# JuliaSmoothOptimizers/CaNNOLeS.jl

Hardware: AMD Instinct MI355X
Metric: Newton systems/sec (fp64), batched n=1e4 NLS; achieved HBM GB/s vs peak (higher is better)
Workload: dtype f64; 1 GPU; cfg3 band constrained NLS n=10000 nequ=10000 ncon=50, 16384 independent problems per GPU, one newton_system! per problem per step; batch_per_gpu=16384, total_problems=16384, ordering=canonical+early, nnzL_stored=145150, nnzL_exact=100180, fronts=1000, all_success=True

## Files before the change

cannoles.jl_amd/csrc/band.cpp:

```cpp
#include "band.h"

#include <algorithm>
#include <cstdio>
#include <map>

namespace cnl {

namespace {

struct XEnt { int32_t src; };
struct RowInfo {
  int32_t dsrc = -1, ndiag = 0;
  std::vector<int32_t> xs, srcs;
};
struct BorderInfo {
  int32_t dsrc = -1, ndiag = 0;
  std::vector<int32_t> xs, srcs;
};

struct RowOp { int32_t di, j[BAND_NB], rr, r; };
struct StepOp {
  int32_t flags = 0;
  int32_t dg[3] = {-1, -1, -1}, rho = -1, od[2 * BAND_HW], bc[2] = {-1, -1}, rx = -1;
  int32_t border = -1;
  int32_t xpiv = -1;
  int32_t lev_b = -1, lev_x = -1;
  std::vector<RowOp> rows;
  StepOp() { for (int i = 0; i < 2 * BAND_HW; i++) od[i] = -1; }
};
inline int32_t rhs_src(int64_t i) { return (int32_t)(-(i + 2)); }

struct Packer {
  int32_t len[3];
  struct Piece { int32_t arr, base, slot; };
  std::vector<Piece> pieces;
  bool pack(std::vector<int32_t> (&need)[3]) {
    pieces.clear();
    for (int a = 0; a < 3; a++) {
      std::vector<int32_t>& v = need[a];
      std::sort(v.begin(), v.end());
      v.erase(std::unique(v.begin(), v.end()), v.end());
      size_t i = 0;
      while (i < v.size()) {
        int32_t b = v[i];
        if (b > len[a] - 8) b = len[a] - 8;
        if (b < 0) return false;
        pieces.push_back({a, b, (int32_t)pieces.size()});
        while (i < v.size() && v[i] < b + 8) i++;
      }
    }
    return (int)pieces.size() <= npiece;
  }
  int32_t npiece = BAND_NPIECE;
  int32_t esz = 8;
  int32_t off(int a, int32_t e) const {
    for (const Piece& pc : pieces)
      if (pc.arr == a && e >= pc.base && e < pc.base + 8) return (int32_t)((BAND_IN_OFF + 8 * pc.slot + (e - pc.base)) * esz);
    return -1;
  }
};

}

void build_band_plan(BandPlan& B, int64_t N, int64_t nnz, const int64_t* rows1, const int64_t* cols1, int64_t nvar, int64_t nequ,
                     int64_t ncon, int nparts_wanted, int esz, int npiece) {
  B = BandPlan();
  if (esz != 8 && esz != 4) { B.ok = false; B.why = "element size must be 8 or 4 bytes"; return; }
  if (npiece != BAND_NPIECE && npiece != BAND_NPIECE_WIDE) { B.ok = false; B.why = "piece count must be 15 or 20"; return; }
  B.npiece = npiece;
  const int32_t LOUT_OFF = band_lout_off(npiece), DX_OFF = band_dx_off(npiece), DR_OFF = band_dr_off(npiece), ZERO_OFF = band_zero_off(npiece);
  const int32_t EW = band_ew(npiece);
  auto EF = [npiece](int f) { return band_ef(f, npiece); };
  auto no = [&](const std::string& w) { B.ok = false; B.why = w; };
  const int64_t n = nvar, m = nequ, p = ncon;
  if (N != n + m + p) return no("N != nvar + nequ + ncon");
  if (n < 2 * BAND_NB + 2 || nnz < 16 || N < 16 || nnz >= (1 << 27) || N >= (1 << 27)) return no("size out of range");
  B.n = (int32_t)n; B.N = (int32_t)N; B.nnz = (int32_t)nnz;
  std::vector<std::vector<int32_t>> xx_of_col(n);
  std::vector<int32_t> xx_row(nnz, -1);
  std::vector<RowInfo> R(m);
  std::vector<BorderInfo> L(p);
  for (int64_t e = 0; e < nnz; e++) {
    const int64_t r0 = rows1[e] - 1, c0 = cols1[e] - 1;
    if (r0 < 0 || r0 >= N || c0 < 0 || c0 > r0) return no("entry outside the lower triangle");
    if (r0 < n) {
      if (r0 - c0 > BAND_HW) return no("Hessian entry outside the band");
      xx_of_col[c0].push_back((int32_t)e);
      xx_row[e] = (int32_t)r0;
    } else if (r0 < n + m) {
      RowInfo& q = R[r0 - n];
      if (c0 < n) { q.xs.push_back((int32_t)c0); q.srcs.push_back((int32_t)e); }
      else if (c0 == r0) { q.dsrc = (int32_t)e; q.ndiag++; }
      else return no("entry inside the residual block off its diagonal");
    } else {
      BorderInfo& q = L[r0 - n - m];
      if (c0 < n) { q.xs.push_back((int32_t)c0); q.srcs.push_back((int32_t)e); }
      else if (c0 == r0) { q.dsrc = (int32_t)e; q.ndiag++; }
      else return no("entry coupling a multiplier with a residual or another multiplier");
    }
  }
  for (int64_t r = 0; r < m; r++) {
    RowInfo& q = R[r];
    if (q.ndiag != 1) return no("residual row without exactly one diagonal entry");
    if (!q.xs.empty()) {
      const auto mm = std::minmax_element(q.xs.begin(), q.xs.end());
      if (*mm.second - *mm.first > BAND_HW) return no("residual row wider than the band");
      std::vector<int32_t> s = q.xs;
      std::sort(s.begin(), s.end());
      if (std::adjacent_find(s.begin(), s.end()) != s.end()) return no("duplicate Jacobian entry");
    }
  }
  for (int64_t k = 0; k < p; k++) {
    BorderInfo& q = L[k];
    if (q.ndiag != 1) return no("multiplier without exactly one diagonal entry");
    if (q.xs.empty()) return no("constraint row without entries");
  }
  const int64_t rho_begin = nnz - n;
  int nparts = nparts_wanted >= 2 && n >= 16 * BAND_NB ? 2 : 1;
  int32_t m0 = (int32_t)n;
  if (nparts == 2) {
    auto valid = [&](int64_t c) {
      if (c < BAND_NB || c + BAND_HW + BAND_NB > n) return false;
      for (int64_t k = 0; k < p; k++) {
        const auto mm = std::minmax_element(L[k].xs.begin(), L[k].xs.end());
        if (!(*mm.second < c + BAND_HW || *mm.first >= c)) return false;
      }
      return true;
    };
    const int64_t want = (n - BAND_HW) / 2;
    int64_t found = -1;
    for (int64_t dlt = 0; dlt <= n / 4 && found < 0; dlt++) {
      if (valid(want + dlt)) found = want + dlt;
      else if (valid(want - dlt)) found = want - dlt;
    }
    if (found < 0) nparts = 1;
    else m0 = (int32_t)found;
  }
  B.nparts = nparts; B.m0 = m0;
  int64_t loff = 0;
  for (int part = 0; part < nparts; part++) {
    BandPart& Q = B.part[part];
    std::vector<int32_t> seq;
    int32_t npiv;
    if (nparts == 1) { for (int32_t x = 0; x < n; x++) seq.push_back(x); npiv = (int32_t)n; }
    else if (part == 0) { for (int32_t x = 0; x < m0 + BAND_HW; x++) seq.push_back(x); npiv = m0; }
    else { for (int32_t x = (int32_t)n - 1; x >= m0; x--) seq.push_back(x); npiv = (int32_t)n - m0 - BAND_HW; }
    std::vector<int32_t> pos(n, -1);
    for (size_t t = 0; t < seq.size(); t++) pos[seq[t]] = (int32_t)t;
    auto owns = [&](int32_t hi) { return nparts == 1 || (part == 0 ? hi < m0 + BAND_HW : hi >= m0 + BAND_HW); };
    const int32_t nsteps_raw = npiv + BAND_HW;
    std::vector<StepOp> S(nsteps_raw);
    for (int32_t u = 0; u < nsteps_raw; u++) {
      if (u < (int32_t)seq.size()) S[u].flags |= BF_ENTER_X;
      if (u >= BAND_HW && u - BAND_HW < npiv) { S[u].flags |= BF_PIVOT_X; S[u].xpiv = seq[u - BAND_HW]; }
    }
    for (int64_t c = 0; c < n; c++)
      for (int32_t e : xx_of_col[c]) {
        const int32_t a = xx_row[e], b = (int32_t)c;
        if (!owns(std::max(a, b))) continue;
        if (pos[a] < 0 || pos[b] < 0) return no("internal: entry outside its part");
        const int32_t u = std::max(pos[a], pos[b]), k = std::abs(pos[a] - pos[b]);
        StepOp& st = S[u];
        if (k == 0) {
          if (e >= rho_begin) { if (st.rho >= 0) return no("two rho slots on one variable"); st.rho = e; }
          else {
            if (st.rho >= 0) return no("plain entry behind the rho slot");
            int q = 0;
            while (q < 3 && st.dg[q] >= 0) q++;
            if (q == 3) return no("more than three plain entries on one diagonal position");
            st.dg[q] = e;
          }
        } else {
          int32_t* o = st.od + 2 * (k - 1);
          if (o[0] < 0) o[0] = e;
          else if (o[1] < 0) o[1] = e;
          else return no("more than two entries on one off-diagonal position");
        }
      }
    for (size_t t = 0; t < seq.size(); t++)
      if (owns(seq[t])) S[t].rx = rhs_src(seq[t]);
    struct RowAt { int32_t r, u, deadline; };
    std::vector<RowAt> mine_rows;
    for (int64_t r = 0; r < m; r++) {
      const RowInfo& q = R[r];
      int32_t hi = -1;
      for (int32_t x : q.xs) hi = std::max(hi, x);
      if (q.xs.empty()) { if (part == 0) mine_rows.push_back({(int32_t)r, 0, 0}); continue; }
      if (!owns(hi)) continue;
      int32_t plo = 1 << 30, phi = -1;
      for (int32_t x : q.xs) { if (pos[x] < 0) return no("internal: row outside its part"); plo = std::min(plo, pos[x]); phi = std::max(phi, pos[x]); }
      if (phi - plo > BAND_HW) return no("residual row wider than the band");
      mine_rows.push_back({(int32_t)r, phi, std::min(plo + BAND_HW, nsteps_raw - 1)});
    }
    std::stable_sort(mine_rows.begin(), mine_rows.end(), [&](const RowAt& x, const RowAt& y) { return x.u != y.u ? x.u < y.u : (part == 0 ? x.r < y.r : x.r > y.r); });
    {
      int32_t next_free = 0;
      for (RowAt& ra : mine_rows) {
        const int32_t want = std::max(ra.u, next_free);
        if (want <= ra.deadline) ra.u = want;
        next_free = std::max(next_free, ra.u + 1);
      }
    }
    for (const RowAt& ra : mine_rows) {
      const RowInfo& q = R[ra.r];
      const int32_t u = ra.u;
      RowOp ro;
      ro.di = q.dsrc; ro.rr = rhs_src(n + ra.r); ro.r = ra.r;
      for (int s = 0; s < BAND_NB; s++) ro.j[s] = -1;
      for (size_t i = 0; i < q.xs.size(); i++) {
        const int32_t k = pos[q.xs[i]] - (u - BAND_HW);
        if (k < 0 || k > BAND_HW) return no("internal: row column outside the window");
        ro.j[k] = q.srcs[i];
      }
      S[u].rows.push_back(ro);
    }
    for (StepOp& st : S) {
      if (st.rows.size() > 15) return no("more than 15 residual rows complete at one variable");
      std::sort(st.rows.begin(), st.rows.end(), [&](const RowOp& x, const RowOp& y) { return part == 0 ? x.r < y.r : x.r > y.r; });
    }
    std::vector<std::pair<int32_t, int32_t>> live;
    for (int64_t k = 0; k < p; k++) {
      const BorderInfo& q = L[k];
      int32_t lo = 1 << 30, hi = -1;
      for (int32_t x : q.xs) { lo = std::min(lo, x); hi = std::max(hi, x); }
      const bool mine = nparts == 1 || (part == 0 ? hi < m0 + BAND_HW : !(hi < m0 + BAND_HW));
      if (!mine) continue;
      int32_t plo = 1 << 30, phi = -1;
      for (int32_t x : q.xs) { if (pos[x] < 0) return no("constraint row straddles the split"); plo = std::min(plo, pos[x]); phi = std::max(phi, pos[x]); }
      if (phi >= nsteps_raw) return no("internal: border beyond the part");
      const int32_t bi = (int32_t)(Q.borders.size() / BAND_BW);
      Q.borders.push_back(q.dsrc); Q.borders.push_back((int32_t)(n + m + k)); Q.borders.push_back((int32_t)(n + m + k)); Q.borders.push_back(0);
      if (S[plo].flags & (BF_ENTER_B | BF_PIVOT_B)) return no("two multipliers live at once");
      if (S[phi].flags & (BF_ENTER_B | BF_PIVOT_B) && plo != phi) return no("two multipliers live at once");
      S[plo].flags |= BF_ENTER_B; S[plo].border = bi;
      S[phi].flags |= BF_PIVOT_B; S[phi].border = bi;
      live.push_back({plo, phi});
      for (size_t i = 0; i < q.xs.size(); i++) {
        StepOp& st = S[pos[q.xs[i]]];
        if (st.bc[0] < 0) st.bc[0] = q.srcs[i];
        else if (st.bc[1] < 0) st.bc[1] = q.srcs[i];
        else return no("more than two entries on one constraint position");
      }
    }
    std::sort(live.begin(), live.end());
    for (size_t i = 1; i < live.size(); i++)
      if (live[i].first <= live[i - 1].second) return no("two multipliers live at once");
    const int32_t nsteps = nsteps_raw;
    Q.nsteps = nsteps; Q.npiv = npiv;
    int32_t nev = 0;
    for (StepOp& st : S) {
      if (st.flags & BF_PIVOT_B) st.lev_b = nev++;
      if (st.flags & BF_PIVOT_X) st.lev_x = nev++;
    }
    Q.nevents = nev;
    Q.loff = loff;
    const int64_t lpart = (int64_t)nev * BAND_LREC;
    loff += (lpart + 16 + 7) & ~(int64_t)7;
    Q.epochs.clear();
    Q.fops.clear(); Q.bops.clear();
    std::vector<std::vector<int32_t>> fblocks(nsteps), bblocks(nsteps);
    Packer pk;
    pk.len[0] = (int32_t)nnz; pk.len[1] = (int32_t)N; pk.len[2] = (int32_t)(lpart + 16);
    pk.esz = esz; pk.npiece = npiece;
    if (lpart + 16 >= (1 << 27)) return no("factor too long");
    const int32_t ZB = ZERO_OFF * esz;
    std::string why_not;
    auto try_epoch = [&](const int32_t u0, const int32_t u1, int32_t* E) -> bool {
      auto no = [&](const std::string& w) { why_not = w; return false; };
      int32_t ev_lo = 1 << 30, ev_hi = -1, x_lo = 1 << 30, x_hi = -1, x_cnt = 0, r_lo = 1 << 30, r_hi = -1, r_cnt = 0;
      for (int32_t u = u0; u < u1; u++) {
        const StepOp& st = S[u];
        for (int32_t ev : {st.lev_b, st.lev_x}) if (ev >= 0) { ev_lo = std::min(ev_lo, ev); ev_hi = std::max(ev_hi, ev); }
        if (st.flags & BF_PIVOT_X) { x_lo = std::min(x_lo, st.xpiv); x_hi = std::max(x_hi, st.xpiv); x_cnt++; }
        for (const RowOp& ro : st.rows) { r_lo = std::min(r_lo, ro.r); r_hi = std::max(r_hi, ro.r); r_cnt++; }
      }
      int32_t oplen = 0;
      for (int32_t u = u0; u < u1; u++) oplen += BAND_SW + BAND_RW * (int32_t)S[u].rows.size();
      if (oplen > BAND_REC_MAX) return no("the blocks of an epoch do not fit the record buffer");
      E[EF(BE_OPLEN)] = oplen;
      const int32_t lbase = ev_hi >= 0 ? ev_lo * BAND_LREC : 0, lcnt = ev_hi >= 0 ? (ev_hi - ev_lo + 1) * BAND_LREC : 0;
      const int32_t uh = std::min(u1, u0 + BAND_EPOCH / 2);
      int32_t evh_lo = 1 << 30, evh_hi = -1, evg_lo = 1 << 30, evg_hi = -1;
      for (int32_t u = u0; u < u1; u++)
        for (int32_t ev : {S[u].lev_b, S[u].lev_x})
          if (ev >= 0) {
            if (u < uh) { evh_lo = std::min(evh_lo, ev); evh_hi = std::max(evh_hi, ev); }
            else { evg_lo = std::min(evg_lo, ev); evg_hi = std::max(evg_hi, ev); }
          }
      const int32_t lbase1 = evh_hi >= 0 ? evh_lo * BAND_LREC : 0, lcnt1 = evh_hi >= 0 ? (evh_hi - evh_lo + 1) * BAND_LREC : 0;
      const int32_t lbase2 = evg_hi >= 0 ? evg_lo * BAND_LREC : 0, lcnt2 = evg_hi >= 0 ? (evg_hi - evg_lo + 1) * BAND_LREC : 0;
      if (lcnt1 > BAND_LOUT_MAX || lcnt2 > BAND_LOUT_MAX) return no("more factor records in half an epoch than the ring holds");
      if (x_cnt && x_hi - x_lo + 1 != x_cnt) return no("pivots of an epoch are not consecutive variables");
      if (r_cnt && r_hi - r_lo + 1 != r_cnt) return no("rows of an epoch are not consecutive");
      if (x_cnt > BAND_DX_MAX || r_cnt > BAND_DR_MAX) return no("more outputs in an epoch than the rings hold");
      E[EF(BE_LBASE)] = lbase1; E[EF(BE_LCNT)] = lcnt1; E[EF(BE_LBASE2)] = lbase2; E[EF(BE_LCNT2)] = lcnt2;
      E[EF(BE_DXLO)] = x_cnt ? x_lo : 0; E[EF(BE_DXCNT)] = x_cnt;
      E[EF(BE_DRLO)] = r_cnt ? (int32_t)(n + r_lo) : 0; E[EF(BE_DRCNT)] = r_cnt;
      for (int dir = 0; dir < 2; dir++) {
        std::vector<int32_t> need[3];
        auto want = [&](int32_t s) {
          if (s == -1) return;
          if (s >= 0) need[0].push_back(s); else need[1].push_back(-(s + 2));
        };
        for (int32_t u = u0; u < u1; u++) {
          const StepOp& st = S[u];
          if (dir == 0) {
            for (int q = 0; q < 3; q++) want(st.dg[q]);
            want(st.rho);
            for (int q = 0; q < 2 * BAND_HW; q++) want(st.od[q]);
            want(st.bc[0]); want(st.bc[1]); want(st.rx);
          }
          for (const RowOp& ro : st.rows) {
            want(ro.di); want(ro.rr);
            for (int s = 0; s < BAND_NB; s++) want(ro.j[s]);
          }
        }
        if (dir == 1) for (int32_t i = 0; i < lcnt; i++) need[2].push_back(lbase + i);
        if (!pk.pack(need)) {
          std::string w = "an epoch needs more operand pieces than a lane holds (part " + std::to_string(part) + ", steps " + std::to_string(u0) + ".." + std::to_string(u1) + (dir ? ", backward" : ", forward") + ":";
          for (auto& pc : pk.pieces) w += " " + std::to_string(pc.arr) + ":" + std::to_string(pc.base);
          B.pieces_short = true;
          return no(w + ")");
        }
        int32_t* PP = E + EF(dir == 0 ? BE_FP : BE_BP);
        for (int k = 0; k < npiece; k++) PP[k] = -1;
        for (const Packer::Piece& pc : pk.pieces) PP[pc.slot] = pc.base | (pc.arr << 28);
        auto off = [&](int32_t s) -> int32_t {
          if (s == -1) return ZB;
          return s >= 0 ? pk.off(0, s) : pk.off(1, -(s + 2));
        };
        for (int32_t u = u0; u < u1; u++) {
          const StepOp& st = S[u];
          std::vector<int32_t>& blk = dir == 0 ? fblocks[u] : bblocks[u];
          blk.assign(BAND_SW + BAND_RW * st.rows.size(), 0);
          blk[BS_FLAGS] = st.flags | ((int32_t)st.rows.size() << 8);
          blk[BS_BORDER] = st.border;
          for (int q = 0; q < 3; q++) blk[BS_DG0 + q] = dir == 0 ? off(st.dg[q]) : ZB;
          blk[BS_RHO] = dir == 0 ? off(st.rho) : ZB;
          if (dir == 0 && st.rho < 0) blk[BS_FLAGS] |= 1 << 16;
          for (int q = 0; q < 2 * BAND_HW; q++) blk[BS_OD + q] = dir == 0 ? off(st.od[q]) : ZB;
          blk[BS_BC0] = dir == 0 ? off(st.bc[0]) : ZB; blk[BS_BC1] = dir == 0 ? off(st.bc[1]) : ZB;
          blk[BS_RX] = dir == 0 ? off(st.rx) : ZB;
          if (dir == 0) {
            const int32_t lbh = u < uh ? lbase1 : lbase2;
            blk[BS_LB] = st.lev_b >= 0 ? (LOUT_OFF + st.lev_b * BAND_LREC - lbh) * esz : ZB;
            blk[BS_LX] = st.lev_x >= 0 ? (LOUT_OFF + st.lev_x * BAND_LREC - lbh) * esz : ZB;
            blk[BS_DX] = ZB;
          } else {
            blk[BS_LB] = st.lev_b >= 0 ? pk.off(2, st.lev_b * BAND_LREC) : ZB;
            blk[BS_LX] = st.lev_x >= 0 ? pk.off(2, st.lev_x * BAND_LREC) : ZB;
            for (int32_t ev : {st.lev_b, st.lev_x})
              if (ev >= 0)
                for (int i = 0; i < BAND_LREC; i++)
                  if (pk.off(2, ev * BAND_LREC + i) != pk.off(2, ev * BAND_LREC) + esz * i) return no("internal: factor record not contiguous in LDS");
            blk[BS_DX] = (st.flags & BF_PIVOT_X) ? (DX_OFF + st.xpiv - x_lo) * esz : ZB;
          }
          for (size_t i = 0; i < st.rows.size(); i++) {
            const RowOp& ro = st.rows[i];
            int32_t* rb = blk.data() + BAND_SW + BAND_RW * i;
            rb[BR_DI] = off(ro.di); rb[BR_RR] = off(ro.rr);
            for (int s = 0; s < BAND_NB; s++) rb[BR_J0 + s] = off(ro.j[s]);
            rb[BR_DR] = (DR_OFF + ro.r - r_lo) * esz;
            if (rb[BR_DI] < 0 || rb[BR_RR] < 0) return no("internal: operand without a piece");
            for (int s = 0; s < BAND_NB; s++) if (rb[BR_J0 + s] < 0) return no("internal: operand without a piece");
          }
          for (int q = BS_DG0; q <= BS_RX; q++) if (blk[q] < 0) return no("internal: operand without a piece");
        }
      }
      return true;
    };
    for (int32_t u0 = 0; u0 < nsteps;) {
      std::vector<int32_t> E(EW, 0);
      const int32_t cnt = std::min<int32_t>(BAND_EPOCH, nsteps - u0);
      if (!try_epoch(u0, u0 + cnt, E.data())) return no(why_not);
      E[EF(BE_NSTEP)] = cnt;
      Q.epochs.insert(Q.epochs.end(), E.begin(), E.end());
      u0 += cnt;
    }
    Q.nepochs = (int32_t)(Q.epochs.size() / EW);
    {
      int32_t fo = 0;
      for (int32_t e = 0; e < Q.nepochs; e++) { Q.epochs[(size_t)e * EW + EF(BE_FOFF)] = fo; fo += Q.epochs[(size_t)e * EW + EF(BE_OPLEN)]; }
      int32_t bo = 0;
      for (int32_t e = Q.nepochs - 1; e >= 0; e--) { Q.epochs[(size_t)e * EW + EF(BE_BOFF)] = bo; bo += Q.epochs[(size_t)e * EW + EF(BE_OPLEN)]; }
    }
    for (int32_t u = 0; u < nsteps; u++) Q.fops.insert(Q.fops.end(), fblocks[u].begin(), fblocks[u].end());
    for (int32_t u = nsteps - 1; u >= 0; u--) {
      const std::vector<int32_t>& blk = bblocks[u];
      Q.bops.insert(Q.bops.end(), blk.begin(), blk.begin() + BAND_SW);
      const int nr = (int)((blk.size() - BAND_SW) / BAND_RW);
      for (int i = nr - 1; i >= 0; i--) Q.bops.insert(Q.bops.end(), blk.begin() + BAND_SW + BAND_RW * i, blk.begin() + BAND_SW + BAND_RW * (i + 1));
    }
    Q.fops.resize(Q.fops.size() + BAND_REC_MAX + 64, 0);
    Q.bops.resize(Q.bops.size() + BAND_REC_MAX + 64, 0);
  }
  B.lsize = loff + 8;
  B.ok = true;
}

}
```

cannoles.jl_amd/csrc/band.h:

```cpp
#pragma once
#include <cstdint>
#include <string>
#include <vector>

namespace cnl {

constexpr int BAND_HW = 4;
constexpr int BAND_NB = BAND_HW + 1;
constexpr int BAND_EPOCH = 8;
constexpr int BAND_NS = BAND_EPOCH;
constexpr int BAND_NPIECE = 15;
constexpr int BAND_NPIECE_WIDE = 20;
constexpr int BAND_REC_MAX = 256;
constexpr int BAND_LREC = 6;

constexpr int BAND_IN_OFF = 0;
constexpr int BAND_LOUT_OFF = BAND_NPIECE * 8;
constexpr int BAND_LOUT_MAX = 32;
constexpr int BAND_DX_OFF = BAND_LOUT_OFF;
constexpr int BAND_DX_MAX = 8;
constexpr int BAND_DR_OFF = BAND_DX_OFF + BAND_DX_MAX;
constexpr int BAND_DR_MAX = 24;
constexpr int BAND_ZERO_OFF = BAND_LOUT_OFF + BAND_LOUT_MAX;
constexpr int BAND_LANE_DOUBLES = BAND_ZERO_OFF + 1;
static_assert(BAND_DR_OFF + BAND_DR_MAX <= BAND_ZERO_OFF && BAND_LANE_DOUBLES % 2 == 1, "lane block layout");
constexpr int band_lout_off(int npc) { return npc * 8; }
constexpr int band_dx_off(int npc) { return band_lout_off(npc); }
constexpr int band_dr_off(int npc) { return band_dx_off(npc) + BAND_DX_MAX; }
constexpr int band_zero_off(int npc) { return band_lout_off(npc) + BAND_LOUT_MAX; }
constexpr int band_lane_elems(int npc) { return band_zero_off(npc) + 1; }
static_assert(band_lout_off(BAND_NPIECE) == BAND_LOUT_OFF && band_dr_off(BAND_NPIECE) == BAND_DR_OFF && band_zero_off(BAND_NPIECE) == BAND_ZERO_OFF &&
              band_lane_elems(BAND_NPIECE) == BAND_LANE_DOUBLES && band_lane_elems(BAND_NPIECE_WIDE) % 2 == 1, "lane block layout");

constexpr int BAND_IL_GROUP = 32;
constexpr long long band_il_blocks(long long len) { return (len + 7) / 8 + 1; }
constexpr long long band_il_len(long long batch, long long len) { return (batch + BAND_IL_GROUP - 1) / BAND_IL_GROUP * band_il_blocks(len) * (BAND_IL_GROUP * 8); }
constexpr long long band_il_index(long long p, long long e, long long len) {
  return ((p / BAND_IL_GROUP * band_il_blocks(len) + e / 8) * BAND_IL_GROUP + p % BAND_IL_GROUP) * 8 + e % 8;
}

enum {
  BS_FLAGS = 0,
  BS_DG0, BS_DG1, BS_DG2,
  BS_RHO,
  BS_OD,
  BS_BC0 = BS_OD + 2 * BAND_HW, BS_BC1,
  BS_RX,
  BS_LB,
  BS_LX,
  BS_DX,
  BS_BORDER,
  BS_SPARE,
  BAND_SW = 20
};
enum { BF_ENTER_B = 1, BF_PIVOT_B = 2, BF_PIVOT_X = 4, BF_ENTER_X = 8 };
enum { BR_DI = 0, BR_J0 , BR_RR = BR_J0 + BAND_NB, BR_DR, BAND_RW = 8 };
enum {
  BE_FP = 0,
  BE_BP = BE_FP + BAND_NPIECE,
  BE_LBASE = BE_BP + BAND_NPIECE,
  BE_LCNT, BE_LBASE2, BE_LCNT2,
  BE_DXLO, BE_DXCNT,
  BE_DRLO, BE_DRCNT,
  BE_NSTEP,
  BE_FOFF,
  BE_BOFF,
  BE_OPLEN,
  BAND_EW = 44
};
constexpr int band_ef(int f, int npc) { return f < BE_BP ? f : f < BE_LBASE ? f + (npc - BAND_NPIECE) : f + 2 * (npc - BAND_NPIECE); }
constexpr int band_ew(int npc) { return (band_ef(BE_OPLEN, npc) + 1 + 3) & ~3; }
static_assert(band_ew(BAND_NPIECE) == BAND_EW && band_ew(BAND_NPIECE_WIDE) == 52, "epoch block layout");
enum { BB_DSRC = 0, BB_RHS, BB_DOUT, BB_SPARE, BAND_BW = 4 };

struct BandPart {
  int32_t nsteps = 0, nepochs = 0, npiv = 0, nevents = 0;
  std::vector<int32_t> fops, bops;
  std::vector<int32_t> epochs;
  std::vector<int32_t> borders;
  int64_t loff = 0;
};

struct BandPlan {
  bool ok = false;
  std::string why;
  bool pieces_short = false;
  int32_t npiece = BAND_NPIECE;
  int32_t nparts = 0;
  int32_t m0 = 0;
  int32_t n = 0, N = 0, nnz = 0;
  int64_t lsize = 0;
  BandPart part[2];
};

void build_band_plan(BandPlan& B, int64_t N, int64_t nnz, const int64_t* rows1, const int64_t* cols1, int64_t nvar, int64_t nequ,
                     int64_t ncon, int nparts_wanted, int esz = 8, int npiece = BAND_NPIECE);

}
```

cannoles.jl_amd/csrc/band.hip:

```cpp
#include <hip/hip_runtime.h>

#include "band.h"
#include "kernels.h"

namespace cnl {

namespace {

template <class T>
__device__ __forceinline__ T* as_global(T* p) {
  return (T*)(__attribute__((address_space(1))) T*)p;
}

typedef const __attribute__((address_space(4))) int* cptr;
__device__ __forceinline__ cptr as_const(const int* p) { return (cptr)(const __attribute__((address_space(1))) int*)p; }

constexpr int EXCH_OFF = BAND_IN_OFF;
static_assert(48 <= BAND_NPIECE * 8, "exchange area inside the operand pieces");

__device__ __forceinline__ constexpr int sidx(int a, int b) { return a >= b ? a * (a + 1) / 2 + b : b * (b + 1) / 2 + a; }

template <class T>
__device__ __forceinline__ T rrcp(T d) {
  T r;
// ... 105 lines not shown
#pragma unroll
    for (int ka = 0; ka < BAND_NB; ka++) {
      const T ta = J[ka] * w;
#pragma unroll
      for (int kb = 0; kb <= ka; kb++) W.S[sidx(lslot(PH, ka), lslot(PH, kb))] = fma(ta, J[kb], W.S[sidx(lslot(PH, ka), lslot(PH, kb))]);
      W.c[lslot(PH, ka)] = fma(tr, J[ka], W.c[lslot(PH, ka)]);
    }
  }
  if (fl & BF_PIVOT_B) {
    cptr bt = borders + BAND_BW * __builtin_amdgcn_readfirstlane(st.v[BS_BORDER]);
    W.S55 += gvals[pv + band_il_offset(bt[BB_DSRC], vstride)];
    W.c5 += has_rhs ? grhs[pr + band_il_offset(bt[BB_RHS], rstride)] : T(0);
    const T d = W.S55;
    npos += d > tol;
    nzer += fabs(d) <= tol;
    const T r = rrcp(d);
    T l[BAND_NB], w[BAND_NB];
#pragma unroll
    for (int k = 0; k < BAND_NB; k++) { w[k] = W.X[lslot(PH, k)]; l[k] = rdiv(w[k], d, r); }
    const T z = rdiv(W.c5, d, r);
#pragma unroll
    for (int ka = 0; ka < BAND_NB; ka++) {
#pragma unroll
      for (int kb = 0; kb <= ka; kb++) W.S[sidx(lslot(PH, ka), lslot(PH, kb))] = fma(w[ka], -l[kb], W.S[sidx(lslot(PH, ka), lslot(PH, kb))]);
      W.c[lslot(PH, ka)] = fma(w[ka], -z, W.c[lslot(PH, ka)]);
    }
    if constexpr (direct_records(RNL)) {
      if (recst) {
        T* lo = recp + frec_index<T>(st.v[BS_LB], recb0) * RNL;
#pragma unroll
        for (int k = 0; k < BAND_NB; k++) lo[k * RNL] = l[k];
        lo[BAND_NB * RNL] = z;
      }
    } else {
      T* lo = reinterpret_cast<T*>(myb + st.v[BS_LB]);
#pragma unroll
      for (int k = 0; k < BAND_NB; k++) lo[k] = l[k];
      lo[BAND_NB] = z;
    }
#pragma unroll
    for (int k = 0; k < BAND_NB; k++) W.X[lslot(PH, k)] = T(0);
    W.S55 = T(0); W.c5 = T(0);
  }
  if (fl & BF_PIVOT_X) {
    const T d = W.S[sidx(ps, ps)];
    npos += d > tol;
    nzer += fabs(d) <= tol;
    const T r = rrcp(d);
    T l[BAND_NB], w[BAND_NB];
#pragma unroll
    for (int k = 1; k < BAND_NB; k++) { w[k] = W.S[sidx(lslot(PH, k), ps)]; l[k] = rdiv(w[k], d, r); }
    const T w5 = W.X[ps], l5 = rdiv(w5, d, r), z = rdiv(W.c[ps], d, r);
#pragma unroll
    for (int ka = 1; ka < BAND_NB; ka++) {
#pragma unroll
      for (int kb = 1; kb <= ka; kb++) W.S[sidx(lslot(PH, ka), lslot(PH, kb))] = fma(w[ka], -l[kb], W.S[sidx(lslot(PH, ka), lslot(PH, kb))]);
      W.X[lslot(PH, ka)] = fma(w5, -l[ka], W.X[lslot(PH, ka)]);
      W.c[lslot(PH, ka)] = fma(w[ka], -z, W.c[lslot(PH, ka)]);
    }
    W.S55 = fma(w5, -l5, W.S55);
    W.c5 = fma(w5, -z, W.c5);
    if constexpr (direct_records(RNL)) {
      if (recst) {
        T* lo = recp + frec_index<T>(st.v[BS_LX], recb0) * RNL;
#pragma unroll
        for (int k = 1; k < BAND_NB; k++) lo[(k - 1) * RNL] = l[k];
        lo[4 * RNL] = l5;
        lo[5 * RNL] = z;
      }
    } else {
      T* lo = reinterpret_cast<T*>(myb + st.v[BS_LX]);
#pragma unroll
      for (int k = 1; k < BAND_NB; k++) lo[k - 1] = l[k];
      lo[4] = l5;
      lo[5] = z;
    }
  }
}

template <class T>
struct BOps { T lx[BAND_LREC], lb[BAND_LREC], rj[BAND_NB]; T rdr, rrr; };
template <class T>
__device__ __forceinline__ void bload(BOps<T>& P, const Rec& st, const RowRec& row0, const int fl, char* myb) {
#pragma unroll
  for (int q = 0; q < BAND_LREC; q++) { P.lx[q] = T(0); P.lb[q] = T(0); }
#pragma unroll
  for (int k = 0; k < BAND_NB; k++) P.rj[k] = T(0);
  P.rdr = T(1); P.rrr = T(0);
  if (fl & BF_PIVOT_X) {
    const T* lo = reinterpret_cast<const T*>(myb + st.v[BS_LX]);
#pragma unroll
    for (int q = 0; q < BAND_LREC; q++) P.lx[q] = lo[q];
  }
  if (fl & BF_PIVOT_B) {
    const T* lo = reinterpret_cast<const T*>(myb + st.v[BS_LB]);
#pragma unroll
    for (int q = 0; q < BAND_LREC; q++) P.lb[q] = lo[q];
  }
  if ((fl >> 8) & 255) {
#pragma unroll
    for (int k = 0; k < BAND_NB; k++) P.rj[k] = LDSD(row0.v[BR_J0 + k]);
    P.rdr = LDSD(row0.v[BR_DI]);
    P.rrr = LDSD(row0.v[BR_RR]);
  }
}
template <int PH, class T>
__device__ __forceinline__ void bstep(T (&xs)[NS + 1], const BOps<T>& OP, const Rec& st, const RowRec& row0, const int fl, const char* recb,
                                      const int o, char* myb, cptr borders, T* __restrict__ gd, long long pd, bool okme) {
  constexpr int ps = lslot(PH, 0);
  const int nrows = (fl >> 8) & 255;
  const T (&lx)[BAND_LREC] = OP.lx;
  const T (&lb)[BAND_LREC] = OP.lb;
  const T (&rj)[BAND_NB] = OP.rj;
  const T rdr = OP.rdr, rrr = OP.rrr;
  if (fl & BF_PIVOT_X) {
    T x = lx[5];
#pragma unroll
    for (int k = 1; k < BAND_NB; k++) x = fma(-lx[k - 1], xs[lslot(PH, k)], x);
    x = fma(-lx[4], xs[NS], x);
    xs[ps] = x;
    LDSW(st.v[BS_DX]) = -x;
  }
  if (fl & BF_PIVOT_B) {
    T x = lb[BAND_NB];
#pragma unroll
    for (int k = 0; k < BAND_NB; k++) x = fma(-lb[k], xs[lslot(PH, k)], x);
    xs[NS] = x;
    if (okme) gd[pd + borders[BAND_BW * __builtin_amdgcn_readfirstlane(st.v[BS_BORDER]) + BB_DOUT]] = -x;
  }
  for (int i = 0; i < nrows; i++) {
    T J[BAND_NB], dr, rr;
    int dro;
    if (i == 0) {
#pragma unroll
      for (int k = 0; k < BAND_NB; k++) J[k] = rj[k];
      dr = rdr; rr = rrr; dro = row0.v[BR_DR];
    } else {
      RowRec rb;
      load_row(rb, recb, o + BAND_SW + BAND_RW * i);
#pragma unroll
      for (int k = 0; k < BAND_NB; k++) J[k] = LDSD(rb.v[BR_J0 + k]);
      dr = LDSD(rb.v[BR_DI]); rr = LDSD(rb.v[BR_RR]); dro = rb.v[BR_DR];
    }
    T acc = -rr;
#pragma unroll
    for (int k = 0; k < BAND_NB; k++) acc = fma(J[k], xs[lslot(PH, k)], acc);
    LDSW(dro) = rdiv(acc, dr, rrcp(dr));
  }
  if (fl & BF_ENTER_B) xs[NS] = T(0);
}

}

#define EF(F) band_ef(F, NPC)
template <class T, int NL, int NPC>
__global__ void __launch_bounds__(128, (NL <= 8 && NPC == BAND_NPIECE ? 2 : 1)) band_newton_kernel(const BandDev P, const LaunchArgs Ain) {
  constexpr int NI = NL / 8;
  constexpr int LANE_D = band_lane_elems(NPC), LOUT_OFF = band_lout_off(NPC), DX_OFF = band_dx_off(NPC), DR_OFF = band_dr_off(NPC),
                ZERO_OFF = band_zero_off(NPC), EW = band_ew(NPC);
  static_assert(NPC == BAND_NPIECE || NPC == BAND_NPIECE_WIDE, "fifteen or twenty operand pieces");
  constexpr int ES = (int)sizeof(T), LS = ES == 8 ? 3 : 2;
  static_assert(ES == 8 || ES == 4, "double or float");
  extern __shared__ double lds[];
  const int mode = Ain.mode, batch = Ain.batch;
  T* const gvals = as_global(reinterpret_cast<T*>(Ain.vals));
  const T* const grhs = as_global(reinterpret_cast<const T*>(Ain.rhs));
  T* const gd = as_global(reinterpret_cast<T*>(Ain.d));
  T* const gL = as_global(reinterpret_cast<T*>(Ain.L));
  const int lane = threadIdx.x & 63;
  const int part = __builtin_amdgcn_readfirstlane((int)(threadIdx.x >> 6));
  const int lq = lane >> 3, le = lane & 7;
  const int prob0 = blockIdx.x * NL;
  const bool has_rhs = mode != MODE_FACTOR && grhs != nullptr;
  T* const ldsT = reinterpret_cast<T*>(lds);
  char* wblk = reinterpret_cast<char*>(ldsT + (size_t)part * NL * LANE_D);
  char* recb = reinterpret_cast<char*>(ldsT + (size_t)P.nparts * NL * LANE_D) + (size_t)part * BAND_REC_MAX * 4;
  double* ctrl = reinterpret_cast<double*>(reinterpret_cast<char*>(ldsT + (size_t)P.nparts * NL * LANE_D) + (size_t)P.nparts * BAND_REC_MAX * 4);
  const int* fops_g = as_global(P.fops[part]);
  const int* bops_g = as_global(P.bops[part]);
  cptr epochs = as_const(P.epochs[part]);
  cptr borders = as_const(P.borders[part]);
  const int nepochs = P.nepochs[part];
  const int nnz = P.nnz, N = P.N;
  const long long lsize = P.lsize;
  constexpr int G8 = BAND_IL_GROUP * 8;
  static_assert(BAND_IL_GROUP % NL == 0, "a workgroup's problems lie in one group of the interleaved layout");
  const bool vil = (Ain.layout & 1) != 0, ril = (Ain.layout & 2) != 0;
  const int vstride = vil ? G8 : 0, rstride = ril ? G8 : 0;
  const long long ilg = prob0 / BAND_IL_GROUP;
  const int ilp = (prob0 % BAND_IL_GROUP) * 8;
  const T* vbase = gvals + (vil ? ilg * band_il_blocks(nnz) * G8 + ilp : (long long)prob0 * nnz);
  const T* rbase = !has_rhs ? gvals : grhs + (ril ? ilg * band_il_blocks(N) * G8 + ilp : (long long)prob0 * N);
  constexpr bool DREC = direct_records(NL);
  T* lbase_g = gL + (long long)prob0 * lsize + (DREC ? 0 : P.loff[part]);
  const int loff8 = DREC ? (int)P.loff[part] : 0;
  T* const recp = lbase_g + (long long)loff8 * NL + (lane < NL ? lane : 0);
  T* dbase = gd ? gd + (long long)prob0 * N : nullptr;
  unsigned movp[NI], ldsb[NI];
  bool movok[NI];
#pragma unroll
  for (int i = 0; i < NI; i++) {
    int pl = i * 8 + lq;
    movok[i] = prob0 + pl < batch;
    if (!movok[i]) pl = batch - 1 - prob0;
    movp[i] = (unsigned)pl;
    ldsb[i] = ((unsigned)(i * 8 + lq) * (unsigned)LANE_D + (unsigned)le) << LS;
  }
  const bool clane = lane < NL;
  const int cprob = prob0 + (clane ? lane : 0);
  const bool valid = clane && cprob < batch;
  const int cpl = valid ? cprob - prob0 : batch - 1 - prob0;
  char* myb = wblk + (size_t)(clane ? lane : 0) * LANE_D * ES;
  const long long pv = vil ? ilg * band_il_blocks(nnz) * G8 + ilp + cpl * 8 : (long long)(prob0 + cpl) * nnz;
  const long long pr = ril ? ilg * band_il_blocks(N) * G8 + ilp + cpl * 8 : (long long)(prob0 + cpl) * N;
  for (int t = lane; t < NL; t += 64) *reinterpret_cast<T*>(wblk + ((size_t)t * LANE_D + ZERO_OFF) * ES) = T(0);

  const T tol = (T)Ain.params[0], kdec = (T)Ain.params[2], kinc = (T)Ain.params[3], klarge = (T)Ain.params[4], rho0 = (T)Ain.params[5],
          rhomax = (T)Ain.params[6], rhomin = (T)Ain.params[7];
  T rho = T(0), wrote = T(0);
  T rho_old = (mode == MODE_NEWTON && valid) ? as_global(reinterpret_cast<T*>(Ain.rho_old))[cprob] : T(0);
  int nfact = 0;
  bool done = !valid, success = false, ovr = false;
  const bool recst = valid && mode != MODE_FACTOR;

  static_assert(NI <= 4, "at most four problem groups per mover lane");
  T stg[NPC][NI];
  int4 rstg0;
  int pcs[NPC];
  static_assert(BAND_REC_MAX <= 256, "record buffer: one dwordx4 per lane");
#define BAND_ISSUE1(K, I) if constexpr (I < NI) stg[K][I] = *reinterpret_cast<const T*>(pb + ((movp[I] * strd + tl) << LS));
#define BAND_COMMIT1(K, I) if constexpr (I < NI) *reinterpret_cast<T*>(wblk + ldsb[I] + (BAND_IN_OFF + 8 * K) * ES) = stg[K][I];
#define BAND_ISSUE(K)                                                                                                         \
  if (pcs[K] >= 0) {                                                                                      \
    const int pc = pcs[K];                                                                                                    \
    const int arr = pc >> 28;                                                                                                 \
    const int el_ = (pc & ((1 << 28) - 1)) + (arr == 2 ? loff8 : 0);                                                          \
                               \
    const bool il_ = arr == 0 ? vil : arr == 1 ? ril : DREC;                                              \
    const int ilw_ = arr == 2 ? NL * 8 : BAND_IL_GROUP * 8;     \
    const int m_ = il_ ? (el_ & 7) : 0;                                                                                       \
    const unsigned gap_ = il_ && !(DREC && arr == 2) ? (unsigned)(ilw_ - 8) : 0u;                                              \
    const unsigned tm_ = arr == 2 && DREC ? (unsigned)NL : 1u;                                                                \
    const char* pb = (arr == 0 ? reinterpret_cast<const char*>(vbase) : arr == 1 ? reinterpret_cast<const char*>(rbase)       \
                                                                                 : reinterpret_cast<const char*>(lbase_g)) +   \
                     ((il_ ? (long long)(el_ >> 3) * ilw_ : (long long)el_) << LS);                                           \
    const unsigned strd = DREC ? (arr == 2 ? 1u : il_ ? 8u : arr == 0 ? (unsigned)nnz : (unsigned)N)                         \
                               : (il_ ? 8u : arr == 0 ? (unsigned)nnz : arr == 1 ? (unsigned)N : (unsigned)lsize);             \
    const unsigned t_ = (unsigned)m_ + (unsigned)le;                                                                          \
    const unsigned tl = t_ * tm_ + (t_ >> 3) * gap_;                                                                          \
    BAND_ISSUE1(K, 0) BAND_ISSUE1(K, 1) BAND_ISSUE1(K, 2) BAND_ISSUE1(K, 3)                                                   \
  }
#define BAND_COMMIT(K) { BAND_COMMIT1(K, 0) BAND_COMMIT1(K, 1) BAND_COMMIT1(K, 2) BAND_COMMIT1(K, 3) }
#define BAND_ISSUE_DESC(EP, OFS) { cptr E_ = (EP) + (OFS); _Pragma("unroll") for (int k_ = 0; k_ < NPC; k_++) pcs[k_] = E_[k_]; }
#define BAND_ISSUE_REC(OPS, OPOFF) { rstg0 = (reinterpret_cast<const int4*>((OPS) + (OPOFF)) + lane)[0]; }
#define BAND_ISSUE_ALL(EP, OFS, OPS, OPOFF)                                                                                   \
  {                                                                                                                           \
    BAND_ISSUE_DESC(EP, OFS)                                                                                                  \
    BAND_ISSUE(0) BAND_ISSUE(1) BAND_ISSUE(2) BAND_ISSUE(3) BAND_ISSUE(4) BAND_ISSUE(5) BAND_ISSUE(6) BAND_ISSUE(7)           \
    BAND_ISSUE(8) BAND_ISSUE(9) BAND_ISSUE(10) BAND_ISSUE(11) BAND_ISSUE(12) BAND_ISSUE(13) BAND_ISSUE(14)                    \
    if constexpr (NPC > 15) { BAND_ISSUE(15) BAND_ISSUE(16) BAND_ISSUE(17) BAND_ISSUE(18) BAND_ISSUE(19) }                    \
    BAND_ISSUE_REC(OPS, OPOFF)                                                                                                \
  }
#define BAND_COMMIT_ALL()                                                                                                     \
  {                                                                                                                           \
    BAND_COMMIT(0) BAND_COMMIT(1) BAND_COMMIT(2) BAND_COMMIT(3) BAND_COMMIT(4) BAND_COMMIT(5) BAND_COMMIT(6) BAND_COMMIT(7)   \
    BAND_COMMIT(8) BAND_COMMIT(9) BAND_COMMIT(10) BAND_COMMIT(11) BAND_COMMIT(12) BAND_COMMIT(13) BAND_COMMIT(14)             \
    if constexpr (NPC > 15) { BAND_COMMIT(15) BAND_COMMIT(16) BAND_COMMIT(17) BAND_COMMIT(18) BAND_COMMIT(19) }               \
    reinterpret_cast<int4*>(recb)[lane] = rstg0;                                                                              \
  }
#define BAND_ISSUE_G0()                                                                                                       \
  if constexpr (NPC > 15) { BAND_ISSUE(0) BAND_ISSUE(1) BAND_ISSUE(2) BAND_ISSUE(3) BAND_ISSUE(4) }                           \
  else { BAND_ISSUE(0) BAND_ISSUE(1) BAND_ISSUE(2) BAND_ISSUE(3) }
#define BAND_ISSUE_G1()                                                                                                       \
  if constexpr (NPC > 15) { BAND_ISSUE(5) BAND_ISSUE(6) BAND_ISSUE(7) BAND_ISSUE(8) BAND_ISSUE(9) }                           \
  else { BAND_ISSUE(4) BAND_ISSUE(5) BAND_ISSUE(6) BAND_ISSUE(7) }
#define BAND_ISSUE_G2()                                                                                                       \
  if constexpr (NPC > 15) { BAND_ISSUE(10) BAND_ISSUE(11) BAND_ISSUE(12) BAND_ISSUE(13) BAND_ISSUE(14) }                      \
  else { BAND_ISSUE(8) BAND_ISSUE(9) BAND_ISSUE(10) BAND_ISSUE(11) }
#define BAND_ISSUE_G3()                                                                                                       \
  if constexpr (NPC > 15) { BAND_ISSUE(15) BAND_ISSUE(16) BAND_ISSUE(17) BAND_ISSUE(18) BAND_ISSUE(19) }                      \
  else { BAND_ISSUE(12) BAND_ISSUE(13) BAND_ISSUE(14) }

  Win<T> W;
  int npos = 0, nzer = 0;
  T lj[6], zj[4];
  for (int q = 0; q < 6; q++) lj[q] = T(0);
  for (int q = 0; q < 4; q++) zj[q] = T(0);
  while (true) {
#pragma unroll
    for (int q = 0; q < NS * (NS + 1) / 2; q++) W.S[q] = T(0);
#pragma unroll
    for (int q = 0; q < NS; q++) { W.X[q] = T(0); W.c[q] = T(0); }
    W.S55 = T(0); W.c5 = T(0);
    npos = 0; nzer = 0;
    BAND_ISSUE_ALL(epochs, EF(BE_FP), fops_g, 0)
    for (int e = 0; e < nepochs; e++) {
      cptr E = epochs + e * EW;
      BAND_COMMIT_ALL()
      const bool more_ = e + 1 < nepochs;
      if (more_) BAND_ISSUE_DESC(epochs + (e + 1) * EW, EF(BE_FP))
      const int nst = E[EF(BE_NSTEP)];
      const int recb1 = E[EF(BE_LBASE)] - LOUT_OFF, recb2 = E[EF(BE_LBASE2)] - LOUT_OFF;
      int o = 0;
      Rec stC, stN;
      RowRec rwC, rwN;
      load_rec(stC, recb, 0);
      load_row(rwC, recb, BAND_SW);
#define BAND_FSTEP(PHV)                                                                                                     \
      if (PHV < nst) {                                                                                                      \
        const int fl = __builtin_amdgcn_readfirstlane(stC.v[BS_FLAGS]);                                                     \
        const int onext = o + BAND_SW + BAND_RW * ((fl >> 8) & 255);                                                        \
        if (PHV + 1 < nst) { load_rec(stN, recb, onext); load_row(rwN, recb, onext + BAND_SW); }                            \
        if (clane) {                                                                                                        \
          FOps<T> op_;                                                                                                      \
          fload(op_, stC, rwC, fl, myb);                                                                                    \
          fstep<PHV, NL>(W, op_, stC, fl, recb, o, myb, gvals, grhs, borders, pv, pr, has_rhs, rho, ovr, tol, npos, nzer, vstride, rstride, \
                         recp, PHV < BAND_EPOCH / 2 ? recb1 : recb2, recst);                                              \
        }                                                                                                                   \
        o = onext; stC = stN; rwC = rwN;                                                                                    \
      }
#define BAND_LFLUSH(LB, LC)                                                                                                 \
      if constexpr (!DREC) {                                                                                                \
        if (mode != MODE_FACTOR) {                                                                                          \
          const int lc_ = (LC);                                                                                             \
          char* lout = reinterpret_cast<char*>(lbase_g) + ((long long)(LB) << LS);                                          \
          T lx_[BAND_LOUT_MAX / 8][NI];                                                                                     \
          _Pragma("unroll") for (int cpc = 0; cpc < BAND_LOUT_MAX / 8; cpc++)                                               \
            _Pragma("unroll") for (int i = 0; i < NI; i++) lx_[cpc][i] = *reinterpret_cast<const T*>(wblk + ldsb[i] + (LOUT_OFF + 8 * cpc) * ES); \
          _Pragma("unroll") for (int cpc = 0; cpc < BAND_LOUT_MAX / 8; cpc++)                                               \
            _Pragma("unroll") for (int i = 0; i < NI; i++)                                                                  \
              if (movok[i] && cpc * 8 + le < lc_)                                                                           \
                *reinterpret_cast<T*>(lout + (((movp[i] * (unsigned)lsize + (unsigned)le) << LS) + 8 * ES * cpc)) = lx_[cpc][i]; \
        }                                                                                                                   \
      }
      BAND_FSTEP(0)
      if (more_) { BAND_ISSUE_G0() }
      BAND_FSTEP(1)
      if (more_) { BAND_ISSUE_G1() }
      BAND_FSTEP(2)
      if (more_) { BAND_ISSUE_G2() }
      BAND_FSTEP(3)
      if (more_) { BAND_ISSUE_G3() BAND_ISSUE_REC(fops_g, epochs[(e + 1) * EW + EF(BE_FOFF)]) }
      BAND_LFLUSH(E[EF(BE_LBASE)], E[EF(BE_LCNT)])
      BAND_FSTEP(4) BAND_FSTEP(5) BAND_FSTEP(6) BAND_FSTEP(7)
      static_assert(BAND_EPOCH == 8, "eight step instantiations per epoch");
      if (nst == BAND_EPOCH) {
#pragma unroll
        for (int a = 0; a < NS; a++)
#pragma unroll
          for (int b = 0; b <= a; b++)
            if (b < 4) W.S[sidx(a, b)] = T(0);
#pragma unroll
        for (int a = 0; a < 4; a++) { W.X[a] = T(0); W.c[a] = T(0); }
      }
      BAND_LFLUSH(E[EF(BE_LBASE2)], E[EF(BE_LCNT2)])
    }
    int tpos = npos, tzer = nzer;
    if (P.nparts == 2) {
      if (clane) {
        T* ex = reinterpret_cast<T*>(myb + EXCH_OFF * ES);
#pragma unroll
        for (int q = 0; q < NS * (NS + 1) / 2; q++) ex[q] = W.S[q];
#pragma unroll
        for (int q = 0; q < NS; q++) ex[36 + q] = W.c[q];
        ex[44] = (T)npos; ex[45] = (T)nzer;
      }
      __syncthreads();
      if (part == 0 && clane) {
        const T* exL = reinterpret_cast<const T*>(myb + EXCH_OFF * ES);
        const T* exR = reinterpret_cast<const T*>(myb + (size_t)NL * LANE_D * ES + EXCH_OFF * ES);
        const int tL = P.m0 % NS, tR = (P.n - 1 - P.m0) % NS;
        T SJ[10], cJ[4];
#pragma unroll
        for (int i = 0; i < 4; i++) {
          const int aL = (tL + i) % NS, aR = (tR - i + NS) % NS;
#pragma unroll
          for (int j = 0; j <= i; j++) {
            const int bL = (tL + j) % NS, bR = (tR - j + NS) % NS;
            const int iL = aL >= bL ? aL * (aL + 1) / 2 + bL : bL * (bL + 1) / 2 + aL;
            const int iR = aR >= bR ? aR * (aR + 1) / 2 + bR : bR * (bR + 1) / 2 + aR;
            SJ[i * (i + 1) / 2 + j] = exL[iL] + exR[iR];
          }
          cJ[i] = exL[36 + aL] + exR[36 + aR];
        }
        tpos += (int)exR[44]; tzer += (int)exR[45];
#pragma unroll
        for (int i = 0; i < 4; i++) {
          const T d = SJ[sidx(i, i)];
          tpos += d > tol;
          tzer += fabs(d) <= tol;
          const T r = rrcp(d);
          zj[i] = rdiv(cJ[i], d, r);
          T w[4];
#pragma unroll
          for (int a = i + 1; a < 4; a++) { w[a] = SJ[sidx(a, i)]; lj[sidx(a - 1, i)] = rdiv(w[a], d, r); }
#pragma unroll
          for (int a = i + 1; a < 4; a++) {
#pragma unroll
            for (int b = i + 1; b <= a; b++) SJ[sidx(a, b)] = fma(w[a], -lj[sidx(b - 1, i)], SJ[sidx(a, b)]);
            cJ[a] = fma(w[a], -zj[i], cJ[a]);
          }
        }
      }
    }
    bool alldone = true;
// ... 39 lines not shown
    return;
  }
  {
    T xs[NS + 1];
#pragma unroll
    for (int q = 0; q < NS + 1; q++) xs[q] = T(0);
    if (P.nparts == 2) {
      if (part == 0 && clane) {
        T xj[4];
        xj[3] = zj[3];
        xj[2] = fma(-lj[sidx(2, 2)], xj[3], zj[2]);
        xj[1] = fma(-lj[sidx(2, 1)], xj[3], fma(-lj[sidx(1, 1)], xj[2], zj[1]));
        xj[0] = fma(-lj[sidx(2, 0)], xj[3], fma(-lj[sidx(1, 0)], xj[2], fma(-lj[sidx(0, 0)], xj[1], zj[0])));
        T* ex = reinterpret_cast<T*>(myb + EXCH_OFF * ES);
        T* exR = reinterpret_cast<T*>(myb + (size_t)NL * LANE_D * ES + EXCH_OFF * ES);
#pragma unroll
        for (int i = 0; i < 4; i++) {
          ex[i] = xj[i]; exR[i] = xj[i];
          if (valid && success) gd[(long long)cprob * N + P.m0 + i] = -xj[i];
        }
      }
      __syncthreads();
      if (clane) {
        const T* ex = reinterpret_cast<const T*>(myb + EXCH_OFF * ES);
        const int t0 = part == 0 ? P.m0 % NS : (P.n - 1 - P.m0) % NS;
#pragma unroll
        for (int s = 0; s < NS; s++) {
          const int i = part == 0 ? (s - t0 + NS) % NS : (t0 - s + NS) % NS;
          xs[s] = i < 4 ? ex[i] : T(0);
        }
      }
    }
    if (part == 0 && clane) ctrl[NL + lane] = (valid && success) ? 2.0 : 0.0;
    __syncthreads();
    bool movst[NI];
#pragma unroll
    for (int i = 0; i < NI; i++) movst[i] = movok[i] && ctrl[NL + i * 8 + lq] != 0.0;
    const bool okme = valid && ctrl[NL + lane % NL] != 0.0 && clane;
    const long long pd = (long long)(prob0 + cpl) * N;
    BAND_ISSUE_ALL(epochs + (nepochs - 1) * EW, EF(BE_BP), bops_g, 0)
    for (int e = nepochs - 1; e >= 0; e--) {
      cptr E = epochs + e * EW;
      BAND_COMMIT_ALL()
      const bool more_ = e > 0;
      if (more_) BAND_ISSUE_DESC(epochs + (e - 1) * EW, EF(BE_BP))
      const int nst = E[EF(BE_NSTEP)];
      int o = 0;
      Rec stC, stN;
      RowRec rwC, rwN;
      load_rec(stC, recb, 0);
      load_row(rwC, recb, BAND_SW);
#define BAND_BSTEP(PHV)                                                                                                     \
      if (PHV < nst) {                                                                                                      \
        const int fl = __builtin_amdgcn_readfirstlane(stC.v[BS_FLAGS]);                                                     \
        const int onext = o + BAND_SW + BAND_RW * ((fl >> 8) & 255);                                                        \
        if (PHV > 0) { load_rec(stN, recb, onext); load_row(rwN, recb, onext + BAND_SW); }                                  \
        if (clane) {                                                                                                        \
          BOps<T> op_;                                                                                                      \
          bload(op_, stC, rwC, fl, myb);                                                                                    \
          bstep<PHV>(xs, op_, stC, rwC, fl, recb, o, myb, borders, gd, pd, okme);                                           \
        }                                                                                                                   \
        o = onext; stC = stN; rwC = rwN;                                                                                    \
      }
      BAND_BSTEP(7)
      if (more_) { BAND_ISSUE_G0() }
      BAND_BSTEP(6)
      if (more_) { BAND_ISSUE_G1() }
      BAND_BSTEP(5)
      if (more_) { BAND_ISSUE_G2() }
      BAND_BSTEP(4)
      if (more_) { BAND_ISSUE_G3() BAND_ISSUE_REC(bops_g, epochs[(e - 1) * EW + EF(BE_BOFF)]) }
      BAND_BSTEP(3) BAND_BSTEP(2) BAND_BSTEP(1) BAND_BSTEP(0)
      const int xlo = E[EF(BE_DXLO)], xc = E[EF(BE_DXCNT)], rlo = E[EF(BE_DRLO)], rc = E[EF(BE_DRCNT)];
      char* dxo = reinterpret_cast<char*>(dbase) + ((long long)xlo << LS);
      char* dro = reinterpret_cast<char*>(dbase) + ((long long)rlo << LS);
      {
        T dx_[NI], dr_[BAND_DR_MAX / 8][NI];
#pragma unroll
        for (int i = 0; i < NI; i++) dx_[i] = *reinterpret_cast<const T*>(wblk + ldsb[i] + DX_OFF * ES);
#pragma unroll
        for (int cpc = 0; cpc < BAND_DR_MAX / 8; cpc++)
#pragma unroll
          for (int i = 0; i < NI; i++) dr_[cpc][i] = *reinterpret_cast<const T*>(wblk + ldsb[i] + (DR_OFF + 8 * cpc) * ES);
#pragma unroll
        for (int i = 0; i < NI; i++)
          if (movst[i] && le < xc) *reinterpret_cast<T*>(dxo + ((movp[i] * (unsigned)N + (unsigned)le) << LS)) = dx_[i];
#pragma unroll
        for (int cpc = 0; cpc < BAND_DR_MAX / 8; cpc++)
#pragma unroll
          for (int i = 0; i < NI; i++)
            if (movst[i] && cpc * 8 + le < rc) *reinterpret_cast<T*>(dro + (((movp[i] * (unsigned)N + (unsigned)le) << LS) + 8 * ES * cpc)) = dr_[cpc][i];
      }
    }
  }
  if (part == 0 && mode == MODE_NEWTON) {
    if (nfact > 1 && rho <= rhomax) rho_old = rho;
    if (valid) {
      as_global(reinterpret_cast<T*>(Ain.rho))[cprob] = rho;
      as_global(reinterpret_cast<T*>(Ain.rho_old))[cprob] = rho_old;
      as_global(Ain.nfact)[cprob] = nfact;
      as_global(Ain.success)[cprob] = success ? 1 : 0;
    }
    for (int q = 0; q < NL; q++) {
      const int nf = __builtin_amdgcn_readlane(nfact, q);
      const int vq = __builtin_amdgcn_readlane((int)valid, q);
      if (nf > 1 && vq) {
        T wq;
        if constexpr (ES == 8) wq = __hiloint2double(__builtin_amdgcn_readlane(__double2hiint(wrote), q), __builtin_amdgcn_readlane(__double2loint(wrote), q));
        else wq = __int_as_float(__builtin_amdgcn_readlane(__float_as_int(wrote), q));
        if (vil) {
          T* vg = gvals + ilg * band_il_blocks(nnz) * G8 + ilp + q * 8;
          for (int i = lane; i < P.nvar; i += 64) vg[band_il_offset(nnz - P.nvar + i, vstride)] = wq;
        } else {
          T* vt = gvals + (long long)(prob0 + q) * nnz + (nnz - P.nvar);
          for (int i = lane; i < P.nvar; i += 64) vt[i] = wq;
        }
      }
    }
  }
}

#undef EF

bool band_wide_has(int esz, int nl) { return nl == 8 || nl == 16 || (nl == 32 && esz == 4); }

size_t band_lds_bytes(int nparts, int nl, int esz, int npiece) {
  return (size_t)nparts * nl * band_lane_elems(npiece) * esz + (2 * (size_t)nl + 8) * sizeof(double) + (size_t)nparts * BAND_REC_MAX * 4;
}

template <class T>
static hipError_t launch_band_t(const BandDev& P, int nl, const LaunchArgs& a, hipStream_t stream, int npiece) {
  if (npiece != BAND_NPIECE && npiece != BAND_NPIECE_WIDE) return hipErrorInvalidConfiguration;
  const bool wide = npiece == BAND_NPIECE_WIDE;
  const size_t ldsb = band_lds_bytes(P.nparts, nl, (int)sizeof(T), npiece);
  const int grid = (a.batch + nl - 1) / nl;
  auto go = [&](auto kern) {
    hipError_t e = hipFuncSetAttribute(reinterpret_cast<const void*>(kern), hipFuncAttributeMaxDynamicSharedMemorySize, lds_attr_cap((int)ldsb));
    if (e != hipSuccess) return e;
    hipLaunchKernelGGL(kern, dim3(grid), dim3(64 * P.nparts), ldsb, stream, P, a);
    return hipGetLastError();
  };
  if (wide) {
    if constexpr (sizeof(T) == 4) { if (nl == 32) return go(band_newton_kernel<T, 32, BAND_NPIECE_WIDE>); }
    if (nl == 16) return go(band_newton_kernel<T, 16, BAND_NPIECE_WIDE>);
    if (nl == 8) return go(band_newton_kernel<T, 8, BAND_NPIECE_WIDE>);
    return hipErrorInvalidConfiguration;
  }
  if (nl == 32) return go(band_newton_kernel<T, 32, BAND_NPIECE>);
  if (nl == 16) return go(band_newton_kernel<T, 16, BAND_NPIECE>);
  if (nl == 8) return go(band_newton_kernel<T, 8, BAND_NPIECE>);
  return hipErrorInvalidConfiguration;
}

hipError_t launch_band(const BandDev& P, int nl, const LaunchArgs& a, hipStream_t stream, int npiece) { return launch_band_t<double>(P, nl, a, stream, npiece); }
hipError_t launch_band_f32(const BandDev& P, int nl, const LaunchArgs& a, hipStream_t stream, int npiece) { return launch_band_t<float>(P, nl, a, stream, npiece); }

}
```

cannoles.jl_amd/csrc/capi.cpp:

```cpp
#include <hip/hip_runtime_api.h>

#include <algorithm>
#include <atomic>
#include <chrono>
#include <condition_variable>
#include <functional>
#include <mutex>
#include <cfloat>
#include <cmath>
#include <cstdio>
#include <cstdlib>
#include <cstring>
#include <string>
#include <thread>
#include <vector>

#include "../../include/cannoles_hip.h"
#include "band.h"
#include "condense.h"
#include "dense.h"
#include "kernels.h"
#include "options.h"
#include "plan.h"

struct cnl_plan {
  cnl::Cond C;
  cnl::Plan P;
  int64_t N = 0, nnz = 0, nvar = 0, nequ = 0, ncon = 0;
  std::vector<int32_t> perm_outer;
  bool latency = false;
  bool prefer_dense = false;
  cnl::DensePlan D;
  std::vector<int32_t> gpos;
  cnl::Tuning opt{};
  std::atomic<int> refs{1};
  bool split_mode = false;
  struct BandSlot {
    cnl::BandPlan B;
    std::vector<int32_t> info, pinfo[2];
  };
  BandSlot band_prog[2][2];
};
static const char* const kBandPrefix[2][2] = {{"band_", "bandw_"}, {"band4_", "bandw4_"}};

struct cnl_handle {
  cnl_plan* plan = nullptr;
  int device = 0;
  int64_t batch = 1;
  std::vector<void*> dev_allocs;
  cnl::DevPlan dp{};
  cnl::KernelConfig cfg{};
  bool use_v2 = false;
  bool staged = false;
  const int32_t* d_tasks = nullptr;
  int* d_gcnt = nullptr;
  void* pin = nullptr;
  size_t pin_bytes = 0;
  int* d_dep = nullptr;
  int* d_status = nullptr;
  int *d_lgcnt = nullptr, *d_lad = nullptr, *d_ldep = nullptr, *d_stat = nullptr;
  long long zero_ints = 0;
  int resident_waves = 0;
  int lad_mode = 0;
  bool ladder_ran = false;
  int ntasks = 0;
  int df_waves = 1024;
  std::vector<int32_t> stage_ptr;
  bool v2_solve = false;
  bool first_attempt_only = false;
  int* d_act = nullptr;
  bool lean = false;
  cnl::DevPlan2 dp2{};
  int wpb2 = 1;
  size_t lds2 = 0;
  double* d_gs = nullptr;
  cnl::DevCond dc{};
  double* d_cbuf = nullptr;
  double* d_d2 = nullptr;
  int *d_xpos = nullptr, *d_xzer = nullptr;
  const double* last_vals = nullptr;
  double* d_L = nullptr;
  double* d_scratch = nullptr;
  double *d_vals = nullptr, *d_rhs = nullptr, *d_d = nullptr, *d_rho_old = nullptr, *d_rho = nullptr;
  int32_t *d_nfact = nullptr, *d_success = nullptr;
  int64_t *d_npos = nullptr, *d_nzero = nullptr;
  hipStream_t stream = nullptr;
  int64_t split_staged = 0;
  bool split_halves = false;
  bool in_split = false;
  cnl_handle* tail = nullptr;
  bool tail_redone = false;
  bool tail_fresh = false;
  hipStream_t aux_stream = nullptr;
  hipEvent_t ev_fork = nullptr, ev_join = nullptr;
  static constexpr int kPipeUp = 2;
  hipStream_t pipe_stream[kPipeUp + 1] = {};
  std::vector<hipEvent_t> pipe_ev;
  hipEvent_t ev0 = nullptr, ev1 = nullptr;
  bool timing = false;
  float last_ms = 0.f;
  bool factorized = false;
  std::vector<char> last_ok;
  cnl::DevJt djt{};
  cnl::DenseState* dense = nullptr;
  cnl::DenseState* gdense = nullptr;
  cnl::GeneralOps gops{};
  void* cgls_ws = nullptr;
  bool band = false;
  cnl::BandDev bd{};
  int band_nl = 16;
  int band_npiece = 15;
  bool jac_segments = false;
  int64_t jf_lo = 0, jf_n = 0, jc_lo = 0, jc_n = 0;
  int layout = 0;
  void* d_Lband = nullptr;
  bool f32 = false;
  float *f_vals = nullptr, *f_rhs = nullptr, *f_d = nullptr, *f_res = nullptr;
};

namespace {

thread_local std::string g_err;

int fail(int code, const std::string& m) {
  g_err = m;
  return code;
}

int need_f64(const cnl_handle* h, const char* fn) {
  if (h && h->f32) return fail(CNL_ERR_STATE, std::string(fn) + ": this is a Float32 handle (cnl_create_f32); it takes the _f32 entry points only");
  return CNL_OK;
}
int need_f32(const cnl_handle* h, const char* fn) {
  if (h && !h->f32) return fail(CNL_ERR_STATE, std::string(fn) + ": this is a Float64 handle; the _f32 entry points need one made by cnl_create_f32");
  return CNL_OK;
}
double* as_args(const float* p) { return reinterpret_cast<double*>(const_cast<float*>(p)); }
#define CNL_NEED_F64(h) do { if (int rc_ = need_f64((h), __func__)) return rc_; } while (0)
#define CNL_NEED_F32(h) do { if (int rc_ = need_f32((h), __func__)) return rc_; } while (0)

const char* const kHostLayout = "host-pointer calls take the reference's problem-major arrays: this handle was created with batch_layout = "
                                "CNL_LAYOUT_INTERLEAVED (device-pointer entry points only)";

void band_summaries(cnl_plan* p) {
  for (auto& row : p->band_prog)
    for (cnl_plan::BandSlot& s : row) {
      const cnl::BandPlan& Bp = s.B;
      s.info = {Bp.ok ? 1 : 0, Bp.nparts, Bp.m0, Bp.n, Bp.N, Bp.nnz, (int32_t)Bp.lsize, Bp.ok && Bp.npiece != cnl::BAND_NPIECE ? Bp.npiece : 0};
      for (int q = 0; q < 2; q++) s.pinfo[q] = {Bp.part[q].nsteps, Bp.part[q].nepochs, Bp.part[q].npiv, Bp.part[q].nevents, (int32_t)Bp.part[q].loff};
    }
}

void build_band_programs(cnl_plan* p, const int64_t* rows1, const int64_t* cols1, int esz) {
  const cnl::Tuning& o = p->opt;
  const int64_t N = p->N, nnz = p->nnz, nvar = p->nvar, nequ = p->nequ, ncon = p->ncon;
  cnl::BandPlan &B15 = p->band_prog[esz == 4][0].B, &Bw = p->band_prog[esz == 4][1].B;
  const int nparts = o.band_kernel == 2 ? 1 : 2;
  cnl::build_band_plan(B15, N, nnz, rows1, cols1, nvar, nequ, ncon, nparts, esz, cnl::BAND_NPIECE);
  Bw = cnl::BandPlan();
  Bw.why = B15.ok ? "fifteen operand pieces per epoch suffice" : B15.why;
  if (o.band_pieces != 15 && (B15.ok ? o.band_pieces == 20 : B15.pieces_short))
    cnl::build_band_plan(Bw, N, nnz, rows1, cols1, nvar, nequ, ncon, nparts, esz, cnl::BAND_NPIECE_WIDE);
}
const cnl::BandPlan& band_program(const cnl_plan* plan, bool f32) {
  return plan->band_prog[f32][plan->band_prog[f32][1].B.ok].B;
}

bool band_wide_serves_f64(const cnl_plan* plan) {
  return band_program(plan, false).npiece == cnl::BAND_NPIECE || plan->opt.band_pieces == cnl::BAND_NPIECE_WIDE;
}

#define HIPCHK(expr)                                                                                   \
  do {                                                                                                 \
    hipError_t e_ = (expr);                                                                            \
    if (e_ != hipSuccess) return fail(CNL_ERR_HIP, std::string(#expr) + ": " + hipGetErrorString(e_)); \
  } while (0)

template <class T>
int upload(cnl_handle* h, const std::vector<T>& v, const T** out) {
  void* p = nullptr;
  size_t bytes = std::max<size_t>(v.size(), 1) * sizeof(T);
  HIPCHK(hipMalloc(&p, bytes));
  h->dev_allocs.push_back(p);
  if (!v.empty()) HIPCHK(hipMemcpy(p, v.data(), v.size() * sizeof(T), hipMemcpyHostToDevice));
  *out = (const T*)p;
  return CNL_OK;
}

template <class T>
int dalloc(cnl_handle* h, T** out, size_t count) {
  void* p = nullptr;
  static const size_t G = getenv("CNL_DBG_GUARD") ? (size_t)atol(getenv("CNL_DBG_GUARD")) : 0;
  const size_t bytes = std::max<size_t>(count, 1) * sizeof(T);
  HIPCHK(hipMalloc(&p, bytes + 2 * G));
  if (G) HIPCHK(hipMemset(p, getenv("CNL_DBG_GUARD_PAT") ? atoi(getenv("CNL_DBG_GUARD_PAT")) : 0xFF, bytes + 2 * G));
  h->dev_allocs.push_back(p);
  *out = (T*)(static_cast<char*>(p) + G);
  if (G && getenv("CNL_DBG_GUARD_LOG")) fprintf(stderr, "[dalloc] #%zu %p + %zu bytes\n", h->dev_allocs.size(), (void*)*out, bytes);
  return CNL_OK;
}

int choose_config(cnl_handle* h) {
  const cnl::Plan& P = h->plan->P;
  cnl::DevPlan& dp = h->dp;
  int64_t pb_off = std::max<int64_t>(P.fwd_peak, P.bwd_peak);
  pb_off = (pb_off + 1) & ~(int64_t)1;
  int64_t wv_off = pb_off + ((P.panel_max + 1) & ~1);
  int64_t work = wv_off + 2 * (int64_t)((P.fmax + 1) & ~1);
  if (work >= ((int64_t)1 << 30)) return fail(CNL_ERR_DIM, "work area too large");
  dp.pb_off = (int32_t)pb_off;
  dp.wv_off = (int32_t)wv_off;
  dp.work_doubles = (int32_t)work;
  size_t maxlds = cnl::max_lds_bytes();
  if (maxlds == 0) return fail(CNL_ERR_HIP, "cannot query LDS size (no HIP device?)");
  maxlds = std::min<size_t>(maxlds, 160 * 1024);
  cnl::KernelConfig& c = h->cfg;
  const size_t hdr = 16 * sizeof(double);
  const size_t per = (size_t)work * sizeof(double);
  int tpp, ppb, ldsw;
  if (hdr + per <= maxlds) {
    ldsw = 1;
    if (P.fmax <= 96) {
      tpp = 64;
      size_t fit = (maxlds - hdr) / per;
      size_t fit2 = maxlds / 2 > hdr ? (maxlds / 2 - hdr) / per : 0;
      size_t cap = fit2 >= 1 ? fit2 : fit;
      size_t want = (size_t)std::min<int64_t>(16, std::max<int64_t>(1, h->batch / 256));
      ppb = 1;
      for (int cand : {16, 8, 4, 2, 1})
        if ((size_t)cand <= cap && (size_t)cand <= want) { ppb = cand; break; }
    } else {
      tpp = P.fmax <= 400 ? 256 : 1024;
      ppb = 1;
    }
  } else {
    ldsw = 0;
    tpp = P.fmax <= 96 ? 64 : (P.fmax <= 400 ? 256 : 1024);
    ppb = tpp == 64 ? 4 : 1;
  }
  const cnl::Tuning& o = h->plan->opt;
  if (o.v1_tpp > 0) tpp = o.v1_tpp;
  if (o.v1_ppb > 0) ppb = o.v1_ppb;
  if (o.v1_lds >= 0) ldsw = o.v1_lds;
  c.tpp = tpp; c.ppb = ppb; c.lds_work = ldsw;
  c.lds_bytes = hdr + (ldsw ? (size_t)ppb * per : 0);
  if (c.lds_bytes > maxlds) return fail(CNL_ERR_DIM, "kernel configuration exceeds LDS");
  return CNL_OK;
}

int setup_v2(cnl_handle* h) {
  const cnl::Plan& P = h->plan->P;
  h->use_v2 = false;
  const cnl::Tuning& o = h->plan->opt;
  if (!P.v2_ok || !o.register_front) return CNL_OK;
  if (!h->plan->gpos.empty() && (o.general_dense == 2 || (h->plan->prefer_dense && h->batch <= 16))) return CNL_OK;
  cnl::DevPlan2& d = h->dp2;
  std::vector<int32_t> rec(P.rec), brec(P.brec);
  rec.resize(rec.size() + 2048, 0);
  brec.resize(brec.size() + 2048, 0);
  int rc;
  if ((rc = upload(h, rec, &d.rec))) return rc;
  if ((rc = upload(h, brec, &d.brec))) return rc;
  d.nsuper = P.nsuper; d.N = (int32_t)P.N; d.nnz = (int32_t)P.nnz; d.rho_begin = P.rho_begin; d.nvar = (int32_t)P.nvar;
  d.N0 = (int32_t)P.N;
  d.reccap = (P.rec_maxlen + 64 + 3) & ~3;
  d.breccap = (P.brec_maxlen + 3) & ~3;
  d.recwords = std::max(d.reccap, 2 * d.breccap);
  d.u2_peak = P.u2_peak;
  d.jraw_off = (int32_t)((P.u2_peak + std::max<int64_t>(P.fs2_max, 72) + 1) & ~(int64_t)1);
  d.bpanel_off = (int32_t)((P.bwd_peak + 2 + 1) & ~(int64_t)1);
  int64_t prob = std::max<int64_t>((int64_t)d.jraw_off + (P.rec_direct && P.listprod_fronts > 0 ? 128 : 0), (int64_t)d.bpanel_off);
  prob = (prob + 1) & ~(int64_t)1;
  if (o.lds_pad) while (prob % 32 != 16) prob += 2;
  d.prob_doubles = (int32_t)prob;
  d.gs_doubles = P.gs_doubles + 64;
  d.lsize = h->dp.lsize;
  d.vstride = h->dp.vstride; d.rstride = h->dp.rstride; d.dstride = h->dp.dstride;
  if (P.rec_direct) {
    d.nnz = P.nnz_outer; d.rho_begin = P.nnz_outer - (int32_t)P.nvar;
    d.vstride = P.nnz_outer; d.rstride = P.n_outer;
    d.N0 = P.n_outer;
    if (P.d_outer) d.dstride = P.n_outer;
    d.count_d = P.d_owned == (int64_t)h->plan->C.r_dsrc.size() ? 1 : 0;
  }
  if (4 * 8 * (uint64_t)std::max<int64_t>({d.lsize, d.vstride, d.rstride, d.dstride, (int64_t)d.nnz + d.N0}) >= (1ull << 32)) return CNL_OK;
  const size_t wave_bytes = ((size_t)(d.recwords >> 1) + 4 * (size_t)d.prob_doubles + 16) * sizeof(double);
  size_t maxlds = std::min<size_t>(cnl::max_lds_bytes(), 160 * 1024);
  if (wave_bytes + 512 > maxlds) return CNL_OK;
  int wpb = 1;
  if (o.waves_per_block > 0) wpb = std::max(1, std::min(4, o.waves_per_block));
  while (wpb > 1 && wpb * wave_bytes + 512 > maxlds) wpb--;
  h->wpb2 = wpb;
  h->lds2 = wpb * wave_bytes + 512;
  if ((rc = dalloc(h, &h->d_gs, (size_t)h->batch * (size_t)d.gs_doubles))) return rc;
  h->use_v2 = true;
  h->staged = false;
  if ((rc = dalloc(h, &h->d_status, 1))) return rc;
  if (hipMemset(h->d_status, 0, sizeof(int)) != hipSuccess) return fail(CNL_ERR_HIP, "hipMemset failed");
  {
    hipDeviceProp_t prop;
    if (hipGetDeviceProperties(&prop, h->device) == hipSuccess && prop.multiProcessorCount > 0) {
      const size_t per_wg = (size_t)wpb * wave_bytes + 512;
      const long long by_lds = (long long)(std::min<size_t>(prop.maxSharedMemoryPerMultiProcessor ? prop.maxSharedMemoryPerMultiProcessor : maxlds, 160 * 1024) / per_wg) * wpb;
      const long long resident = (long long)prop.multiProcessorCount * std::max<long long>(1, std::min<long long>(8, by_lds));
      h->resident_waves = (int)std::min<long long>(resident, 1 << 20);
    }
  }
  if (!P.tasks.empty() && P.rec_direct && P.d_outer && d.count_d && o.staged) {
    std::vector<int32_t> tk;
    for (const cnl::Task& t : P.tasks) { tk.push_back(t.rec_off); tk.push_back(t.f1 - t.f0); tk.push_back(t.brec_off); tk.push_back(t.is_root); tk.push_back(t.parent); tk.push_back(t.nchild); }
    if ((rc = upload(h, tk, &h->d_tasks))) return rc;
    h->ntasks = (int)P.tasks.size();
    h->df_waves = o.dataflow_waves > 0 ? o.dataflow_waves : 1024;
    if (h->resident_waves > 0) h->df_waves = std::min(h->df_waves, h->resident_waves);
    {
      const size_t B = (size_t)h->batch, nq = (B + 3) / 4, tq = 2 * (size_t)h->ntasks * nq;
      const size_t total = 4 * B + (size_t)cnl::LAD_WORDS * nq + tq + 2 + (o.dataflow ? tq : 0);
      if ((rc = dalloc(h, &h->d_gcnt, total))) return rc;
      if (hipMemset(h->d_gcnt, 0, total * sizeof(int)) != hipSuccess) return fail(CNL_ERR_HIP, "hipMemset failed");
      h->d_lgcnt = h->d_gcnt + 2 * B;
      h->d_lad = h->d_lgcnt + 2 * B;
      h->d_ldep = h->d_lad + (size_t)cnl::LAD_WORDS * nq;
      h->d_stat = h->d_ldep + tq;
      if (o.dataflow) h->d_dep = h->d_stat + 2;
      h->zero_ints = (long long)total;
    }
    h->stage_ptr = P.stage_ptr;
    h->staged = true;
    h->lad_mode = 0;
    if (o.device_ladder && h->resident_waves >= h->ntasks) {
      const long long slots = h->resident_waves / h->ntasks, nq = (h->batch + 3) / 4;
      const long long launches = (nq + slots - 1) / slots;
      if (launches == 1 || (launches <= 4 && h->ntasks >= 16)) h->lad_mode = o.device_ladder_fused ? 2 : 1;
    }
  }
  h->v2_solve = P.rec_direct && P.d_outer && P.ncls[1] == 0 && P.ncls[2] == 0 && !o.v1_solve;
  h->lean = o.lean_kernel && P.rec_direct && P.d_outer && d.count_d && P.ncls[1] == 0 && P.ncls[2] == 0 && P.listprod_fronts == 0;
  return CNL_OK;
}

const int* dbg_ldsfill() {
  static const int pat = [] { const char* e = getenv("CNL_DBG_LDSFILL"); return e ? (int)strtol(e, nullptr, 0) : -1; }();
  static const bool on = getenv("CNL_DBG_LDSFILL") != nullptr;
  return on ? &pat : nullptr;
}

std::atomic<long long> g_launches[3];

int read_timing(cnl_handle* h) {
  HIPCHK(hipEventSynchronize(h->ev1));
  HIPCHK(hipEventElapsedTime(&h->last_ms, h->ev0, h->ev1));
  return CNL_OK;
}

int ensure_pinned(cnl_handle* h, size_t bytes) {
  if (h->pin && h->pin_bytes >= bytes) return CNL_OK;
  if (h->pin) (void)hipHostFree(h->pin);
  h->pin = nullptr;
  HIPCHK(hipHostMalloc(&h->pin, bytes, hipHostMallocDefault));
  h->pin_bytes = bytes;
  return CNL_OK;
}

template <class T, class Ok>
hipError_t copy_rows_where(Ok ok, T* dst, const T* d_src, size_t B, size_t N, hipStream_t stream) {
  size_t b0 = 0;
  while (b0 < B) {
    while (b0 < B && !ok(b0)) b0++;
    size_t b1 = b0;
    while (b1 < B && ok(b1)) b1++;
    if (b1 > b0)
      if (hipError_t e = hipMemcpyAsync(dst + b0 * N, d_src + b0 * N, (b1 - b0) * N * sizeof(T), hipMemcpyDeviceToHost, stream)) return e;
    b0 = b1;
  }
  return hipSuccess;
}

cnl::LaunchArgs shifted(cnl::LaunchArgs a, int64_t b0) {
  if (a.rho_old) a.rho_old += b0;
  if (a.rho) a.rho += b0;
  if (a.nfact) a.nfact += b0;
  if (a.success) a.success += b0;
  if (a.npos) a.npos += b0;
  if (a.nzero) a.nzero += b0;
  return a;
}

int run_band(cnl_handle* h, cnl::LaunchArgs& a, double* d_vals, const double* d_rhs, double* d_d, hipStream_t stream) {
  if (a.skip_done || a.only_if_status || (a.mode == cnl::MODE_NEWTON && !d_rhs))
    return fail(CNL_ERR_STATE, "this call is not served by the band kernels, and a band handle has no other"
                               " (no factor panels, no condensed buffer; interleaved `vals` are the band kernels' layout)");
  if (a.mode == cnl::MODE_SOLVE && !h->last_vals) return fail(CNL_ERR_STATE, "cnl_solve before cnl_factorize");
  if (const int* pat = dbg_ldsfill()) (void)cnl::launch_lds_fill(*pat, stream);
  a.vals = a.mode == cnl::MODE_SOLVE ? const_cast<double*>(h->last_vals) : d_vals;
  a.rhs = d_rhs; a.d = d_d;
  a.batch = (int)h->batch;
  a.L = static_cast<double*>(h->d_Lband);
  a.layout = h->layout;
  if (h->timing) HIPCHK(hipEventRecord(h->ev0, stream));
  const hipError_t e = h->f32 ? cnl::launch_band_f32(h->bd, h->band_nl, a, stream, h->band_npiece)
                              : cnl::launch_band(h->bd, h->band_nl, a, stream, h->band_npiece);
  g_launches[0]++;
  if (e != hipSuccess)
    return fail(CNL_ERR_HIP, std::string("band kernel launch (") + (h->f32 ? "Float32, " : "") + std::to_string(h->band_nl) +
                                 " problems per workgroup): " + hipGetErrorString(e));
  if (a.mode == cnl::MODE_FACTOR) h->last_vals = d_vals;
  if (h->timing) {
    HIPCHK(hipEventRecord(h->ev1, stream));
    return read_timing(h);
  }
  return CNL_OK;
}

int launch(cnl_handle* h, cnl::LaunchArgs& a, hipStream_t stream) {
  if (const int* pat = dbg_ldsfill()) (void)cnl::launch_lds_fill(*pat, stream);
  a.batch = (int)h->batch;
  a.lean = h->lean ? 1 : 0;
  a.back_rows = (h->lean && h->plan->P.back_rows) ? 1 : 0;
  a.L = h->d_L;
  a.scratch = h->d_scratch;
  hipError_t e;
  if (h->timing) HIPCHK(hipEventRecord(h->ev0, stream));
  if (h->use_v2 && (a.mode != cnl::MODE_SOLVE || h->v2_solve)) {
    a.scratch = h->d_gs;
    e = cnl::launch_newton2(h->dp2, h->wpb2, h->lds2, a, stream);
    g_launches[1]++;
  } else {
    e = cnl::launch_newton(h->dp, h->cfg, a, stream);
    g_launches[2]++;
  }
  if (e != hipSuccess)
    return fail(CNL_ERR_HIP, std::string("kernel launch (tpp=") + std::to_string(h->cfg.tpp) + " ppb=" + std::to_string(h->cfg.ppb) +
                                 " lds=" + std::to_string(h->cfg.lds_work) + "): " + hipGetErrorString(e));
  if (h->timing) HIPCHK(hipEventRecord(h->ev1, stream));
  return CNL_OK;
}

int launch_staged(cnl_handle* h, cnl::LaunchArgs& a, hipStream_t stream) {
  if (const int* pat = dbg_ldsfill()) (void)cnl::launch_lds_fill(*pat, stream);
  a.batch = (int)h->batch; a.L = h->d_L; a.scratch = h->d_gs;
  a.tasks = h->d_tasks; a.gcnt = h->d_gcnt; a.skip_done = 0; a.dep = h->d_dep; a.df_waves = h->df_waves;
  a.lean = h->lean ? 1 : 0;
  a.back_rows = (h->lean && h->plan->P.back_rows) ? 1 : 0;
  a.status_total = h->d_status;
  a.status_call = h->d_stat;
  a.lad = h->d_lad; a.lgcnt = h->d_lgcnt; a.ldep = h->d_ldep; a.lad_zero_ints = h->d_stat ? h->zero_ints : 0;
  a.lad_capacity = h->resident_waves;
  a.lad_mode = (a.mode == cnl::MODE_NEWTON && h->d_lad && !h->first_attempt_only) ? h->lad_mode : 0;
  h->ladder_ran = a.lad_mode != 0;
  a.spin_limit = h->plan->opt.dataflow_spin_limit > 0 ? h->plan->opt.dataflow_spin_limit : (1 << 22);
  if (h->timing) HIPCHK(hipEventRecord(h->ev0, stream));
  hipError_t e = cnl::launch_newton2_staged(h->dp2, h->wpb2, h->lds2, a, h->stage_ptr.data(), (int)h->stage_ptr.size() - 1, stream);
  if (e != hipSuccess) return fail(CNL_ERR_HIP, std::string("staged launch: ") + hipGetErrorString(e));
  return CNL_OK;
}

struct SubBatch {
  cnl_handle* h;
  int64_t batch;
  double *L, *gs, *scratch, *cbuf, *d2;
  void* Lband;
  int *xpos, *xzer, *gcnt, *dep, *lad, *stat;
  const double* last_vals;
  bool staged;
  SubBatch(cnl_handle* h_, int64_t b0, int64_t nb, bool allow_staged = true) : h(h_) {
    last_vals = h->last_vals; staged = h->staged;
    const size_t esz = h->f32 ? sizeof(float) : sizeof(double);
    if (h->last_vals) h->last_vals = reinterpret_cast<const double*>(reinterpret_cast<const char*>(h->last_vals) + b0 * h->plan->nnz * esz);
    if (!allow_staged) h->staged = false;
    batch = h->batch; L = h->d_L; gs = h->d_gs; scratch = h->d_scratch; cbuf = h->d_cbuf; d2 = h->d_d2;
    xpos = h->d_xpos; xzer = h->d_xzer; gcnt = h->d_gcnt; dep = h->d_dep; lad = h->d_lad; stat = h->d_stat;
    Lband = h->d_Lband;
    if (h->d_Lband) h->d_Lband = static_cast<char*>(h->d_Lband) + b0 * h->bd.lsize * esz;
    const cnl::Cond& C = h->plan->C;
    h->batch = nb;
    h->d_L += b0 * h->dp.lsize;
    if (h->d_gs) h->d_gs += b0 * h->dp2.gs_doubles;
    if (h->d_scratch) h->d_scratch += b0 * (int64_t)h->dp.work_doubles;
    if (h->d_cbuf) h->d_cbuf += b0 * C.cstride;
    if (h->d_d2) h->d_d2 += b0 * C.N2;
    if (h->d_xpos) h->d_xpos += b0;
    if (h->d_xzer) h->d_xzer += b0;
    if (h->d_gcnt) h->d_gcnt += 2 * b0;
    h->d_dep = nullptr; h->d_lad = nullptr; h->d_stat = nullptr;
  }
  ~SubBatch() {
    h->batch = batch; h->d_L = L; h->d_gs = gs; h->d_scratch = scratch; h->d_cbuf = cbuf; h->d_d2 = d2;
    h->d_xpos = xpos; h->d_xzer = xzer; h->d_gcnt = gcnt; h->d_dep = dep; h->d_lad = lad; h->d_stat = stat;
    h->last_vals = last_vals; h->staged = staged; h->d_Lband = Lband;
  }
};

int run(cnl_handle* h, cnl::LaunchArgs& a, double* d_vals, const double* d_rhs, double* d_d, hipStream_t stream);

int run_split(cnl_handle* h, cnl::LaunchArgs& a, double* d_vals, const double* d_rhs, double* d_d, hipStream_t stream) {
  if (!h->aux_stream && !h->tail && !h->split_halves) {
    HIPCHK(hipStreamCreateWithFlags(&h->aux_stream, hipStreamNonBlocking));
    HIPCHK(hipEventCreateWithFlags(&h->ev_fork, hipEventDisableTiming));
    HIPCHK(hipEventCreateWithFlags(&h->ev_join, hipEventDisableTiming));
  }
  const int64_t nA = h->split_staged, nB = h->batch - nA, nnz = h->plan->nnz, N = h->plan->N;
  const bool tm = h->timing;
  if (tm) HIPCHK(hipEventRecord(h->ev0, stream));
  h->timing = false;
  h->in_split = true;
  if (h->tail) {
    cnl_handle* t = h->tail;
    const bool on_tail = a.mode != cnl::MODE_SOLVE || h->tail_fresh;
    int rc;
    {
      SubBatch view(h, 0, nA, true);
      cnl::LaunchArgs b = a;
      rc = run(h, b, d_vals, d_rhs, d_d, stream);
    }
    if (rc == CNL_OK) {
      cnl::LaunchArgs b = shifted(a, nA);
      double* tv = d_vals ? d_vals + nA * nnz : nullptr;
      const double* tr = d_rhs ? d_rhs + nA * N : nullptr;
      double* td = d_d ? d_d + nA * N : nullptr;
      if (on_tail) {
        t->first_attempt_only = h->first_attempt_only;
        rc = run(t, b, tv, tr, td, stream);
        t->first_attempt_only = false;
        if (rc == CNL_OK && a.mode != cnl::MODE_SOLVE) { t->last_vals = tv; t->factorized = true; h->tail_fresh = true; }
      } else {
        SubBatch view(h, nA, nB, true);
        rc = run(h, b, tv, tr, td, stream);
      }
    }
    h->in_split = false;
    h->timing = tm;
    if (rc) return rc;
    if (a.mode == cnl::MODE_FACTOR) h->last_vals = d_vals;
    if (tm) {
      HIPCHK(hipEventRecord(h->ev1, stream));
      return read_timing(h);
    }
    return CNL_OK;
  }
  if (h->split_halves) {
    int rc = CNL_OK;
    for (int part = 0; part < 2 && rc == CNL_OK; part++) {
      const int64_t b0 = part ? nA : 0, nb = part ? nB : nA;
      SubBatch view(h, b0, nb, true);
      cnl::LaunchArgs b = shifted(a, b0);
      rc = run(h, b, d_vals ? d_vals + b0 * nnz : nullptr, d_rhs ? d_rhs + b0 * N : nullptr, d_d ? d_d + b0 * N : nullptr, stream);
    }
    h->in_split = false;
    h->timing = tm;
    if (rc) return rc;
    if (a.mode == cnl::MODE_FACTOR) h->last_vals = d_vals;
    if (tm) {
      HIPCHK(hipEventRecord(h->ev1, stream));
      return read_timing(h);
// ... 195 lines not shown
  if ((rc = dalloc(h, &h->d_rho, 3 * B + 8))) return rc;
  h->d_rho_old = h->d_rho + B;
  h->d_nfact = reinterpret_cast<int32_t*>(h->d_rho_old + B);
  h->d_success = h->d_nfact + B;
  if ((rc = dalloc(h, &h->d_npos, B * 2))) return rc;
  h->d_nzero = h->d_npos + B;
  return CNL_OK;
}

}

struct cnl_multi {
  std::vector<cnl_handle*> h;
  std::vector<int64_t> start, count;
  std::vector<int> device;
  int64_t N = 0, nnz = 0, batch = 0;
  std::vector<std::thread> workers;
  std::mutex mu;
  std::condition_variable cv_job, cv_done;
  std::function<int(size_t)> job;
  uint64_t generation = 0;
  size_t pending = 0;
  bool stop = false;
  std::vector<int> rc;
  std::vector<std::string> msg;
};

namespace {
void multi_worker(cnl_multi* m, size_t i) {
  (void)hipSetDevice(m->device[i]);
  uint64_t seen = 0;
  for (;;) {
    std::function<int(size_t)> f;
    {
      std::unique_lock<std::mutex> lk(m->mu);
      m->cv_job.wait(lk, [&] { return m->stop || m->generation != seen; });
      if (m->stop) return;
      seen = m->generation;
      f = m->job;
    }
    const int r = f(i);
    {
      std::lock_guard<std::mutex> lk(m->mu);
      m->rc[i] = r;
      if (r) m->msg[i] = g_err;
      if (--m->pending == 0) m->cv_done.notify_all();
    }
  }
}

template <class F>
int multi_run(cnl_multi* m, F f) {
  const size_t n = m->h.size();
  {
    std::unique_lock<std::mutex> lk(m->mu);
    m->job = f;
    m->rc.assign(n, CNL_OK);
    m->msg.assign(n, std::string());
    m->pending = n;
    m->generation++;
    m->cv_job.notify_all();
    m->cv_done.wait(lk, [&] { return m->pending == 0; });
    m->job = nullptr;
  }
  for (size_t i = 0; i < n; i++)
    if (m->rc[i]) return fail(m->rc[i], "shard " + std::to_string(i) + " (device " + std::to_string(m->device[i]) + "): " + m->msg[i]);
  return CNL_OK;
}
}


template <class T>
static int prepare_impl(cnl_handle* h, int64_t nnzhF, int64_t nnzhc, int64_t nnzjF, int64_t nnzjc, const T* d_hF, const T* d_hc, const T* d_Jx,
                        const T* d_Jcx, const T* d_delta, T* d_vals, void* stream) {
  const cnl::DevJt& J = h->djt;
  if (nnzhF < 0 || nnzhc < 0 || nnzjF < 0 || nnzjc < 0 || nnzhF + nnzhc + nnzjF + nnzjc + J.nequ + J.ncon + J.nvar != J.nnz)
    return fail(CNL_ERR_DIM, "segment sizes do not add up to nnz (7-segment layout of src/CaNNOLeS.jl:256-315)");
  if (J.ncon > 0 && (!d_hc || !d_Jcx || !d_delta)) return fail(CNL_ERR_ARG, "hc / Jcx / delta are required when ncon > 0");
  if (J.ncon == 0 && (nnzhc != 0 || nnzjc != 0)) return fail(CNL_ERR_DIM, "constraint segments must be empty when ncon == 0");
  HIPCHK(hipSetDevice(h->device));
  hipError_t e = cnl::launch_prepare((int)nnzhF, (int)nnzhc, (int)nnzjF, (int)nnzjc, J.nvar, J.nequ, J.ncon, d_hF, d_hc, d_Jx, d_Jcx,
                                     d_delta, d_vals, (int)h->batch, h->layout & 1, (hipStream_t)stream);
  if (e != hipSuccess) return fail(CNL_ERR_HIP, std::string("prepare_newton_system: ") + hipGetErrorString(e));
  return CNL_OK;
}

template <class T>
static int cgls_impl(cnl_handle* h, const cnl::JacSrcT<T>& S, const T* d_r, T* d_lambda, T* d_Jxtr, T atol, T rtol, int64_t itmax,
                     int ones_if_zero, int32_t* d_iters, void* stream) {
  if (h->djt.ncon == 0) return CNL_OK;
  if (!d_lambda) return fail(CNL_ERR_ARG, "null lambda");
  if (h->djt.ncon > 1024) return fail(CNL_ERR_DIM, "cnl_cgls_multipliers_dev supports at most 1024 constraints");
  HIPCHK(hipSetDevice(h->device));
  T* ws = static_cast<T*>(h->cgls_ws);
  if (!ws) {
    int rc = dalloc(h, &ws, (size_t)h->batch * 2 * (size_t)h->djt.nvar);
    if (rc) return rc;
    h->cgls_ws = ws;
  }
  if (itmax <= 0) itmax = (int64_t)h->djt.nvar + h->djt.ncon;
  hipError_t e = cnl::launch_cgls(h->djt, S, d_r, d_lambda, d_Jxtr, ws, d_iters, atol, rtol, (int)itmax, ones_if_zero,
                                  (int)h->batch, (hipStream_t)stream);
  if (e != hipSuccess) return fail(CNL_ERR_HIP, std::string("cgls: ") + hipGetErrorString(e));
  return CNL_OK;
}

template <class T>
static int jac_source(cnl_handle* h, int64_t nnzjF, int64_t nnzjc, const T* d_Jx, const T* d_Jcx, cnl::JacSrcT<T>* S) {
  if (!h->jac_segments) return fail(CNL_ERR_STATE, "the J_F / J_c entries of this pattern are not one run of slots each (7-segment layout of src/CaNNOLeS.jl:256-315)");
  if (nnzjF != h->jf_n || nnzjc != h->jc_n) return fail(CNL_ERR_DIM, "nnzjF / nnzjc do not match the pattern's Jacobian entries");
  if (h->jf_n == 0) return fail(CNL_ERR_STATE, "the pattern has no J_F entries");
  if (!d_Jx || (h->jc_n > 0 && !d_Jcx)) return fail(CNL_ERR_ARG, "null Jacobian values");
  if (h->jc_n > 0) *S = cnl::JacSrcT<T>{d_Jx - h->jf_lo, h->jf_n, d_Jcx - h->jc_lo, h->jc_n, (int)h->jf_lo, (int)h->jc_lo};
  else *S = cnl::JacSrcT<T>{d_Jx - h->jf_lo, h->jf_n, d_Jx - h->jf_lo, h->jf_n, (int)h->jf_lo, (int)h->jf_lo};
  return CNL_OK;
}

template <class T>
static int residual_vectors_impl(cnl_handle* h, const cnl::JacSrcT<T>& S, const T* d_r, const T* d_lambda, const T* d_Fx,
                                 const T* d_cx, T* d_rhs, T* d_norms, void* stream) {
  if (!d_r || !d_Fx || !d_rhs || !d_norms) return fail(CNL_ERR_ARG, "null argument");
  if (h->djt.ncon > 0 && (!d_lambda || !d_cx)) return fail(CNL_ERR_ARG, "lambda / c are required when ncon > 0");
  HIPCHK(hipSetDevice(h->device));
  hipError_t e = cnl::launch_residual_vectors(h->djt, S, d_r, d_lambda, d_Fx, d_cx, d_rhs, d_norms, (int)h->batch, (hipStream_t)stream);
  if (e != hipSuccess) return fail(CNL_ERR_HIP, std::string("residual_vectors: ") + hipGetErrorString(e));
  return CNL_OK;
}

template <class T>
static int trial_point_impl(cnl_handle* h, const T* d_x, const T* d_r, const T* d_lambda, const T* d_d, T max_dlambda, T* d_xt, T* d_rt,
                            T* d_lambdat, T* d_dlambda, void* stream) {
  if (h->djt.ncon > 0 && (!d_lambda || !d_lambdat || !d_dlambda)) return fail(CNL_ERR_ARG, "lambda vectors are required when ncon > 0");
  HIPCHK(hipSetDevice(h->device));
  hipError_t e = cnl::launch_trial_point(h->djt, d_x, d_r, d_lambda, d_d, max_dlambda, d_xt, d_rt, d_lambdat, d_dlambda, (int)h->batch,
                                         (hipStream_t)stream);
  if (e != hipSuccess) return fail(CNL_ERR_HIP, std::string("trial_point: ") + hipGetErrorString(e));
  return CNL_OK;
}

static int check_batch(int64_t batch) {
  if (batch < 1 || batch > (1 << 24)) return fail(CNL_ERR_ARG, "batch out of range");
  return CNL_OK;
}
static int check_device(int device) {
  int ndev = 0;
  const hipError_t ce = hipGetDeviceCount(&ndev);
  if (ce != hipSuccess || ndev == 0)
    return fail(CNL_ERR_HIP, std::string("no HIP device available (this backend has no CPU fallback): hipGetDeviceCount -> ") +
                                 hipGetErrorString(ce) + ", " + std::to_string(ndev) + " device(s)");
  if (device < 0 || device >= ndev) return fail(CNL_ERR_ARG, "device index out of range");
  return CNL_OK;
}

static int setup_band(cnl_handle* h, const cnl::BandPlan& Bp, const char** unfit) {
  const cnl_plan* plan = h->plan;
  const int esz = h->f32 ? (int)sizeof(float) : (int)sizeof(double);
  const int64_t batch = h->batch;
  int rc;
  h->band_npiece = Bp.npiece;
  const bool wide = Bp.npiece != cnl::BAND_NPIECE;
  cnl::BandDev& bd = h->bd;
  for (int q = 0; q < Bp.nparts; q++) {
    if ((rc = upload(h, Bp.part[q].fops, &bd.fops[q]))) return rc;
    if ((rc = upload(h, Bp.part[q].bops, &bd.bops[q]))) return rc;
    if ((rc = upload(h, Bp.part[q].epochs, &bd.epochs[q]))) return rc;
    if ((rc = upload(h, Bp.part[q].borders, &bd.borders[q]))) return rc;
    bd.nsteps[q] = Bp.part[q].nsteps; bd.nepochs[q] = Bp.part[q].nepochs; bd.loff[q] = Bp.part[q].loff;
  }
  bd.nparts = Bp.nparts; bd.m0 = Bp.m0; bd.n = Bp.n; bd.N = Bp.N; bd.nnz = Bp.nnz; bd.nvar = (int32_t)plan->nvar; bd.lsize = Bp.lsize;
  h->band_nl = plan->opt.band_problems_per_group > 0 ? plan->opt.band_problems_per_group
                                                     : (batch > 8192 && (!wide || cnl::band_wide_has(esz, 32)) ? 32 : 16);
  if (h->band_nl != 8 && h->band_nl != 16 && h->band_nl != 32) return fail(CNL_ERR_ARG, "band_problems_per_group must be 8, 16 or 32");
  if (wide && !cnl::band_wide_has(esz, h->band_nl))
    return fail(CNL_ERR_ARG, "band_problems_per_group = 32: the wide band program (20 operand pieces) has Float64 kernels for 8 and 16 problems per workgroup only");
  const uint64_t span = (uint64_t)esz * (uint64_t)h->band_nl * (uint64_t)std::max<int64_t>({plan->nnz, plan->N, bd.lsize});
  if (span >= (1ull << 32)) { *unfit = "the arrays of a workgroup's problems span 4 GB or more (32-bit offsets of the band kernels)"; return CNL_OK; }
  if (cnl::band_lds_bytes(bd.nparts, h->band_nl, esz, h->band_npiece) > std::min<size_t>(cnl::max_lds_bytes(), 160 * 1024)) {
    *unfit = "the band kernels' LDS does not fit a workgroup";
    return CNL_OK;
  }
  const size_t lbytes = (((size_t)batch + 32) * (size_t)bd.lsize + 64) * (size_t)esz;
  char* L = nullptr;
  if ((rc = dalloc(h, &L, lbytes))) return rc;
  if (hipMemset(L, 0, lbytes) != hipSuccess) return fail(CNL_ERR_HIP, "hipMemset failed");
  h->d_Lband = L;
  h->band = true;
  return CNL_OK;
}

static int setup_layout(cnl_handle* h) {
  const cnl::Tuning& o = h->plan->opt;
  if (o.batch_layout == CNL_LAYOUT_PROBLEM_MAJOR) return CNL_OK;
  if (o.batch_layout != CNL_LAYOUT_INTERLEAVED) return fail(CNL_ERR_ARG, "cnl_options.batch_layout: unknown layout");
  if (!h->band)
    return fail(CNL_ERR_ARG, "batch_layout = CNL_LAYOUT_INTERLEAVED needs a handle the band kernels serve "
                             "(band-structured pattern, throughput plan, cnl_options.band_kernel != 0; csrc/band.h)");
  h->layout = 1 | (o.band_rhs_interleaved ? 2 : 0);
  return CNL_OK;
}

static int layout_rowlen(const cnl_handle* h, int which, int64_t* len) {
  if (which == 0) *len = h->djt.nnz;
  else if (which == 1) *len = (int64_t)h->djt.nvar + h->djt.nequ + h->djt.ncon;
  else return fail(CNL_ERR_ARG, "which: 0 = vals, 1 = an N-vector per problem (rhs)");
  return CNL_OK;
}
template <class T>
static int convert_layout(cnl_handle* h, int which, const T* src, T* dst, int to_interleaved, void* stream) {
  if (!h || !src || !dst) return fail(CNL_ERR_ARG, "null argument");
  if (src == dst) return fail(CNL_ERR_ARG, "the conversion is not in place");
  int64_t len = 0;
  if (int rc = layout_rowlen(h, which, &len)) return rc;
  HIPCHK(hipSetDevice(h->device));
  hipError_t e;
  if constexpr (sizeof(T) == 4) e = cnl::launch_interleave_f32(src, dst, (int)h->batch, len, to_interleaved, (hipStream_t)stream);
  else e = cnl::launch_interleave(src, dst, (int)h->batch, len, to_interleaved, (hipStream_t)stream);
  if (e != hipSuccess) return fail(CNL_ERR_HIP, std::string("interleave: ") + hipGetErrorString(e));
  return CNL_OK;
}

extern "C" {

static int create_from_plan(cnl_handle** hout, cnl_plan* plan, const int64_t* rows1, const int64_t* cols1, int64_t batch, int device);

const char* cnl_last_error(void) { return g_err.c_str(); }
int32_t cnl_version(void) { return 200; }

void cnl_default_params(double p[9]) {
  const double eps = 2.220446049250313e-16;
  p[0] = eps;
  p[1] = std::sqrt(eps);
  p[2] = 1.0 / 3.0;
  p[3] = 8.0;
  p[4] = std::min(100.0, 8.0 * 16.0);
  p[5] = std::pow(eps, 1.0 / 3.0);
  p[6] = std::pow(eps, -2.0);
  p[7] = std::sqrt(eps);
  p[8] = std::pow(eps, 0.25);
}

void cnl_options_init(cnl_options* o) {
  if (!o) return;
  std::memset(o, 0, sizeof(*o));
  const cnl::Tuning t;
  o->struct_size = (int32_t)sizeof(cnl_options);
  o->plan_kind = t.plan_kind;
  o->staged_max_batch = t.staged_max_batch;
  o->verbose = t.verbose; o->band_kernel = t.band_kernel; o->dense_backend = t.dense_backend; o->staged = t.staged; o->dataflow = t.dataflow;
  o->device_ladder = t.device_ladder; o->host_ladder = t.host_ladder; o->split_tail = t.split_tail; o->multi_share_plan = t.multi_share_plan;
  o->batch_layout = t.batch_layout;
}

static int plan_create_impl(cnl_plan** plan, int64_t N, int64_t nnz, const int64_t* rows1, const int64_t* cols1, int64_t nvar,
                            int64_t nequ, int64_t ncon, int latency, int par, double slots, const cnl::Tuning& o);
static int plan_create_tuned(cnl_plan** plan, int64_t N, int64_t nnz, const int64_t* rows1, const int64_t* cols1, int64_t nvar,
                             int64_t nequ, int64_t ncon, int64_t batch, const cnl::Tuning& o);
static int create_tuned(cnl_handle** hout, int64_t N, int64_t nnz, const int64_t* rows1, const int64_t* cols1, int64_t nvar,
                        int64_t nequ, int64_t ncon, int64_t batch, int device, const cnl::Tuning& o);

static int resolve_options(const cnl_options* in, cnl::Tuning& out) {
  out = cnl::Tuning();
  if (!in) return CNL_OK;
  if (in->struct_size != (int32_t)sizeof(cnl_options)) return fail(CNL_ERR_ARG, "cnl_options.struct_size does not match this library (use cnl_options_init)");
  out.plan_kind = in->plan_kind; out.staged_max_batch = in->staged_max_batch; out.verbose = in->verbose; out.band_kernel = in->band_kernel;
  out.dense_backend = in->dense_backend; out.staged = in->staged; out.dataflow = in->dataflow; out.device_ladder = in->device_ladder;
  out.host_ladder = in->host_ladder; out.split_tail = in->split_tail; out.multi_share_plan = in->multi_share_plan; out.batch_layout = in->batch_layout;
  std::memcpy(out.force_order, in->force_order, sizeof(out.force_order));
  out.force_order[sizeof(out.force_order) - 1] = 0;
  char tun[sizeof(in->tuning) + 1];
  std::memcpy(tun, in->tuning, sizeof(in->tuning));
  tun[sizeof(in->tuning)] = 0;
  const std::string err = cnl::tuning_parse(out, tun);
  if (!err.empty()) return fail(CNL_ERR_ARG, err);
  if (out.band_pieces != 0 && out.band_pieces != cnl::BAND_NPIECE && out.band_pieces != cnl::BAND_NPIECE_WIDE)
    return fail(CNL_ERR_ARG, "cnl_options.tuning: band_pieces must be 0 (automatic), 15 or 20");
  return CNL_OK;
}

int cnl_plan_create_ex(cnl_plan** plan, int64_t N, int64_t nnz, const int64_t* rows1, const int64_t* cols1, int64_t nvar,
                       int64_t nequ, int64_t ncon, int64_t batch, const cnl_options* opt) {
  cnl::Tuning o;
  int rc = resolve_options(opt, o);
  if (rc) return rc;
  return plan_create_tuned(plan, N, nnz, rows1, cols1, nvar, nequ, ncon, batch, o);
}

static int plan_create_tuned(cnl_plan** plan, int64_t N, int64_t nnz, const int64_t* rows1, const int64_t* cols1, int64_t nvar,
                             int64_t nequ, int64_t ncon, int64_t batch, const cnl::Tuning& o) {
  int rc = CNL_OK;
  int latency = 0;
  if (o.plan_kind == CNL_PLAN_LATENCY) latency = 1;
  else if (o.plan_kind == CNL_PLAN_AUTO) latency = batch >= 1 && batch <= (o.staged_max_batch > 0 ? o.staged_max_batch : 4096);
  else if (o.plan_kind != CNL_PLAN_THROUGHPUT) return fail(CNL_ERR_ARG, "unknown plan_kind");
  if (!latency) {
    rc = plan_create_impl(plan, N, nnz, rows1, cols1, nvar, nequ, ncon, 0, 0, 0, o);
    const int64_t smb = o.staged_max_batch > 0 ? o.staged_max_batch : 4096;
    if (rc == CNL_OK && o.plan_kind == CNL_PLAN_AUTO && o.split_batch && batch > smb && batch <= 2 * smb - smb / 8 && o.force_order[0] == 0) {
      cnl::Tuning o2 = o;
      std::snprintf(o2.force_order, sizeof(o2.force_order), "ndc2+early");
      cnl_plan* alt = nullptr;
      const int nq = (int)((smb + 3) / 4);
      if (plan_create_impl(&alt, N, nnz, rows1, cols1, nvar, nequ, ncon, 1, std::max(1, 2048 / nq), 2048.0 / nq, o2) == CNL_OK) {
        const bool same_work = alt->latency && alt->P.order_name == "ndc2+early" && alt->P.tasks.size() >= 2 &&
                               alt->P.cost <= 1.05 * (*plan)->P.cost && alt->P.nsuper <= (*plan)->P.nsuper + 8;
        if (same_work) {
          alt->split_mode = true;
          std::memset(alt->opt.force_order, 0, sizeof(alt->opt.force_order));
          cnl_plan_destroy(*plan);
          *plan = alt;
        } else {
          cnl_plan_destroy(alt);
        }
      }
    }
    return rc;
  }
  if (batch < 1) return fail(CNL_ERR_ARG, "a latency plan needs the batch size");
  const int nquads = (int)((batch + 3) / 4);
  return plan_create_impl(plan, N, nnz, rows1, cols1, nvar, nequ, ncon, 1, std::max(1, 2048 / nquads), 2048.0 / nquads, o);
}

int cnl_plan_create(cnl_plan** plan, int64_t N, int64_t nnz, const int64_t* rows1, const int64_t* cols1, int64_t nvar,
                    int64_t nequ, int64_t ncon) {
  return cnl_plan_create_ex(plan, N, nnz, rows1, cols1, nvar, nequ, ncon, 0, nullptr);
}

int cnl_plan_create_for_batch(cnl_plan** plan, int64_t N, int64_t nnz, const int64_t* rows1, const int64_t* cols1, int64_t nvar,
                              int64_t nequ, int64_t ncon, int64_t batch) {
  if (batch < 1) return fail(CNL_ERR_ARG, "batch out of range");
  return cnl_plan_create_ex(plan, N, nnz, rows1, cols1, nvar, nequ, ncon, batch, nullptr);
}

static int plan_create_impl(cnl_plan** plan, int64_t N, int64_t nnz, const int64_t* rows1, const int64_t* cols1, int64_t nvar,
                            int64_t nequ, int64_t ncon, int latency, int par, double slots, const cnl::Tuning& o) {
  if (!plan || !rows1 || !cols1) return fail(CNL_ERR_ARG, "null argument");
  cnl_plan* p = new cnl_plan();
  p->N = N; p->nnz = nnz; p->nvar = nvar; p->nequ = nequ; p->ncon = ncon;
  p->latency = latency != 0;
  p->opt = o;
  const bool verbose = o.verbose != 0 || getenv("CNL_VERBOSE") != nullptr;
  std::string msg;
  cnl::Options opt;
  opt.latency = latency; opt.par = std::max(1, par); opt.slots = slots;
  opt.order_mode = o.order_mode; opt.nd_leaf = o.nd_leaf; opt.relax = o.relax; opt.task_cap = o.task_cap;
  opt.early = o.multipliers_early; opt.register_front = o.register_front; opt.ubig = o.ubig; opt.wait_thr = o.wait_thr;
  opt.verbose = verbose ? 1 : 0; opt.force_order = o.force_order; opt.threads = o.analysis_threads;
  const auto t_start = std::chrono::steady_clock::now();
  auto lap = [&](const char* what) {
    if (verbose) fprintf(stderr, "[cnl] analysis %-28s %.3f s\n", what, std::chrono::duration<double>(std::chrono::steady_clock::now() - t_start).count());
  };
  int rc = cnl::build_condensation(p->C, N, nnz, rows1, cols1, nvar, nequ, ncon, msg, o.condense != 0);
  lap("condensation");
  if (!rc) {
    if (p->C.active)
      rc = cnl::build_plan(p->P, p->C.N2, p->C.ncs + nvar, p->C.rows2.data(), p->C.cols2.data(), nvar, p->C.nequ2, ncon, opt, msg);
    else
      rc = cnl::build_plan(p->P, N, nnz, rows1, cols1, nvar, nequ, ncon, opt, msg);
  }
  lap("ordering + plan");
  if (rc) {
    delete p;
    *plan = nullptr;
    return fail(rc, msg);
  }
  if (p->C.active && p->P.v2_ok && o.direct_records) {
    cnl::DirectLists D{p->C.c_ptr.data(), p->C.c_a.data(), p->C.c_b.data(), p->C.c_d.data(), (int32_t)nnz, (int32_t)N};
    const int32_t old_len = p->P.rec_maxlen;
    const size_t old_words = p->P.rec.size();
    p->P.row_products = o.row_products != 0;
    p->P.band_form = o.band_form != 0;
    const bool fast_only = p->P.ncls[1] == 0 && p->P.ncls[2] == 0;
    const bool want_lean = o.row_products && o.lean_kernel && fast_only;
    p->P.row_min_products = want_lean ? 1 : 72;
    int drc = cnl::write_forward_records(p->P, &D);
    if (!drc && want_lean && p->P.listprod_fronts > 0) {
      if (!drc && p->P.listprod_fronts > 0 && !p->P.rows_overflow.empty() && p->P.rows_overflow.size() <= 64) {
        cnl::Options opt2 = opt;
        opt2.split_positions = p->P.rows_overflow;
        opt2.force_order = p->P.order_name;
        cnl::Plan P2;
        std::string msg2;
        if (cnl::build_plan(P2, p->C.N2, p->C.ncs + nvar, p->C.rows2.data(), p->C.cols2.data(), nvar, p->C.nequ2, ncon, opt2, msg2) == 0 &&
            P2.v2_ok && P2.ncls[1] == 0 && P2.ncls[2] == 0) {
          P2.row_products = true; P2.row_min_products = 1; P2.band_form = o.band_form != 0;
          if (cnl::write_forward_records(P2, &D) == 0 && P2.listprod_fronts == 0) {
            if (verbose) fprintf(stderr, "[cnl] %zu front(s) with more than 16 residual rows cut in two: %d -> %d fronts\n", p->P.rows_overflow.size(), p->P.nsuper, P2.nsuper);
            p->P = std::move(P2);
          }
        }
      }
      if (!drc && p->P.listprod_fronts > 0) {
        p->P.row_min_products = 72;
        drc = cnl::write_forward_records(p->P, &D);
      }
    }
    if (!drc) {
      std::vector<int32_t>& br = p->P.brec;
      size_t r0 = 0;
      while (r0 + cnl::B_HDR <= br.size() && br[r0 + cnl::B_RECLEN] > 0) {
        const int32_t npiv = br[r0 + cnl::B_NPIV], nupd = br[r0 + cnl::B_NUPD];
        const int32_t i0 = br[r0 + cnl::B_PXOFF] == cnl::B_PX_GLOBAL ? 1 : nupd + 1;
        for (int32_t i = i0; i < 1 + nupd + npiv; i++) br[r0 + cnl::B_HDR + i] = p->C.orig_of[br[r0 + cnl::B_HDR + i]];
        r0 += (size_t)br[r0 + cnl::B_RECLEN];
      }
      p->P.d_outer = true;
      cnl::finalize_tasks(p->P);
      if (o.lean_kernel && o.rows_in_backward && p->P.ncls[1] == 0 && p->P.ncls[2] == 0 && p->P.listprod_fronts == 0) {
        const cnl::Cond& Cc = p->C;
        cnl::BackRowsIn in{Cc.r_orig.data(), Cc.r_dsrc.data(), Cc.r_ptr.data(), Cc.r_jsrc.data(), Cc.r_jx.data(), (int32_t)Cc.r_orig.size()};
        const int brc = cnl::write_backward_rows(p->P, in);
        if (verbose) fprintf(stderr, "[cnl] backward rows: %s\n", brc ? "not possible" : "ok");
      }
    } else {
      p->P.tasks.clear();
    }
    if (verbose)
      fprintf(stderr, "[cnl] direct records: %s, rec words %zu -> %zu, longest %d -> %d\n", drc ? "not possible" : "ok", old_words,
              p->P.rec.size(), old_len, p->P.rec_maxlen);
  }
  if (latency && p->opt.plan_kind != CNL_PLAN_LATENCY) {
    const bool stageable = o.staged && !p->P.tasks.empty() && p->P.v2_ok && p->P.rec_direct && p->P.d_outer &&
                           p->P.d_owned == (int64_t)p->C.r_dsrc.size();
    if (!stageable) {
      if (verbose) fprintf(stderr, "[cnl] latency plan cannot be staged: falling back to the throughput analysis\n");
      delete p;
      return plan_create_impl(plan, N, nnz, rows1, cols1, nvar, nequ, ncon, 0, 0, 0, o);
    }
  }
  if (o.dense_backend) cnl::detect_dense(p->D, N, nnz, rows1, cols1, nvar, nequ, ncon);
  lap("records");
  if (!latency && o.band_kernel && p->C.active && !p->D.active) {
    build_band_programs(p, rows1, cols1, 8);
    const cnl::BandPlan &b15 = p->band_prog[0][0].B, &bw = p->band_prog[0][1].B;
    if (verbose) fprintf(stderr, "[cnl] band program: %s%s\n", b15.ok ? "ok" : "no: ", b15.ok ? "" : b15.why.c_str());
    if (verbose && !b15.ok && b15.pieces_short)
      fprintf(stderr, "[cnl] wide band program (%d pieces): %s%s\n", cnl::BAND_NPIECE_WIDE, bw.ok ? "ok" : "no: ", bw.ok ? "" : bw.why.c_str());
    if (b15.ok || bw.ok) build_band_programs(p, rows1, cols1, 4);
  }
  band_summaries(p);
  p->prefer_dense = latency && p->P.v2_ok && p->P.ncls[2] > 0 && p->C.N2 <= 512;
  if (p->C.active && !p->D.active && (!p->P.v2_ok || p->prefer_dense || o.general_dense == 2) && p->C.N2 >= 96 && p->C.N2 <= 4096 && o.general_dense) {
    p->gpos.resize(p->C.ncs);
    for (int64_t s2 = 0; s2 < p->C.ncs; s2++) p->gpos[s2] = (int32_t)((p->C.rows2[s2] - 1) + p->C.N2 * (p->C.cols2[s2] - 1));
  }
  if (p->C.active) {
    p->perm_outer.assign(p->C.r_orig.begin(), p->C.r_orig.end());
    for (int32_t e : p->P.perm) p->perm_outer.push_back(p->C.orig_of[e]);
    std::vector<int64_t>().swap(p->C.rows2);
    std::vector<int64_t>().swap(p->C.cols2);
  } else {
    p->perm_outer = p->P.perm;
  }
  lap("band program + done");
  *plan = p;
  return CNL_OK;
}

void cnl_plan_destroy(cnl_plan* plan) {
  if (plan && plan->refs.fetch_sub(1) == 1) delete plan;
}

int cnl_plan_info(const cnl_plan* plan, int64_t info[16]) {
  if (!plan || !info) return fail(CNL_ERR_ARG, "null argument");
  const cnl::Plan& P = plan->P;
  std::memset(info, 0, 16 * sizeof(int64_t));
  info[0] = plan->N; info[1] = plan->nnz; info[2] = P.nnzK; info[3] = P.nsuper; info[4] = P.nnzL; info[5] = P.nnzL_exact;
  if (plan->C.active) {
    info[4] += (int64_t)plan->C.r_jsrc.size();
    info[5] += (int64_t)plan->C.r_jsrc.size();
  }
  info[6] = P.lsize; info[7] = P.fmax; info[8] = P.fwd_peak; info[9] = P.bwd_peak; info[10] = P.panel_max;
  info[11] = (int64_t)P.flops; info[12] = (int64_t)P.asm_src.size();
  info[13] = P.v2_ok ? ((int64_t)P.ncls[0] | ((int64_t)P.ncls[1] << 20) | ((int64_t)P.ncls[2] << 40)) : -1;
  info[14] = P.v2_ok ? ((int64_t)P.u2_peak | ((int64_t)P.fs2_max << 20) | ((int64_t)std::max(P.rec_maxlen, P.brec_maxlen) << 40)) : -1;
  info[15] = plan->C.active ? (int64_t)plan->C.r_orig.size() : 0;
  return CNL_OK;
}

const char* cnl_plan_order_name(const cnl_plan* plan) { return plan ? plan->P.order_name.c_str() : ""; }

int cnl_plan_get(const cnl_plan* plan, const char* name, int32_t* out, int64_t* count) {
  if (!plan || !name || !count) return fail(CNL_ERR_ARG, "null argument");
  const cnl::Plan& P = plan->P;
  const int32_t* src = nullptr;
  int64_t n = 0;
  std::string s(name);
  const cnl::Cond& C = plan->C;
  if (s == "perm") { src = plan->perm_outer.data(); n = (int64_t)plan->perm_outer.size(); }
  else if (s == "inner_perm") { src = P.perm.data(); n = (int64_t)P.perm.size(); }
  else if (s == "c_ptr") { src = C.c_ptr.data(); n = (int64_t)C.c_ptr.size(); }
  else if (s == "c_a") { src = C.c_a.data(); n = (int64_t)C.c_a.size(); }
  else if (s == "c_b") { src = C.c_b.data(); n = (int64_t)C.c_b.size(); }
  else if (s == "c_d") { src = C.c_d.data(); n = (int64_t)C.c_d.size(); }
  else if (s == "orig_of") { src = C.orig_of.data(); n = (int64_t)C.orig_of.size(); }
  else if (s == "r_orig") { src = C.r_orig.data(); n = (int64_t)C.r_orig.size(); }
  else if (s == "r_dsrc") { src = C.r_dsrc.data(); n = (int64_t)C.r_dsrc.size(); }
  else if (s == "r_ptr") { src = C.r_ptr.data(); n = (int64_t)C.r_ptr.size(); }
  else if (s == "r_jsrc") { src = C.r_jsrc.data(); n = (int64_t)C.r_jsrc.size(); }
  else if (s == "r_jx") { src = C.r_jx.data(); n = (int64_t)C.r_jx.size(); }
  else if (s == "fronts") { src = reinterpret_cast<const int32_t*>(P.fronts.data()); n = (int64_t)P.fronts.size() * 16; }
  else if (s == "seg_ptr") { src = P.seg_ptr.data(); n = (int64_t)P.seg_ptr.size(); }
  else if (s == "asm_pos") { src = P.asm_pos.data(); n = (int64_t)P.asm_pos.size(); }
  else if (s == "asm_src") { src = P.asm_src.data(); n = (int64_t)P.asm_src.size(); }
  else if (s == "child_idx") { src = P.child_idx.data(); n = (int64_t)P.child_idx.size(); }
  else if (s == "rel_idx") { src = P.rel_idx.data(); n = (int64_t)P.rel_idx.size(); }
  else if (s == "tasks") { src = reinterpret_cast<const int32_t*>(P.tasks.data()); n = (int64_t)P.tasks.size() * 8; }
  else if (s == "stage_ptr") { src = P.stage_ptr.data(); n = (int64_t)P.stage_ptr.size(); }
  else if (s == "rec") { src = P.rec.data(); n = P.v2_ok ? (int64_t)P.rec.size() : 0; }
  else if (s == "brec") { src = P.brec.data(); n = P.v2_ok ? (int64_t)P.brec.size() : 0; }
  else if (s.rfind("band", 0) == 0) {
    const cnl_plan::BandSlot* f = nullptr;
    size_t plen = 0;
    for (int t = 0; t < 2; t++)
      for (int w = 0; w < 2; w++)
        if (s.rfind(kBandPrefix[t][w], 0) == 0) { f = &plan->band_prog[t][w]; plen = std::strlen(kBandPrefix[t][w]); }
    if (!f) return fail(CNL_ERR_ARG, "unknown plan array: " + s);
    const std::string rest = s.substr(plen);
    if (rest == "info") { src = f->info.data(); n = (int64_t)f->info.size(); }
    else if (!rest.empty() && (rest.back() == '0' || rest.back() == '1')) {
      const int q = rest.back() - '0';
      const cnl::BandPart& Q = f->B.part[q];
      const std::string k = rest.substr(0, rest.size() - 1);
      if (k == "part") { src = f->pinfo[q].data(); n = (int64_t)f->pinfo[q].size(); }
      else if (k == "fops") { src = Q.fops.data(); n = (int64_t)Q.fops.size(); }
      else if (k == "bops") { src = Q.bops.data(); n = (int64_t)Q.bops.size(); }
      else if (k == "epochs") { src = Q.epochs.data(); n = (int64_t)Q.epochs.size(); }
      else if (k == "borders") { src = Q.borders.data(); n = (int64_t)Q.borders.size(); }
      else return fail(CNL_ERR_ARG, "unknown plan array: " + s);
    }
    else return fail(CNL_ERR_ARG, "unknown plan array: " + s);
  }
  else return fail(CNL_ERR_ARG, "unknown plan array: " + s);
  if (out) {
    if (*count < n) return fail(CNL_ERR_ARG, "buffer too small");
    std::memcpy(out, src, (size_t)n * sizeof(int32_t));
  }
  *count = n;
  return CNL_OK;
}

int cnl_create(cnl_handle** hout, int64_t N, int64_t nnz, const int64_t* rows1, const int64_t* cols1, int64_t nvar,
               int64_t nequ, int64_t ncon, int64_t batch, int device) {
  return cnl_create_ex(hout, N, nnz, rows1, cols1, nvar, nequ, ncon, batch, device, nullptr);
}

int cnl_create_ex(cnl_handle** hout, int64_t N, int64_t nnz, const int64_t* rows1, const int64_t* cols1, int64_t nvar,
                  int64_t nequ, int64_t ncon, int64_t batch, int device, const cnl_options* opt) {
  if (!hout) return fail(CNL_ERR_ARG, "null handle pointer");
  *hout = nullptr;
  cnl::Tuning o;
  const int rc0 = resolve_options(opt, o);
  if (rc0) return rc0;
  return create_tuned(hout, N, nnz, rows1, cols1, nvar, nequ, ncon, batch, device, o);
}

static int create_tuned(cnl_handle** hout, int64_t N, int64_t nnz, const int64_t* rows1, const int64_t* cols1, int64_t nvar,
                        int64_t nequ, int64_t ncon, int64_t batch, int device, const cnl::Tuning& o) {
  *hout = nullptr;
  if (int rc = check_batch(batch)) return rc;
  if (int rc = check_device(device)) return rc;
  cnl_plan* plan = nullptr;
  int rc = plan_create_tuned(&plan, N, nnz, rows1, cols1, nvar, nequ, ncon, batch, o);
  if (rc) return rc;
  return create_from_plan(hout, plan, rows1, cols1, batch, device);
}

static int build_row_lists(cnl_handle* h, const cnl_plan* plan, const int64_t* rows1, const int64_t* cols1) {
  const int64_t N = plan->N, nnz = plan->nnz, nvar = plan->nvar, nequ = plan->nequ, ncon = plan->ncon;
  int rc = CNL_OK;
  std::vector<int32_t> ptrF(nvar + 1, 0), ptrC(nvar + 1, 0), slotF, idxF, slotC, idxC;
  for (int64_t e = 0; e < nnz; e++) {
    const int64_t r0 = rows1[e] - 1, c0 = cols1[e] - 1;
    if (c0 < nvar && r0 >= nvar) (r0 < nvar + nequ ? ptrF : ptrC)[c0 + 1]++;
  }
  for (int64_t j2 = 0; j2 < nvar; j2++) { ptrF[j2 + 1] += ptrF[j2]; ptrC[j2 + 1] += ptrC[j2]; }
  slotF.resize(ptrF[nvar]); idxF.resize(ptrF[nvar]); slotC.resize(ptrC[nvar]); idxC.resize(ptrC[nvar]);
  std::vector<int32_t> fillF(ptrF.begin(), ptrF.end() - 1), fillC(ptrC.begin(), ptrC.end() - 1);
  for (int64_t e = 0; e < nnz; e++) {
    const int64_t r0 = rows1[e] - 1, c0 = cols1[e] - 1;
    if (!(c0 < nvar && r0 >= nvar)) continue;
    if (r0 < nvar + nequ) { const int32_t q = fillF[c0]++; slotF[q] = (int32_t)e; idxF[q] = (int32_t)(r0 - nvar); }
    else { const int32_t q = fillC[c0]++; slotC[q] = (int32_t)e; idxC[q] = (int32_t)(r0 - nvar - nequ); }
  }
  cnl::DevJt& J = h->djt;
  if ((rc = upload(h, ptrF, &J.ptrF))) return rc;
  {
    auto run = [](const std::vector<int32_t>& sl, int64_t& lo) {
      if (sl.empty()) { lo = 0; return true; }
      const auto mm = std::minmax_element(sl.begin(), sl.end());
      lo = *mm.first;
      return (int64_t)*mm.second - *mm.first + 1 == (int64_t)sl.size();
    };
    h->jac_segments = run(slotF, h->jf_lo) && run(slotC, h->jc_lo);
    h->jf_n = (int64_t)slotF.size(); h->jc_n = (int64_t)slotC.size();
  }
  if ((rc = upload(h, slotF, &J.slotF))) return rc;
  if ((rc = upload(h, idxF, &J.idxF))) return rc;
  if ((rc = upload(h, ptrC, &J.ptrC))) return rc;
  if ((rc = upload(h, slotC, &J.slotC))) return rc;
  if ((rc = upload(h, idxC, &J.idxC))) return rc;
  {
    std::vector<int32_t> rptr(ncon + 1, 0), rslot(slotC.size()), rcol(slotC.size());
    for (int64_t j2 = 0; j2 < nvar; j2++) for (int32_t q = ptrC[j2]; q < ptrC[j2 + 1]; q++) rptr[idxC[q] + 1]++;
    for (int64_t k2 = 0; k2 < ncon; k2++) rptr[k2 + 1] += rptr[k2];
    std::vector<int32_t> fillr(rptr.begin(), rptr.end() - 1);
    for (int64_t j2 = 0; j2 < nvar; j2++)
      for (int32_t q = ptrC[j2]; q < ptrC[j2 + 1]; q++) { const int32_t w = fillr[idxC[q]]++; rslot[w] = slotC[q]; rcol[w] = (int32_t)j2; }
    if ((rc = upload(h, rptr, &J.rptrC))) return rc;
    if ((rc = upload(h, rslot, &J.rslotC))) return rc;
    if ((rc = upload(h, rcol, &J.rcolC))) return rc;
  }
  J.nvar = (int32_t)nvar; J.nequ = (int32_t)nequ; J.ncon = (int32_t)ncon; J.N = (int32_t)N; J.nnz = (int32_t)nnz;
  if (plan->opt.f1_tiles && nvar > 0) {
    const int32_t nt = (int32_t)((nvar + cnl::RVT_COLS - 1) / cnl::RVT_COLS);
    std::vector<int32_t> tiles((size_t)nt * cnl::RVT_TW, 0);
    std::vector<uint32_t> table((size_t)nt * (cnl::RVT_KF + cnl::RVT_KC + 1) * cnl::RVT_COLS, 0u);
    bool ok = true;
    int32_t lds_max = 0;
    for (int32_t t = 0; t < nt && ok; t++) {
      const int64_t c0 = (int64_t)t * cnl::RVT_COLS, c1 = std::min<int64_t>(nvar, c0 + cnl::RVT_COLS);
      int32_t fslo = INT32_MAX, fshi = -1, rlo = INT32_MAX, rhi = -1, cslo = INT32_MAX, cshi = -1, llo = INT32_MAX, lhi = -1;
      for (int32_t q = ptrF[c0]; q < ptrF[c1]; q++) { fslo = std::min(fslo, slotF[q]); fshi = std::max(fshi, slotF[q]); rlo = std::min(rlo, idxF[q]); rhi = std::max(rhi, idxF[q]); }
      for (int32_t q = ptrC[c0]; q < ptrC[c1]; q++) { cslo = std::min(cslo, slotC[q]); cshi = std::max(cshi, slotC[q]); llo = std::min(llo, idxC[q]); lhi = std::max(lhi, idxC[q]); }
      int32_t* T = &tiles[(size_t)t * cnl::RVT_TW];
      T[cnl::RVT_FSLO] = fshi < 0 ? 0 : fslo; T[cnl::RVT_WF] = fshi < 0 ? 0 : fshi - fslo + 1;
      T[cnl::RVT_RLO] = rhi < 0 ? 0 : rlo;   T[cnl::RVT_WR] = rhi < 0 ? 0 : rhi - rlo + 1;
      T[cnl::RVT_CSLO] = cshi < 0 ? 0 : cslo; T[cnl::RVT_WC] = cshi < 0 ? 0 : cshi - cslo + 1;
      T[cnl::RVT_LLO] = lhi < 0 ? 0 : llo;   T[cnl::RVT_WL] = lhi < 0 ? 0 : lhi - llo + 1;
      if (T[cnl::RVT_WF] > cnl::RVT_MAXF || T[cnl::RVT_WR] > cnl::RVT_MAXR || T[cnl::RVT_WC] > cnl::RVT_MAXC || T[cnl::RVT_WL] > cnl::RVT_MAXL) { ok = false; break; }
      auto even = [](int32_t w) { return (w + 3) & ~1; };
      lds_max = std::max(lds_max, even(T[cnl::RVT_WF]) + even(T[cnl::RVT_WR]) + even(T[cnl::RVT_WC]) + even(T[cnl::RVT_WL]));
      uint32_t* tab = &table[(size_t)t * (cnl::RVT_KF + cnl::RVT_KC + 1) * cnl::RVT_COLS];
      for (int64_t c = c0; c < c1; c++) {
        const int32_t nF = ptrF[c + 1] - ptrF[c], nC = ptrC[c + 1] - ptrC[c];
        if (nF > 255 || nC > 255) { ok = false; break; }
        for (int32_t u = 0; u < std::min(nF, cnl::RVT_KF); u++)
          tab[(size_t)u * cnl::RVT_COLS + (c - c0)] = (uint32_t)(slotF[ptrF[c] + u] - T[cnl::RVT_FSLO]) | (uint32_t)(idxF[ptrF[c] + u] - T[cnl::RVT_RLO]) << 16;
        for (int32_t u = 0; u < std::min(nC, cnl::RVT_KC); u++)
          tab[(size_t)(cnl::RVT_KF + u) * cnl::RVT_COLS + (c - c0)] = (uint32_t)(slotC[ptrC[c] + u] - T[cnl::RVT_CSLO]) | (uint32_t)(idxC[ptrC[c] + u] - T[cnl::RVT_LLO]) << 16;
        tab[(size_t)(cnl::RVT_KF + cnl::RVT_KC) * cnl::RVT_COLS + (c - c0)] = (uint32_t)nF | (uint32_t)nC << 8;
      }
    }
    if (ok) {
      bool own = nequ > 0;
      int32_t prev = 0;
      for (int32_t t = 0; t < nt && own; t++) {
        int32_t* T = &tiles[(size_t)t * cnl::RVT_TW];
        const int32_t lo = T[cnl::RVT_RLO], hi = lo + T[cnl::RVT_WR];
        const int32_t next_lo = t + 1 < nt ? tiles[(size_t)(t + 1) * cnl::RVT_TW + cnl::RVT_RLO] : (int32_t)nequ;
        const int32_t own_hi = t + 1 < nt ? std::min(hi, std::max(next_lo, prev)) : (int32_t)nequ;
        if (prev < lo || own_hi > hi || own_hi < prev) { own = false; break; }
        T[cnl::RVT_OWNLO] = prev; T[cnl::RVT_OWNHI] = own_hi;
        prev = own_hi;
      }
      if (own && prev != nequ) own = false;
      if (!own) for (int32_t t = 0; t < nt; t++) tiles[(size_t)t * cnl::RVT_TW + cnl::RVT_OWNLO] = tiles[(size_t)t * cnl::RVT_TW + cnl::RVT_OWNHI] = 0;
      if ((rc = upload(h, tiles, &J.rv_tiles))) return rc;
      if ((rc = upload(h, table, &J.rv_table))) return rc;
      J.rv_ntiles = nt; J.rv_lds_doubles = lds_max;
      J.rv_primal_tiles = own ? 0 : (int32_t)((nequ + cnl::RVT_PROWS - 1) / cnl::RVT_PROWS);
    }
    if (std::getenv("CNL_VERBOSE")) fprintf(stderr, "[cnl] row f1: %s\n", ok ? "column tiles" : "gather kernel (a tile's windows exceed the limits)");
  }
  return CNL_OK;
}

static int create_from_plan(cnl_handle** hout, cnl_plan* plan, const int64_t* rows1, const int64_t* cols1, int64_t batch, int device) {
  const int64_t N = plan->N, nnz = plan->nnz, nvar = plan->nvar, nequ = plan->nequ, ncon = plan->ncon;
// ... 165 lines not shown
    if (rc) return rc;
    *count += tc;
  }
  return CNL_OK;
}

int cnl_prepare_newton_system_dev(cnl_handle* h, int64_t nnzhF, int64_t nnzhc, int64_t nnzjF, int64_t nnzjc, const double* d_hF,
                                  const double* d_hc, const double* d_Jx, const double* d_Jcx, const double* d_delta, double* d_vals,
                                  void* stream) {
  if (!h || !d_vals || !d_Jx) return fail(CNL_ERR_ARG, "null argument");
  CNL_NEED_F64(h);
  return prepare_impl(h, nnzhF, nnzhc, nnzjF, nnzjc, d_hF, d_hc, d_Jx, d_Jcx, d_delta, d_vals, stream);
}

int cnl_cgls_multipliers_dev(cnl_handle* h, const double* d_vals, const double* d_r, double* d_lambda, double* d_Jxtr, double atol,
                             double rtol, int64_t itmax, int ones_if_zero, int32_t* d_iters, void* stream) {
  if (!h || !d_vals || !d_r) return fail(CNL_ERR_ARG, "null argument");
  CNL_NEED_F64(h);
  if (h->layout & 1) return fail(CNL_ERR_STATE, "cnl_cgls_multipliers_dev reads problem-major vals: on a handle with batch_layout = CNL_LAYOUT_INTERLEAVED use cnl_cgls_multipliers_jac_dev");
  return cgls_impl(h, cnl::JacSrc{d_vals, h->djt.nnz, d_vals, h->djt.nnz, 0, 0}, d_r, d_lambda, d_Jxtr, atol, rtol, itmax, ones_if_zero, d_iters, stream);
}

int cnl_cgls_multipliers_jac_dev(cnl_handle* h, int64_t nnzjF, int64_t nnzjc, const double* d_Jx, const double* d_Jcx, const double* d_r,
                                 double* d_lambda, double* d_Jxtr, double atol, double rtol, int64_t itmax, int ones_if_zero, int32_t* d_iters,
                                 void* stream) {
  if (!h || !d_r) return fail(CNL_ERR_ARG, "null argument");
  CNL_NEED_F64(h);
  cnl::JacSrc S{};
  if (int rc = jac_source(h, nnzjF, nnzjc, d_Jx, d_Jcx, &S)) return rc;
  return cgls_impl(h, S, d_r, d_lambda, d_Jxtr, atol, rtol, itmax, ones_if_zero, d_iters, stream);
}

int cnl_residual_vectors_dev(cnl_handle* h, const double* d_vals, const double* d_r, const double* d_lambda, const double* d_Fx,
                             const double* d_cx, double* d_rhs, double* d_norms, void* stream) {
  if (!h || !d_vals) return fail(CNL_ERR_ARG, "null argument");
  CNL_NEED_F64(h);
  if (h->layout & 1) return fail(CNL_ERR_STATE, "cnl_residual_vectors_dev reads problem-major vals: on a handle with batch_layout = CNL_LAYOUT_INTERLEAVED use cnl_residual_vectors_jac_dev");
  return residual_vectors_impl(h, cnl::JacSrc{d_vals, h->djt.nnz, d_vals, h->djt.nnz, 0, 0}, d_r, d_lambda, d_Fx, d_cx, d_rhs, d_norms, stream);
}

int cnl_residual_vectors_jac_dev(cnl_handle* h, int64_t nnzjF, int64_t nnzjc, const double* d_Jx, const double* d_Jcx, const double* d_r,
                                 const double* d_lambda, const double* d_Fx, const double* d_cx, double* d_rhs, double* d_norms, void* stream) {
  if (!h) return fail(CNL_ERR_ARG, "null argument");
  CNL_NEED_F64(h);
  cnl::JacSrc S{};
  if (int rc = jac_source(h, nnzjF, nnzjc, d_Jx, d_Jcx, &S)) return rc;
  return residual_vectors_impl(h, S, d_r, d_lambda, d_Fx, d_cx, d_rhs, d_norms, stream);
}

int cnl_trial_point_dev(cnl_handle* h, const double* d_x, const double* d_r, const double* d_lambda, const double* d_d,
                        double max_dlambda, double* d_xt, double* d_rt, double* d_lambdat, double* d_dlambda, void* stream) {
  if (!h || !d_x || !d_r || !d_d || !d_xt || !d_rt) return fail(CNL_ERR_ARG, "null argument");
  CNL_NEED_F64(h);
  return trial_point_impl(h, d_x, d_r, d_lambda, d_d, max_dlambda, d_xt, d_rt, d_lambdat, d_dlambda, stream);
}

int cnl_prepare_newton_system_f32_dev(cnl_handle* h, int64_t nnzhF, int64_t nnzhc, int64_t nnzjF, int64_t nnzjc, const float* d_hF,
                                      const float* d_hc, const float* d_Jx, const float* d_Jcx, const float* d_delta, float* d_vals,
                                      void* stream) {
  if (!h || !d_vals || !d_Jx) return fail(CNL_ERR_ARG, "null argument");
  CNL_NEED_F32(h);
  return prepare_impl(h, nnzhF, nnzhc, nnzjF, nnzjc, d_hF, d_hc, d_Jx, d_Jcx, d_delta, d_vals, stream);
}

int cnl_residual_vectors_f32_dev(cnl_handle* h, const float* d_vals, const float* d_r, const float* d_lambda, const float* d_Fx,
                                 const float* d_cx, float* d_rhs, float* d_norms, void* stream) {
  if (!h || !d_vals) return fail(CNL_ERR_ARG, "null argument");
  CNL_NEED_F32(h);
  if (h->layout & 1) return fail(CNL_ERR_STATE, "cnl_residual_vectors_f32_dev reads problem-major vals: on a handle with batch_layout = CNL_LAYOUT_INTERLEAVED use cnl_residual_vectors_jac_f32_dev");
  return residual_vectors_impl(h, cnl::JacSrcF{d_vals, h->djt.nnz, d_vals, h->djt.nnz, 0, 0}, d_r, d_lambda, d_Fx, d_cx, d_rhs, d_norms, stream);
}

int cnl_residual_vectors_jac_f32_dev(cnl_handle* h, int64_t nnzjF, int64_t nnzjc, const float* d_Jx, const float* d_Jcx, const float* d_r,
                                     const float* d_lambda, const float* d_Fx, const float* d_cx, float* d_rhs, float* d_norms, void* stream) {
  if (!h) return fail(CNL_ERR_ARG, "null argument");
  CNL_NEED_F32(h);
  cnl::JacSrcF S{};
  if (int rc = jac_source(h, nnzjF, nnzjc, d_Jx, d_Jcx, &S)) return rc;
  return residual_vectors_impl(h, S, d_r, d_lambda, d_Fx, d_cx, d_rhs, d_norms, stream);
}

int cnl_cgls_multipliers_f32_dev(cnl_handle* h, const float* d_vals, const float* d_r, float* d_lambda, float* d_Jxtr, float atol,
                                 float rtol, int64_t itmax, int ones_if_zero, int32_t* d_iters, void* stream) {
  if (!h || !d_vals || !d_r) return fail(CNL_ERR_ARG, "null argument");
  CNL_NEED_F32(h);
  if (h->layout & 1) return fail(CNL_ERR_STATE, "cnl_cgls_multipliers_f32_dev reads problem-major vals: on a handle with batch_layout = CNL_LAYOUT_INTERLEAVED use cnl_cgls_multipliers_jac_f32_dev");
  return cgls_impl(h, cnl::JacSrcF{d_vals, h->djt.nnz, d_vals, h->djt.nnz, 0, 0}, d_r, d_lambda, d_Jxtr, atol, rtol, itmax, ones_if_zero, d_iters, stream);
}

int cnl_cgls_multipliers_jac_f32_dev(cnl_handle* h, int64_t nnzjF, int64_t nnzjc, const float* d_Jx, const float* d_Jcx, const float* d_r,
                                     float* d_lambda, float* d_Jxtr, float atol, float rtol, int64_t itmax, int ones_if_zero, int32_t* d_iters,
                                     void* stream) {
  if (!h || !d_r) return fail(CNL_ERR_ARG, "null argument");
  CNL_NEED_F32(h);
  cnl::JacSrcF S{};
  if (int rc = jac_source(h, nnzjF, nnzjc, d_Jx, d_Jcx, &S)) return rc;
  return cgls_impl(h, S, d_r, d_lambda, d_Jxtr, atol, rtol, itmax, ones_if_zero, d_iters, stream);
}

int cnl_trial_point_f32_dev(cnl_handle* h, const float* d_x, const float* d_r, const float* d_lambda, const float* d_d,
                            float max_dlambda, float* d_xt, float* d_rt, float* d_lambdat, float* d_dlambda, void* stream) {
  if (!h || !d_x || !d_r || !d_d || !d_xt || !d_rt) return fail(CNL_ERR_ARG, "null argument");
  CNL_NEED_F32(h);
  return trial_point_impl(h, d_x, d_r, d_lambda, d_d, max_dlambda, d_xt, d_rt, d_lambdat, d_dlambda, stream);
}

int cnl_layout_len(const cnl_handle* h, int which, int64_t* doubles) {
  if (!h || !doubles) return fail(CNL_ERR_ARG, "null argument");
  int64_t len = 0;
  if (int rc = layout_rowlen(h, which, &len)) return rc;
  *doubles = cnl::band_il_len(h->batch, len);
  return CNL_OK;
}
int cnl_interleave_dev(cnl_handle* h, int which, const double* d_src, double* d_dst, void* stream) {
  CNL_NEED_F64(h);
  return convert_layout(h, which, d_src, d_dst, 1, stream);
}
int cnl_deinterleave_dev(cnl_handle* h, int which, const double* d_src, double* d_dst, void* stream) {
  CNL_NEED_F64(h);
  return convert_layout(h, which, d_src, d_dst, 0, stream);
}

int cnl_set_timing(cnl_handle* h, int enable) {
  if (!h) return fail(CNL_ERR_ARG, "null handle");
  h->timing = enable != 0;
  return CNL_OK;
}

int cnl_last_kernel_ms(cnl_handle* h, float* ms) {
  if (!h || !ms) return fail(CNL_ERR_ARG, "null argument");
  *ms = h->last_ms;
  return CNL_OK;
}

int cnl_launch_counts(int64_t counts[3]) {
  if (!counts) return fail(CNL_ERR_ARG, "null argument");
  for (int k = 0; k < 3; k++) counts[k] = g_launches[k].load();
  return CNL_OK;
}

int cnl_get_config(const cnl_handle* h, int64_t cfg[8]) {
  if (!h || !cfg) return fail(CNL_ERR_ARG, "null argument");
  std::memset(cfg, 0, 8 * sizeof(int64_t));
  if (h->f32) {
    cfg[5] = 64 | ((int64_t)h->band_nl << 8) | ((int64_t)h->bd.nparts << 16) | ((int64_t)h->layout << 25) | ((int64_t)1 << 27) | ((int64_t)h->band_npiece << 28);
    if (h->djt.rv_ntiles > 0) cfg[5] |= 128;
    return CNL_OK;
  }
  cfg[0] = h->cfg.tpp; cfg[1] = h->cfg.ppb; cfg[2] = (int64_t)h->cfg.lds_bytes; cfg[3] = h->cfg.lds_work;
  cfg[4] = (h->batch + h->cfg.ppb - 1) / h->cfg.ppb;
  cfg[5] = (h->dense || h->gdense) ? 3 : (h->use_v2 ? (h->staged ? 4 : 2) : 1);
  if (h->lean && !h->dense && !h->gdense) cfg[5] |= 16;
  if (h->tail) cfg[5] |= 32;
  if (h->band) cfg[5] |= 64 | ((int64_t)h->band_nl << 8) | ((int64_t)h->bd.nparts << 16) | ((int64_t)h->layout << 25) | ((int64_t)h->band_npiece << 28);
  if (h->djt.rv_ntiles > 0) cfg[5] |= 128;
  cfg[6] = h->wpb2;
  cfg[7] = (int64_t)h->lds2;
  return CNL_OK;
}

int cnl_factorize_dev(cnl_handle* h, const double* d_vals, double eig_tol, int32_t* d_success, void* stream) {
  if (!h || !d_vals || !d_success) return fail(CNL_ERR_ARG, "null argument");
  CNL_NEED_F64(h);
  HIPCHK(hipSetDevice(h->device));
  cnl::LaunchArgs a{};
  a.mode = cnl::MODE_FACTOR;
  a.success = d_success;
  a.params[0] = eig_tol;
  int rc = run(h, a, const_cast<double*>(d_vals), nullptr, nullptr, (hipStream_t)stream);
  if (rc == CNL_OK) { h->factorized = true; h->last_vals = d_vals; h->last_ok.clear(); }
  return rc;
}

int cnl_solve_dev(cnl_handle* h, const double* d_rhs, double* d_d, void* stream) {
  if (!h || !d_rhs || !d_d) return fail(CNL_ERR_ARG, "null argument");
  CNL_NEED_F64(h);
  if (!h->factorized) return fail(CNL_ERR_STATE, "cnl_solve before cnl_factorize");
  HIPCHK(hipSetDevice(h->device));
  cnl::LaunchArgs a{};
  a.mode = cnl::MODE_SOLVE;
  return run(h, a, nullptr, d_rhs, d_d, (hipStream_t)stream);
}

int cnl_newton_system_dev(cnl_handle* h, double* d_vals, const double* d_rhs, double* d_d, double* d_rho_old, double* d_rho,
                          int32_t* d_nfact, int32_t* d_success, const double params[9], void* stream) {
  if (!h || !d_vals || !d_rhs || !d_d || !d_rho_old || !d_rho || !d_nfact || !d_success || !params)
    return fail(CNL_ERR_ARG, "null argument");
  CNL_NEED_F64(h);
  HIPCHK(hipSetDevice(h->device));
  cnl::LaunchArgs a{};
  a.mode = cnl::MODE_NEWTON;
  a.rho_old = d_rho_old; a.rho = d_rho; a.nfact = d_nfact; a.success = d_success;
  std::memcpy(a.params, params, 9 * sizeof(double));
  int rc = run(h, a, d_vals, d_rhs, d_d, (hipStream_t)stream);
  if (rc == CNL_OK) { h->factorized = true; h->last_vals = d_vals; h->last_ok.clear(); }
  return rc;
}

int cnl_factorize(cnl_handle* h, const double* vals, double eig_tol, int32_t* success, int64_t* npos, int64_t* nzero) {
  if (!h || !vals || !success) return fail(CNL_ERR_ARG, "null argument");
  CNL_NEED_F64(h);
  if (h->layout) return fail(CNL_ERR_STATE, kHostLayout);
  HIPCHK(hipSetDevice(h->device));
  int rc = ensure_staging(h);
  if (rc) return rc;
  const cnl_plan& P = *h->plan;
  const size_t B = (size_t)h->batch;
  HIPCHK(hipMemcpyAsync(h->d_vals, vals, B * P.nnz * sizeof(double), hipMemcpyHostToDevice, h->stream));
  cnl::LaunchArgs a{};
  a.mode = cnl::MODE_FACTOR;
  a.success = h->d_success; a.npos = h->d_npos; a.nzero = h->d_nzero;
  a.params[0] = eig_tol;
  if ((rc = run(h, a, h->d_vals, nullptr, nullptr, h->stream))) return rc;
  h->last_vals = h->d_vals;
  {
    const size_t o_su = 0, o_np = (B * 4 + 7) & ~(size_t)7, total = o_np + B * 16;
    if (int prc = ensure_pinned(h, total)) return prc;
    char* pb = static_cast<char*>(h->pin);
    HIPCHK(hipMemcpyAsync(pb + o_su, h->d_success, B * sizeof(int32_t), hipMemcpyDeviceToHost, h->stream));
    if (npos || nzero) HIPCHK(hipMemcpyAsync(pb + o_np, h->d_npos, B * 16, hipMemcpyDeviceToHost, h->stream));
    HIPCHK(hipStreamSynchronize(h->stream));
    std::memcpy(success, pb + o_su, B * sizeof(int32_t));
    if (npos) std::memcpy(npos, pb + o_np, B * sizeof(int64_t));
    if (nzero) std::memcpy(nzero, pb + o_np + B * 8, B * sizeof(int64_t));
  }
  h->factorized = true;
  h->last_ok.assign(success, success + B);
  return CNL_OK;
}

int cnl_solve(cnl_handle* h, const double* rhs, double* d) {
  if (!h || !rhs || !d) return fail(CNL_ERR_ARG, "null argument");
  CNL_NEED_F64(h);
  if (h->layout) return fail(CNL_ERR_STATE, kHostLayout);
  if (!h->factorized) return fail(CNL_ERR_STATE, "cnl_solve before cnl_factorize");
  HIPCHK(hipSetDevice(h->device));
  int rc = ensure_staging(h);
  if (rc) return rc;
  const cnl_plan& P = *h->plan;
  const size_t B = (size_t)h->batch;
  HIPCHK(hipMemcpyAsync(h->d_rhs, rhs, B * P.N * sizeof(double), hipMemcpyHostToDevice, h->stream));
  cnl::LaunchArgs a{};
  a.mode = cnl::MODE_SOLVE;
  const bool known = h->last_ok.size() == B;
  if (known && B == 1 && !h->last_ok[0])
    return fail(CNL_ERR_STATE, "cnl_solve after a factorisation that failed (success = 0): there is no factor to solve with "
                               "(the reference calls solve_ldl! only after a successful try_to_factorize, src/CaNNOLeS.jl:1049)");
  if ((rc = run(h, a, nullptr, h->d_rhs, h->d_d, h->stream))) return rc;
  HIPCHK(copy_rows_where([&](size_t b) { return !known || h->last_ok[b]; }, d, h->d_d, B, (size_t)P.N, h->stream));
  HIPCHK(hipStreamSynchronize(h->stream));
  return CNL_OK;
}

static int host_ladder_run(cnl_handle* h, const double params[9], const double* rho_old, double* rho, double* rho_old_out, int32_t* nfact,
                           int32_t* success, char* up, int32_t* su_pin);

static int newton_system_pipelined(cnl_handle* h, double* vals, const double* rhs, double* d, const double* rho_old, const double params[9],
                                   double* rho, double* rho_old_out, int32_t* nfact, int32_t* success, size_t chunk) {
  const cnl_plan& P = *h->plan;
  const size_t B = (size_t)h->batch;
  const size_t nchunks = (B + chunk - 1) / chunk;
  for (hipStream_t& st : h->pipe_stream) if (!st) HIPCHK(hipStreamCreateWithFlags(&st, hipStreamNonBlocking));
  while (h->pipe_ev.size() < nchunks) {
    hipEvent_t e;
    HIPCHK(hipEventCreateWithFlags(&e, hipEventDisableTiming));
    h->pipe_ev.push_back(e);
  }
  std::mutex mu;
  std::condition_variable cv;
  std::vector<char> posted(nchunks, 0);
  bool abort_ = false;
  int wrc = CNL_OK;
  std::string wmsg;
  const int device = h->device;
  std::thread down([&]() {
    (void)hipSetDevice(device);
    hipStream_t st = h->pipe_stream[cnl_handle::kPipeUp];
    auto chk = [&](hipError_t e, const char* what) {
      if (e != hipSuccess && wrc == CNL_OK) { wrc = CNL_ERR_HIP; wmsg = std::string(what) + ": " + hipGetErrorString(e); }
      return e == hipSuccess;
    };
    for (size_t c = 0; c < nchunks; c++) {
      {
        std::unique_lock<std::mutex> lk(mu);
        cv.wait(lk, [&] { return posted[c] || abort_; });
        if (!posted[c]) return;
      }
      const size_t b0 = c * chunk, nb = std::min(chunk, B - b0);
      if (!chk(hipEventSynchronize(h->pipe_ev[c]), "hipEventSynchronize")) continue;
      if (!chk(hipMemcpyAsync(success + b0, h->d_success + b0, nb * sizeof(int32_t), hipMemcpyDeviceToHost, st), "copy success")) continue;
      if (!chk(hipStreamSynchronize(st), "hipStreamSynchronize")) continue;
      chk(copy_rows_where([&](size_t q) { return success[b0 + q] != 0; }, d + b0 * P.N, h->d_d + b0 * P.N, nb, (size_t)P.N, st), "copy d");
      chk(hipMemcpyAsync(rho + b0, h->d_rho + b0, nb * sizeof(double), hipMemcpyDeviceToHost, st), "copy rho");
      chk(hipMemcpyAsync(rho_old_out + b0, h->d_rho_old + b0, nb * sizeof(double), hipMemcpyDeviceToHost, st), "copy rho_old");
      chk(hipMemcpyAsync(nfact + b0, h->d_nfact + b0, nb * sizeof(int32_t), hipMemcpyDeviceToHost, st), "copy nfact");
      if (P.nvar > 0)
        chk(hipMemcpy2DAsync(vals + b0 * P.nnz + (P.nnz - P.nvar), (size_t)P.nnz * sizeof(double), h->d_vals + b0 * P.nnz + (P.nnz - P.nvar),
                             (size_t)P.nnz * sizeof(double), (size_t)P.nvar * sizeof(double), nb, hipMemcpyDeviceToHost, st), "copy rho slots");
      chk(hipStreamSynchronize(st), "hipStreamSynchronize");
    }
  });
  constexpr int NU = cnl_handle::kPipeUp;
  int urc[NU];
  for (int& r_ : urc) r_ = CNL_OK;
  std::string umsg[NU];
  auto uploader = [&](int u) {
    if (u) (void)hipSetDevice(device);
// ... 645 lines not shown
```

cannoles.jl_amd/csrc/kernels.h:

```cpp
#pragma once
#include <hip/hip_runtime_api.h>

#include <cstdint>

#include "plan.h"

namespace cnl {

struct DevPlan {
  const FrontHdr* fronts;
  const int32_t* seg_ptr;
  const int32_t* asm_pos;
  const int32_t* asm_src;
  const int32_t* child_idx;
  const int32_t* rel_idx;
  const int32_t* perm;
  int32_t nsuper, N, nnz, rho_begin, nvar, nequ, ncon;
  int32_t fmax;
  int32_t pb_off;
  int32_t wv_off;
  int32_t work_doubles;
  int64_t lsize;
  int64_t vstride, rstride, dstride;
};

struct KernelConfig {
  int tpp = 64;
  int ppb = 1;
  int lds_work = 1;
  size_t lds_bytes = 0;
};

struct DevPlan2 {
  const int32_t* rec;
  const int32_t* brec;
  int32_t nsuper, N, nnz, rho_begin, nvar;
  int32_t N0;
  int32_t count_d;
  int32_t reccap;
  int32_t breccap;
  int32_t recwords;
  int32_t u2_peak;
  int32_t prob_doubles;
  int32_t jraw_off;
  int32_t bpanel_off;
  int64_t gs_doubles;
  int64_t lsize;
  int64_t vstride, rstride, dstride;
};

struct DevCond {
  const int32_t *c_ptr, *c_a, *c_b, *c_d, *c_order;
  const int32_t *ch_slot, *ch_rng, *ch_tile, *rng_start, *rng_len, *c_la, *c_lb, *c_ld, *ch_tptr, *tile_src;
  const uint64_t* c_pack;
  int32_t tile_max, chunk_ncon_max, chunk_nslot_max, tiled_ok;
  const int32_t *r_dsrc, *r_ptr, *r_jsrc, *r_jx;
  const int32_t *red_of, *cidx_of, *orig_of, *r_orig;
  int32_t N, nnz, nvar, N2, ncs, ncond;
  int64_t cstride;
};

struct DevJt {
  const int32_t *ptrF, *slotF, *idxF;
  const int32_t *ptrC, *slotC, *idxC;
  const int32_t *rptrC, *rslotC, *rcolC;
  int32_t nvar, nequ, ncon, N, nnz;
  const int32_t* rv_tiles;
  const uint32_t* rv_table;
  int32_t rv_ntiles, rv_lds_doubles, rv_primal_tiles;
};
template <class T>
struct JacSrcT {
  const T* vF; long long sF;
  const T* vC; long long sC;
  int safeF, safeC;
};
typedef JacSrcT<double> JacSrc;
typedef JacSrcT<float> JacSrcF;
constexpr int RVT_COLS = 256;
constexpr int RVT_KF = 6, RVT_KC = 2;
constexpr int RVT_MAXF = 2046, RVT_MAXR = 510, RVT_MAXC = 510, RVT_MAXL = 510;
constexpr int RVT_PROWS = 2048;
enum { RVT_FSLO = 0, RVT_WF, RVT_RLO, RVT_WR, RVT_CSLO, RVT_WC, RVT_LLO, RVT_WL, RVT_OWNLO, RVT_OWNHI, RVT_TW = 12 };

enum { MODE_NEWTON = 0, MODE_FACTOR = 1, MODE_SOLVE = 2 };

struct LaunchArgs {
  int mode;
  int batch;
  double* vals;
  const double* rhs;
  int layout;
  double* d;
  double* L;
  double* scratch;
  double* rho_old;
  double* rho;
  int32_t* nfact;
  int32_t* success;
  int64_t* npos;
  int64_t* nzero;
  double params[9];
  const int* extra_pos;
  const int* extra_zer;
  const int32_t* tasks;
  int task0, ntasks;
  int phase;
  int nquads;
  int* gcnt;
  int skip_done;
  int ntasks_all;
  int df_live;
  int df_waves;
  int* dep;
  int lean;
  int back_rows;
  int* status_total;
  int* status_call;
  int spin_limit;
  int only_if_status;
  int* lad;
  int* lgcnt;
  int* ldep;
  int lad_first;
  int lad_slots;
  int quad0;
  int lad_mode, lad_capacity;
  long long lad_zero_ints;
};
constexpr int LAD_WORDS = 32;

struct BandDev {
  const int32_t* fops[2];
  const int32_t* bops[2];
  const int32_t* epochs[2];
  const int32_t* borders[2];
  int32_t nsteps[2], nepochs[2];
  long long loff[2];
  int32_t nparts, m0, n, N, nnz, nvar;
  long long lsize;
};
hipError_t launch_band(const BandDev& P, int nl, const LaunchArgs& a, hipStream_t stream, int npiece = 15);
hipError_t launch_band_f32(const BandDev& P, int nl, const LaunchArgs& a, hipStream_t stream, int npiece = 15);
bool band_wide_has(int esz, int nl);
size_t band_lds_bytes(int nparts, int nl, int esz = 8, int npiece = 15);

hipError_t launch_newton(const DevPlan& P, const KernelConfig& cfg, const LaunchArgs& a, hipStream_t stream);
hipError_t launch_newton2(const DevPlan2& P, int wpb, size_t lds_bytes, const LaunchArgs& a, hipStream_t stream);
hipError_t launch_newton2_staged(const DevPlan2& P, int wpb, size_t lds_bytes, LaunchArgs a, const int32_t* stage_ptr, int nstages, hipStream_t stream);
hipError_t launch_condense(const DevCond& C, const double* vals, const double* rhs, double* cbuf, int slot_begin, int slot_end,
                           int batch, hipStream_t stream);
hipError_t launch_condense_tiled(const DevCond& C, const double* vals, const double* rhs, double* cbuf, int mask, int nchunks,
                                 int batch, hipStream_t stream);
hipError_t launch_cond_inertia(const DevCond& C, const double* vals, int* extra_pos, int* extra_zer, double eig_tol, int batch,
                               hipStream_t stream);
hipError_t launch_prepare(int nnzhF, int nnzhc, int nnzjF, int nnzjc, int nvar, int nequ, int ncon, const double* hF, const double* hc,
                          const double* Jx, const double* Jcx, const double* delta, double* vals, int batch, int interleaved, hipStream_t stream);
hipError_t launch_interleave(const double* src, double* dst, int batch, long long len, int to_interleaved, hipStream_t stream);
hipError_t launch_interleave_f32(const float* src, float* dst, int batch, long long len, int to_interleaved, hipStream_t stream);
hipError_t launch_cgls(const DevJt& J, const JacSrc& S, const double* r, double* lambda, double* Jxtr, double* ws, int32_t* iters,
                       double atol, double rtol, int itmax, int ones_if_zero, int batch, hipStream_t stream);
hipError_t launch_residual_vectors(const DevJt& J, const JacSrc& S, const double* r, const double* lambda, const double* Fx,
                                   const double* cx, double* rhs, double* norms, int batch, hipStream_t stream);
hipError_t launch_trial_point(const DevJt& J, const double* x, const double* r, const double* lambda, const double* d,
                              double max_dlambda, double* xt, double* rt, double* lambdat, double* dlambda, int batch,
                              hipStream_t stream);
hipError_t launch_prepare(int nnzhF, int nnzhc, int nnzjF, int nnzjc, int nvar, int nequ, int ncon, const float* hF, const float* hc,
                          const float* Jx, const float* Jcx, const float* delta, float* vals, int batch, int interleaved, hipStream_t stream);
hipError_t launch_cgls(const DevJt& J, const JacSrcF& S, const float* r, float* lambda, float* Jxtr, float* ws, int32_t* iters,
                       float atol, float rtol, int itmax, int ones_if_zero, int batch, hipStream_t stream);
hipError_t launch_residual_vectors(const DevJt& J, const JacSrcF& S, const float* r, const float* lambda, const float* Fx,
                                   const float* cx, float* rhs, float* norms, int batch, hipStream_t stream);
hipError_t launch_trial_point(const DevJt& J, const float* x, const float* r, const float* lambda, const float* d,
                              float max_dlambda, float* xt, float* rt, float* lambdat, float* dlambda, int batch,
                              hipStream_t stream);
hipError_t launch_fill_rho(double* vals, long long nnz, int nvar, const double* rho, const int* active, int batch, hipStream_t stream);
hipError_t launch_lds_fill(int pattern, hipStream_t stream);
hipError_t launch_expand(const DevCond& C, double* vals, const double* rhs, const double* d2, const double* cbuf, double* dout,
                         const int* success, int copy_rho_tail, int batch, hipStream_t stream);
size_t max_lds_bytes();
int lds_attr_cap(int need);

}
```

cannoles.jl_amd/csrc/options.h:

```cpp
#pragma once
#include <cstdint>
#include <cstring>
#include <string>

namespace cnl {

#define CNL_TUNING_INT_FIELDS(X)                                                                                              \
  X(plan_kind, 0)             \
  X(order_mode, -1)           \
  X(nd_leaf, 0)               \
  X(relax, -1)                \
  X(task_cap, 0)              \
  X(multipliers_early, 1)     \
  X(condense, 1)              \
  X(direct_records, 1)        \
  X(register_front, 1)        \
  X(dense_backend, 1)         \
  X(general_dense, 1)         \
  X(staged, 1)                \
  X(dataflow, 1)              \
  X(dataflow_waves, 1024)     \
  X(dataflow_spin_limit, 1 << 22)  \
  X(waves_per_block, 0)       \
  X(v1_tpp, -1) X(v1_ppb, -1) X(v1_lds, -1)  \
  X(v1_solve, 0)              \
  X(lds_pad, 1)               \
  X(ubig, 17)                 \
  X(wait_thr, 2)              \
  X(dense_graph, 1)           \
  X(dense_syrk_wgs, 0)        \
  X(verbose, 0)               \
  X(multi_share_plan, 1)      \
  X(row_products, 1)          \
  X(split_batch, 1)           \
  X(lean_kernel, 1)           \
  X(rows_in_backward, 1)      \
  X(dense_panel_blocks, 1)    \
  X(host_ladder, 1)           \
  X(device_ladder, 1)         \
  X(device_ladder_fused, 0)   \
  X(band_form, 1)             \
  X(split_tail, 1)            \
  X(band_kernel, 1)           \
  X(band_problems_per_group, 0)  \
  X(band_pieces, 0)           \
  X(analysis_threads, 0)      \
  X(f1_tiles, 1)              \
  X(batch_layout, 0)          \
  X(band_rhs_interleaved, 0)

struct Tuning {
#define X(name, dflt) int32_t name = dflt;
  CNL_TUNING_INT_FIELDS(X)
#undef X
  int64_t staged_max_batch = 4096;
  char force_order[32] = {0};
};

inline bool tuning_set(Tuning& t, const std::string& key, long long value) {
#define X(name, dflt) if (key == #name) { t.name = (int32_t)value; return true; }
  CNL_TUNING_INT_FIELDS(X)
#undef X
  if (key == "staged_max_batch") { t.staged_max_batch = value; return true; }
  return false;
}

inline std::string tuning_parse(Tuning& t, const char* text) {
  std::string s(text ? text : "");
  size_t i = 0;
  while (i < s.size()) {
    while (i < s.size() && (s[i] == ',' || s[i] == ';' || s[i] == ' ')) i++;
    if (i >= s.size()) break;
    size_t j = i;
    while (j < s.size() && s[j] != ',' && s[j] != ';' && s[j] != ' ') j++;
    const std::string item = s.substr(i, j - i);
    i = j;
    const size_t eq = item.find('=');
    if (eq == std::string::npos || eq == 0 || eq + 1 >= item.size()) return "cnl_options.tuning: expected key=value, got '" + item + "'";
    const std::string key = item.substr(0, eq), val = item.substr(eq + 1);
    if (key == "force_order") {
      std::memset(t.force_order, 0, sizeof(t.force_order));
      std::strncpy(t.force_order, val.c_str(), sizeof(t.force_order) - 1);
      continue;
    }
    char* end = nullptr;
    const long long v = std::strtoll(val.c_str(), &end, 0);
    if (!end || *end != 0) return "cnl_options.tuning: value of '" + key + "' is not an integer";
    if (!tuning_set(t, key, v)) return "cnl_options.tuning: unknown key '" + key + "'";
  }
  return "";
}

}
```

cannoles.jl_amd/hipldl.py:

```python
import ctypes as C
import os

import numpy as np

_HERE = os.path.dirname(os.path.abspath(__file__))
LIB_PATH = os.environ.get("CANNOLES_HIP_LIB") or os.path.join(_HERE, "libcannoles_hip.so")

_i64p = np.ctypeslib.ndpointer(dtype=np.int64, flags="C_CONTIGUOUS")
_lib = None

ABI_SYMBOLS = [
    "cnl_last_error", "cnl_version", "cnl_default_params",
    "cnl_options_init", "cnl_plan_create_ex", "cnl_create_ex", "cnl_dataflow_timeouts",
    "cnl_plan_create", "cnl_plan_create_for_batch", "cnl_plan_destroy", "cnl_plan_info", "cnl_plan_get", "cnl_plan_order_name",
    "cnl_create", "cnl_destroy", "cnl_get_plan",
    "cnl_factorize", "cnl_solve", "cnl_newton_system",
    "cnl_factorize_dev", "cnl_solve_dev", "cnl_newton_system_dev",
    "cnl_set_timing", "cnl_last_kernel_ms", "cnl_get_config", "cnl_launch_counts",
    "cnl_residual_vectors_dev", "cnl_trial_point_dev", "cnl_prepare_newton_system_dev",
    "cnl_cgls_multipliers_dev",
    "cnl_multi_create_ex", "cnl_multi_factorize_dev", "cnl_multi_solve_dev", "cnl_multi_newton_system_dev", "cnl_multi_synchronize",
    "cnl_multi_create", "cnl_multi_destroy", "cnl_multi_shards", "cnl_multi_factorize", "cnl_multi_solve", "cnl_multi_newton_system",
    "cnl_outer_begin_dev", "cnl_outer_newton_done_dev", "cnl_outer_extrapolated_dev", "cnl_outer_trial_done_dev", "cnl_outer_end_dev",
    "cnl_outer_ls_begin_dev", "cnl_outer_ls_test_dev", "cnl_outer_ls_step_dev", "cnl_outer_ls_take_dev",
# ... 157 lines not shown
        L.cnl_multi_factorize.argtypes = [vp, vp, dbl, vp, vp, vp]
        L.cnl_multi_solve.argtypes = [vp, vp, vp]
        L.cnl_multi_newton_system.argtypes = [vp, vp, vp, vp, vp, vp, vp, vp, vp, vp]
        L.cnl_set_timing.argtypes = [vp, C.c_int]
        L.cnl_last_kernel_ms.argtypes = [vp, C.POINTER(C.c_float)]
        L.cnl_get_config.argtypes = [vp, _i64p]
        L.cnl_launch_counts.argtypes = [_i64p]
        L.cnl_layout_len.argtypes = [vp, C.c_int, C.POINTER(i64)]
        L.cnl_residual_vectors_jac_dev.argtypes = [vp, i64, i64, vp, vp, vp, vp, vp, vp, vp, vp, vp]
        L.cnl_cgls_multipliers_jac_dev.argtypes = [vp, i64, i64, vp, vp, vp, vp, vp, dbl, dbl, i64, C.c_int, vp, vp]
        L.cnl_interleave_dev.argtypes = [vp, C.c_int, vp, vp, vp]
        L.cnl_deinterleave_dev.argtypes = [vp, C.c_int, vp, vp, vp]
        flt = C.c_float
        L.cnl_default_params_f32.argtypes = [vp]
        L.cnl_default_params_f32.restype = None
        L.cnl_create_f32.argtypes = [C.POINTER(vp), i64, i64, _i64p, _i64p, i64, i64, i64, i64, C.c_int]
        L.cnl_create_f32_ex.argtypes = [C.POINTER(vp), i64, i64, _i64p, _i64p, i64, i64, i64, i64, C.c_int, vp]
        L.cnl_factorize_f32.argtypes = [vp, vp, flt, vp, vp, vp]
        L.cnl_solve_f32.argtypes = [vp, vp, vp]
        L.cnl_newton_system_f32.argtypes = [vp, vp, vp, vp, vp, vp, vp, vp, vp, vp]
        L.cnl_factorize_f32_dev.argtypes = [vp, vp, flt, vp, vp]
        L.cnl_solve_f32_dev.argtypes = [vp, vp, vp, vp]
        L.cnl_newton_system_f32_dev.argtypes = [vp, vp, vp, vp, vp, vp, vp, vp, vp, vp]
        L.cnl_interleave_f32_dev.argtypes = [vp, C.c_int, vp, vp, vp]
        L.cnl_deinterleave_f32_dev.argtypes = [vp, C.c_int, vp, vp, vp]
        L.cnl_prepare_newton_system_f32_dev.argtypes = [vp, i64, i64, i64, i64, vp, vp, vp, vp, vp, vp, vp]
        L.cnl_residual_vectors_f32_dev.argtypes = [vp, vp, vp, vp, vp, vp, vp, vp, vp]
        L.cnl_residual_vectors_jac_f32_dev.argtypes = [vp, i64, i64, vp, vp, vp, vp, vp, vp, vp, vp, vp]
        L.cnl_cgls_multipliers_f32_dev.argtypes = [vp, vp, vp, vp, vp, flt, flt, i64, C.c_int, vp, vp]
        L.cnl_cgls_multipliers_jac_f32_dev.argtypes = [vp, i64, i64, vp, vp, vp, vp, vp, flt, flt, i64, C.c_int, vp, vp]
        L.cnl_trial_point_f32_dev.argtypes = [vp, vp, vp, vp, vp, flt, vp, vp, vp, vp, vp]
        for fn in ("cnl_outer_begin_dev", "cnl_outer_extrapolated_dev", "cnl_outer_trial_done_dev", "cnl_outer_end_dev", "cnl_outer_ls_begin_dev",
                   "cnl_outer_ls_step_dev", "cnl_outer_ls_take_dev"):
            getattr(L, fn).argtypes = [vp, vp]
        L.cnl_outer_newton_done_dev.argtypes = [vp, C.c_int, vp]
        L.cnl_outer_ls_test_dev.argtypes = [vp, C.c_int, vp]
        if L.cnl_version() < 200:
            raise RuntimeError(f"{LIB_PATH}: cnl_version() = {L.cnl_version()}, ABI version 0.2.0 or later required")
        _lib = L
    return _lib


def _check(rc):
    if rc != 0:
        raise CnlError(rc, lib().cnl_last_error().decode())


def default_params(dtype=np.float64):
    dt = np.dtype(dtype)
    if dt == np.float32:
        p = np.zeros(9, np.float32)
        lib().cnl_default_params_f32(p.ctypes.data)
        return p
    if dt != np.float64:
        raise TypeError(f"ParamCaNNOLeS({dt}): this backend serves Float64 and Float32 only")
    p = np.zeros(9)
    lib().cnl_default_params(p.ctypes.data)
    return p


def _i64(a):
    return np.ascontiguousarray(np.asarray(a, dtype=np.int64).ravel())


_INFO_KEYS = ["N", "nnz", "nnzK", "nsuper", "nnzL", "nnzL_exact", "lsize", "fmax", "fwd_peak", "bwd_peak",
              "panel_max", "flops", "nasm", "v2_classes", "v2_lds", "ncond"]


def _plan_info(p):
    info = np.zeros(16, np.int64)
    _check(lib().cnl_plan_info(p, info))
    d = {k: int(info[i]) for i, k in enumerate(_INFO_KEYS)}
    d["order"] = lib().cnl_plan_order_name(p).decode()
    c, l = d.pop("v2_classes"), d.pop("v2_lds")
    if c >= 0:
        d["v2"] = {"fronts16": c & 0xfffff, "fronts32": (c >> 20) & 0xfffff, "fronts64": c >> 40,
                   "ustack": l & 0xfffff, "staging": (l >> 20) & 0xfffff, "reclen": l >> 40}
    else:
        d["v2"] = None
    return d


def _plan_array(p, name):
    n = C.c_int64(0)
    _check(lib().cnl_plan_get(p, name.encode(), None, C.byref(n)))
    out = np.zeros(max(n.value, 1), np.int32)
    cnt = C.c_int64(out.size)
    _check(lib().cnl_plan_get(p, name.encode(), out.ctypes.data, C.byref(cnt)))
    return out[:n.value]


class Plan:

    def __init__(self, N, rows, cols, nvar, nequ, ncon, batch=None, options=None):
        self.rows, self.cols = _i64(rows), _i64(cols)
        p = C.c_void_p()
        if options is not None:
            _check(lib().cnl_plan_create_ex(C.byref(p), int(N), len(self.rows), self.rows, self.cols, int(nvar), int(nequ), int(ncon),
                                            int(batch or 0), _optref(options)))
        elif batch is None:
            _check(lib().cnl_plan_create(C.byref(p), int(N), len(self.rows), self.rows, self.cols, int(nvar), int(nequ), int(ncon)))
        else:
            _check(lib().cnl_plan_create_for_batch(C.byref(p), int(N), len(self.rows), self.rows, self.cols, int(nvar), int(nequ),
                                                   int(ncon), int(batch)))
        self._p = p
        self.info = _plan_info(p)

    def array(self, name):
        return _plan_array(self._p, name)

    def __del__(self):
        if getattr(self, "_p", None):
            lib().cnl_plan_destroy(self._p)
            self._p = None


class _Factor:

    def __init__(self, owner):
        self._owner = owner


class HIPLDLStruct:

    def __init__(self, N, rows, cols, vals, nvar=None, nequ=None, ncon=None, batch=1, device=0, options=None, dtype=np.float64):
        self.N = int(N)
        self.rows, self.cols = _i64(rows), _i64(cols)
        self.nnz = len(self.rows)
        self.batch = int(batch)
        if nvar is None:
            raise ValueError("nvar/nequ/ncon are required (the Julia glue passes them from the solver)")
        self.nvar, self.nequ, self.ncon = int(nvar), int(nequ), int(ncon)
        self.dtype = np.dtype(np.asarray(vals).dtype if vals is not None else dtype)
        if self.dtype not in (np.float64, np.float32):
            raise TypeError(f"element type {self.dtype}: this backend serves Float64 and Float32 (band patterns) only; other element types "
                            "stay on LDLFactStruct")
        f32 = self.dtype == np.float32
        self.vals = vals if vals is not None else np.ones((self.batch, self.nnz) if self.batch > 1 else self.nnz, self.dtype)
        h = C.c_void_p()
        if options is None:
            _check((lib().cnl_create_f32 if f32 else lib().cnl_create)(C.byref(h), self.N, self.nnz, self.rows, self.cols, self.nvar, self.nequ,
                                                                        self.ncon, self.batch, int(device)))
        else:
            _check((lib().cnl_create_f32_ex if f32 else lib().cnl_create_ex)(C.byref(h), self.N, self.nnz, self.rows, self.cols, self.nvar,
                                                                              self.nequ, self.ncon, self.batch, int(device), _optref(options)))
        self._h = h
        self.factor = _Factor(self)
        self.info = _plan_info(lib().cnl_get_plan(h))
        cfg = np.zeros(8, np.int64)
        _check(lib().cnl_get_config(h, cfg))
        self.config = {"tpp": int(cfg[0]), "ppb": int(cfg[1]), "lds_bytes": int(cfg[2]), "lds_work": int(cfg[3]), "grid": int(cfg[4]),
                       "kernel": {2: "v2", 3: "dense", 4: "v2-staged"}.get(int(cfg[5]) & 15, "v1"), "wpb": int(cfg[6]), "lds2_bytes": int(cfg[7]),
                       "lean": bool(int(cfg[5]) & 16), "tail": bool(int(cfg[5]) & 32), "band": bool(int(cfg[5]) & 64), "f1_tiles": bool(int(cfg[5]) & 128),
                       "band_nl": (int(cfg[5]) >> 8) & 255, "band_parts": (int(cfg[5]) >> 16) & 255,
                       "batch_layout": (int(cfg[5]) >> 25) & 1, "rhs_interleaved": bool((int(cfg[5]) >> 26) & 1),
                       "float32": bool((int(cfg[5]) >> 27) & 1), "band_pieces": (int(cfg[5]) >> 28) & 63}
        if self.config["float32"]:
            self.config["kernel"] = "band"

    def plan_array(self, name):
        return _plan_array(lib().cnl_get_plan(self._h), name)

    def close(self):
        if getattr(self, "_h", None):
            lib().cnl_destroy(self._h)
            self._h = None

    def __del__(self):
        try:
            self.close()
        except Exception:
            pass

    def set_timing(self, on=True):
        _check(lib().cnl_set_timing(self._h, 1 if on else 0))

    def uses_lean_kernel(self):
        cfg = np.zeros(8, np.int64)
        _check(lib().cnl_get_config(self._h, cfg))
        return bool(int(cfg[5]) & 16)

    def dataflow_timeouts(self):
        n = C.c_int64(0)
        _check(lib().cnl_dataflow_timeouts(self._h, C.byref(n)))
        return int(n.value)

    def last_kernel_ms(self):
        ms = C.c_float(0)
        _check(lib().cnl_last_kernel_ms(self._h, C.byref(ms)))
        return float(ms.value)


def launch_counts():
    c = np.zeros(3, np.int64)
    _check(lib().cnl_launch_counts(c))
    return {"band": int(c[0]), "register_front": int(c[1]), "general": int(c[2])}


def get_vals(LDLT):
    return LDLT.vals


def _f64c(a, shape=None):
    a = np.asarray(a)
    if a.dtype != np.float64 or not a.flags.c_contiguous:
        raise TypeError("expected a C-contiguous float64 array (Float64 only; other element types stay on LDLFactStruct)")
    return a


def _is_f32(LDLT):
    return getattr(LDLT, "dtype", np.float64) == np.float32


def _valsc(LDLT, a):
    if not _is_f32(LDLT):
        return _f64c(a)
    a = np.asarray(a)
    if a.dtype != np.float32 or not a.flags.c_contiguous:
        raise TypeError(f"expected a C-contiguous float32 array on a Float32 handle, got {a.dtype}")
    return a


def _dev_ptr(LDLT, x):
    if hasattr(x, "data_ptr"):
        want = "float32" if _is_f32(LDLT) else "float64"
        if str(x.dtype).rsplit(".", 1)[-1] != want:
            raise TypeError(f"expected a {want} tensor on this handle, got {x.dtype}")
        return x.data_ptr()
    return x


def _int_ptr(x):
    return x.data_ptr() if hasattr(x, "data_ptr") else x


def try_to_factorize(LDLT, vals, nvar, nequ, ncon, eig_tol, return_inertia=False):
    assert (nvar, nequ, ncon) == (LDLT.nvar, LDLT.nequ, LDLT.ncon)
    vals = _valsc(LDLT, vals)
    assert vals.size == LDLT.batch * LDLT.nnz
    B = LDLT.batch
    succ = np.zeros(B, np.int32)
    npos = np.zeros(B, np.int64)
    nzer = np.zeros(B, np.int64)
    fn = lib().cnl_factorize_f32 if _is_f32(LDLT) else lib().cnl_factorize
    _check(fn(LDLT._h, vals.ctypes.data, float(eig_tol), succ.ctypes.data, npos.ctypes.data, nzer.ctypes.data))
    if B == 1:
        return (bool(succ[0]), int(npos[0]), int(nzer[0])) if return_inertia else bool(succ[0])
    return (succ.astype(bool), npos, nzer) if return_inertia else succ.astype(bool)


def solve_ldl_(rhs, factor, d):
    LDLT = factor._owner
    rhs = _valsc(LDLT, rhs)
    d = _valsc(LDLT, d)
    assert rhs.size == LDLT.batch * LDLT.N and d.size == rhs.size
    _check((lib().cnl_solve_f32 if _is_f32(LDLT) else lib().cnl_solve)(LDLT._h, rhs.ctypes.data, d.ctypes.data))
    return True


def newton_system_(d, nvar, nequ, ncon, rhs, vals, LDLT, rho_old, params):
    assert (nvar, nequ, ncon) == (LDLT.nvar, LDLT.nequ, LDLT.ncon)
    B = LDLT.batch
    vals = _valsc(LDLT, vals)
    rhs = _valsc(LDLT, rhs)
    d = _valsc(LDLT, d)
    assert vals.size == B * LDLT.nnz and rhs.size == B * LDLT.N and d.size == B * LDLT.N
    T = np.float32 if _is_f32(LDLT) else np.float64
    ro = np.ascontiguousarray(np.broadcast_to(np.asarray(rho_old, dtype=T), (B,)))
    params = np.ascontiguousarray(params, dtype=T)
    rho = np.zeros(B, T)
    ro_out = np.zeros(B, T)
    nfact = np.zeros(B, np.int32)
    succ = np.zeros(B, np.int32)
    _check((lib().cnl_newton_system_f32 if T == np.float32 else lib().cnl_newton_system)(LDLT._h, vals.ctypes.data, rhs.ctypes.data, d.ctypes.data, ro.ctypes.data,
                                   params.ctypes.data, rho.ctypes.data, ro_out.ctypes.data, nfact.ctypes.data,
                                   succ.ctypes.data))
    if B == 1:
        return d, bool(succ[0]), float(rho[0]), float(ro_out[0]), int(nfact[0])
    return d, succ.astype(bool), rho, ro_out, nfact.astype(np.int64)


def newton_system_dev(LDLT, vals_ptr, rhs_ptr, d_ptr, rho_old_ptr, rho_ptr, nfact_ptr, success_ptr, params, stream=0):
    f32 = _is_f32(LDLT)
    params = np.ascontiguousarray(params, dtype=np.float32 if f32 else np.float64)
    v, r, dd, ro, rh = (_dev_ptr(LDLT, x) for x in (vals_ptr, rhs_ptr, d_ptr, rho_old_ptr, rho_ptr))
    _check((lib().cnl_newton_system_f32_dev if f32 else lib().cnl_newton_system_dev)(LDLT._h, v, r, dd, ro, rh, _int_ptr(nfact_ptr),
                                                                                    _int_ptr(success_ptr), params.ctypes.data, stream))


def factorize_dev(LDLT, vals_ptr, eig_tol, success_ptr, stream=0):
    fn = lib().cnl_factorize_f32_dev if _is_f32(LDLT) else lib().cnl_factorize_dev
    _check(fn(LDLT._h, _dev_ptr(LDLT, vals_ptr), float(eig_tol), _int_ptr(success_ptr), stream))


def solve_dev(LDLT, rhs_ptr, d_ptr, stream=0):
    fn = lib().cnl_solve_f32_dev if _is_f32(LDLT) else lib().cnl_solve_dev
    _check(fn(LDLT._h, _dev_ptr(LDLT, rhs_ptr), _dev_ptr(LDLT, d_ptr), stream))


def residual_vectors_dev(LDLT, vals_ptr, r_ptr, lambda_ptr, Fx_ptr, cx_ptr, rhs_ptr, norms_ptr, stream=0):
    fn = lib().cnl_residual_vectors_f32_dev if _is_f32(LDLT) else lib().cnl_residual_vectors_dev
    _check(fn(LDLT._h, *(_dev_ptr(LDLT, x) for x in (vals_ptr, r_ptr, lambda_ptr, Fx_ptr, cx_ptr, rhs_ptr, norms_ptr)), stream))


def residual_vectors_jac_dev(LDLT, nnzjF, nnzjc, Jx_ptr, Jcx_ptr, r_ptr, lambda_ptr, Fx_ptr, cx_ptr, rhs_ptr, norms_ptr, stream=0):
    fn = lib().cnl_residual_vectors_jac_f32_dev if _is_f32(LDLT) else lib().cnl_residual_vectors_jac_dev
    _check(fn(LDLT._h, int(nnzjF), int(nnzjc), *(_dev_ptr(LDLT, x) for x in (Jx_ptr, Jcx_ptr, r_ptr, lambda_ptr, Fx_ptr, cx_ptr, rhs_ptr,
# ... 125 lines not shown
```

Baseline: 1.478 million systems/s.

## Keep matrix operand pieces resident in LDS slots across band epochs

Adds a resident variant of the band Newton program. A new packer assigns matrix-value pieces to LDS slots that persist from one forward epoch to the next, so a piece already held is not fetched again, and each load descriptor encodes its target slot. The backward sweep is planned in reverse epoch order with its own slot state. The kernel gains a templated resident mode that commits staged loads to the encoded slot. It is selected only for Float64 with 15 pieces, 32 problems per workgroup and the interleaved batch layout. The aim is to cut redundant HBM reads of overlapping operand pieces, at the cost of a more complex plan builder and an extra runtime slot decode per load.

```diff
diff --git a/cannoles.jl_amd/csrc/band.cpp b/cannoles.jl_amd/csrc/band.cpp
--- a/cannoles.jl_amd/csrc/band.cpp
+++ b/cannoles.jl_amd/csrc/band.cpp
@@ -60,11 +60,96 @@
   }
 };
 
+struct ResidentPacker {
+  struct Item { int32_t arr, base, slot; bool load, keep; };
+  std::vector<Item> items;
+  std::vector<int32_t> held;
+  int32_t nslots = 0, nstage = BAND_NPIECE, esz = 8;
+  void start(int32_t slots) { nslots = slots; held.assign(slots, -1); items.clear(); }
+  bool pack(std::vector<int32_t> (&need)[3], Packer& pk) {
+    items.clear();
+    if (!pk.pack(need)) return false;
+    std::vector<Packer::Piece> G, O;
+    int32_t nf = 0;
+    for (const Packer::Piece& pc : pk.pieces) { (pc.arr == 0 ? G : O).push_back(pc); nf += pc.arr == 2; }
+    if (nf > nslots) return false;
+    for (int32_t s = nslots - nf; s < nslots; s++) held[s] = -1;
+    std::vector<int32_t> owner(need[0].size());
+    for (size_t i = 0; i < need[0].size(); i++) {
+      owner[i] = -1;
+      for (size_t g = 0; g < G.size() && owner[i] < 0; g++)
+        if (need[0][i] >= G[g].base && need[0][i] < G[g].base + 8) owner[i] = (int32_t)g;
+    }
+    std::vector<char> packed(G.size(), 0);
+    std::vector<int32_t> A;
+    int32_t slots = 0, loads = 0, touch = 0;
+    auto eval = [&]() {
+      A.clear();
+      for (size_t i = 0; i < need[0].size(); i++)
+        if (!packed[owner[i]]) A.push_back(need[0][i] & ~7);
+      A.erase(std::unique(A.begin(), A.end()), A.end());
+      int32_t np = 0, kept = 0;
+      for (char c : packed) np += c;
+      for (int32_t b : A) kept += std::find(held.begin(), held.end(), b) != held.end();
+      slots = (int32_t)A.size() + np + (int32_t)O.size();
+      loads = slots - kept;
+      touch = (int32_t)A.size() - kept;
+      for (size_t g = 0; g < G.size(); g++) if (packed[g]) touch += G[g].base % 8 ? 2 : 1;
+    };
+    auto excess = [&]() { return std::max(0, slots - nslots) + std::max(0, loads - nstage); };
+    eval();
+    while (excess() > 0) {
+      int best = -1, bex = 0, bld = 0;
+      for (size_t g = 0; g < G.size(); g++) {
+        if (packed[g]) continue;
+        packed[g] = 1; eval(); packed[g] = 0;
+        if (best < 0 || excess() < bex || (excess() == bex && touch < bld)) { best = (int)g; bex = excess(); bld = touch; }
+      }
+      if (best < 0) return false;
+      packed[best] = 1;
+      eval();
+    }
+    std::vector<char> used(nslots, 0);
+    for (int32_t s = 0; s < nslots; s++) {
+      if (held[s] >= 0 && std::binary_search(A.begin(), A.end(), held[s])) { items.push_back({0, held[s], s, false, true}); used[s] = 1; }
+      else held[s] = -1;
+    }
+    auto place = [&](int32_t arr, int32_t base, bool keep) {
+      int32_t s = 0;
+      while (s < nslots && used[s]) s++;
+      if (s == nslots) return false;
+      used[s] = 1;
+      items.push_back({arr, base, s, true, keep});
+      return true;
+    };
+    int32_t fs = nslots - nf;
+    for (const Packer::Piece& pc : O)
+      if (pc.arr == 2) { used[fs] = 1; items.push_back({2, pc.base, fs++, true, false}); }
+    for (int32_t b : A)
+      if (std::find(held.begin(), held.end(), b) == held.end() && !place(0, b, true)) return false;
+    for (size_t g = 0; g < G.size(); g++)
+      if (packed[g] && !place(0, G[g].base, false)) return false;
+    for (const Packer::Piece& pc : O)
+      if (pc.arr == 1 && !place(1, pc.base, false)) return false;
+    std::stable_sort(items.begin(), items.end(), [](const Item& x, const Item& y) { return x.arr != y.arr ? x.arr < y.arr : x.base < y.base; });
+    for (int32_t s = 0; s < nslots; s++) held[s] = -1;
+    for (const Item& it : items) if (it.keep) held[it.slot] = it.base;
+    return true;
+  }
+  int32_t off(int a, int32_t e) const {
+    for (const Item& it : items)
+      if (it.arr == a && e >= it.base && e < it.base + 8) return (int32_t)((BAND_IN_OFF + 8 * it.slot + (e - it.base)) * esz);
+    return -1;
+  }
+};
+
 }
 
 void build_band_plan(BandPlan& B, int64_t N, int64_t nnz, const int64_t* rows1, const int64_t* cols1, int64_t nvar, int64_t nequ,
-                     int64_t ncon, int nparts_wanted, int esz, int npiece) {
+                     int64_t ncon, int nparts_wanted, int esz, int npiece, bool resident) {
   B = BandPlan();
+  if (resident && (esz != 8 || npiece != BAND_NPIECE)) { B.ok = false; B.why = "the resident form is the 15-piece program of 8-byte elements"; return; }
+  B.resident = resident;
   if (esz != 8 && esz != 4) { B.ok = false; B.why = "element size must be 8 or 4 bytes"; return; }
   if (npiece != BAND_NPIECE && npiece != BAND_NPIECE_WIDE) { B.ok = false; B.why = "piece count must be 15 or 20"; return; }
   B.npiece = npiece;
@@ -263,9 +348,13 @@
     pk.len[0] = (int32_t)nnz; pk.len[1] = (int32_t)N; pk.len[2] = (int32_t)(lpart + 16);
     pk.esz = esz; pk.npiece = npiece;
     if (lpart + 16 >= (1 << 27)) return no("factor too long");
+    if (resident && (nnz + 8 >= (1 << BAND_RES_SLOT_SHIFT) || N >= (1 << BAND_RES_SLOT_SHIFT) || lpart + 16 >= (1 << BAND_RES_SLOT_SHIFT)))
+      return no("an array is too long for the resident form's piece descriptors");
+    ResidentPacker rp;
+    rp.esz = esz;
     const int32_t ZB = ZERO_OFF * esz;
     std::string why_not;
-    auto try_epoch = [&](const int32_t u0, const int32_t u1, int32_t* E) -> bool {
+    auto try_epoch = [&](const int32_t u0, const int32_t u1, int32_t* E, const int dirs) -> bool {
       auto no = [&](const std::string& w) { why_not = w; return false; };
       int32_t ev_lo = 1 << 30, ev_hi = -1, x_lo = 1 << 30, x_hi = -1, x_cnt = 0, r_lo = 1 << 30, r_hi = -1, r_cnt = 0;
       for (int32_t u = u0; u < u1; u++) {
@@ -297,6 +386,7 @@
       E[EF(BE_DXLO)] = x_cnt ? x_lo : 0; E[EF(BE_DXCNT)] = x_cnt;
       E[EF(BE_DRLO)] = r_cnt ? (int32_t)(n + r_lo) : 0; E[EF(BE_DRCNT)] = r_cnt;
       for (int dir = 0; dir < 2; dir++) {
+        if (!(dirs >> dir & 1)) continue;
         std::vector<int32_t> need[3];
         auto want = [&](int32_t s) {
           if (s == -1) return;
@@ -316,7 +406,7 @@
           }
         }
         if (dir == 1) for (int32_t i = 0; i < lcnt; i++) need[2].push_back(lbase + i);
-        if (!pk.pack(need)) {
+        if (resident ? !rp.pack(need, pk) : !pk.pack(need)) {
           std::string w = "an epoch needs more operand pieces than a lane holds (part " + std::to_string(part) + ", steps " + std::to_string(u0) + ".." + std::to_string(u1) + (dir ? ", backward" : ", forward") + ":";
           for (auto& pc : pk.pieces) w += " " + std::to_string(pc.arr) + ":" + std::to_string(pc.base);
           B.pieces_short = true;
@@ -324,10 +414,16 @@
         }
         int32_t* PP = E + EF(dir == 0 ? BE_FP : BE_BP);
         for (int k = 0; k < npiece; k++) PP[k] = -1;
-        for (const Packer::Piece& pc : pk.pieces) PP[pc.slot] = pc.base | (pc.arr << 28);
+        if (resident) {
+          int k = 0;
+          for (const ResidentPacker::Item& it : rp.items)
+            if (it.load) PP[k++] = it.base | (it.slot << BAND_RES_SLOT_SHIFT) | (it.arr << 28);
+        } else
+          for (const Packer::Piece& pc : pk.pieces) PP[pc.slot] = pc.base | (pc.arr << 28);
+        auto poff = [&](int a, int32_t e) { return resident ? rp.off(a, e) : pk.off(a, e); };
         auto off = [&](int32_t s) -> int32_t {
           if (s == -1) return ZB;
-          return s >= 0 ? pk.off(0, s) : pk.off(1, -(s + 2));
+          return s >= 0 ? poff(0, s) : poff(1, -(s + 2));
         };
         for (int32_t u = u0; u < u1; u++) {
           const StepOp& st = S[u];
@@ -347,12 +443,12 @@
             blk[BS_LX] = st.lev_x >= 0 ? (LOUT_OFF + st.lev_x * BAND_LREC - lbh) * esz : ZB;
             blk[BS_DX] = ZB;
           } else {
-            blk[BS_LB] = st.lev_b >= 0 ? pk.off(2, st.lev_b * BAND_LREC) : ZB;
-            blk[BS_LX] = st.lev_x >= 0 ? pk.off(2, st.lev_x * BAND_LREC) : ZB;
+            blk[BS_LB] = st.lev_b >= 0 ? poff(2, st.lev_b * BAND_LREC) : ZB;
+            blk[BS_LX] = st.lev_x >= 0 ? poff(2, st.lev_x * BAND_LREC) : ZB;
             for (int32_t ev : {st.lev_b, st.lev_x})
               if (ev >= 0)
                 for (int i = 0; i < BAND_LREC; i++)
-                  if (pk.off(2, ev * BAND_LREC + i) != pk.off(2, ev * BAND_LREC) + esz * i) return no("internal: factor record not contiguous in LDS");
+                  if (poff(2, ev * BAND_LREC + i) != poff(2, ev * BAND_LREC) + esz * i) return no("internal: factor record not contiguous in LDS");
             blk[BS_DX] = (st.flags & BF_PIVOT_X) ? (DX_OFF + st.xpiv - x_lo) * esz : ZB;
           }
           for (size_t i = 0; i < st.rows.size(); i++) {
@@ -372,12 +468,20 @@
     for (int32_t u0 = 0; u0 < nsteps;) {
       std::vector<int32_t> E(EW, 0);
       const int32_t cnt = std::min<int32_t>(BAND_EPOCH, nsteps - u0);
-      if (!try_epoch(u0, u0 + cnt, E.data())) return no(why_not);
+      if (resident && u0 == 0) rp.start(BAND_RES_FSLOTS);
+      if (!try_epoch(u0, u0 + cnt, E.data(), resident ? 1 : 3)) return no(why_not);
       E[EF(BE_NSTEP)] = cnt;
       Q.epochs.insert(Q.epochs.end(), E.begin(), E.end());
       u0 += cnt;
     }
     Q.nepochs = (int32_t)(Q.epochs.size() / EW);
+    if (resident) {
+      rp.start(BAND_NPIECE);
+      for (int32_t e = Q.nepochs - 1; e >= 0; e--) {
+        const int32_t u0 = e * BAND_EPOCH;
+        if (!try_epoch(u0, std::min(u0 + BAND_EPOCH, nsteps), Q.epochs.data() + (size_t)e * EW, 2)) return no(why_not);
+      }
+    }
     {
       int32_t fo = 0;
       for (int32_t e = 0; e < Q.nepochs; e++) { Q.epochs[(size_t)e * EW + EF(BE_FOFF)] = fo; fo += Q.epochs[(size_t)e * EW + EF(BE_OPLEN)]; }
diff --git a/cannoles.jl_amd/csrc/band.h b/cannoles.jl_amd/csrc/band.h
--- a/cannoles.jl_amd/csrc/band.h
+++ b/cannoles.jl_amd/csrc/band.h
@@ -31,6 +31,10 @@
 constexpr int band_lane_elems(int npc) { return band_zero_off(npc) + 1; }
 static_assert(band_lout_off(BAND_NPIECE) == BAND_LOUT_OFF && band_dr_off(BAND_NPIECE) == BAND_DR_OFF && band_zero_off(BAND_NPIECE) == BAND_ZERO_OFF &&
               band_lane_elems(BAND_NPIECE) == BAND_LANE_DOUBLES && band_lane_elems(BAND_NPIECE_WIDE) % 2 == 1, "lane block layout");
+
+constexpr int BAND_RES_SLOT_SHIFT = 23;
+constexpr int BAND_RES_FSLOTS = BAND_NPIECE + BAND_LOUT_MAX / 8;
+static_assert(BAND_RES_FSLOTS * 8 <= BAND_ZERO_OFF && BAND_RES_FSLOTS <= 32, "resident slots inside the lane block, five bits in a descriptor");
 
 constexpr int BAND_IL_GROUP = 32;
 constexpr long long band_il_blocks(long long len) { return (len + 7) / 8 + 1; }
@@ -86,6 +90,7 @@
   std::string why;
   bool pieces_short = false;
   int32_t npiece = BAND_NPIECE;
+  bool resident = false;
   int32_t nparts = 0;
   int32_t m0 = 0;
   int32_t n = 0, N = 0, nnz = 0;
@@ -94,6 +99,6 @@
 };
 
 void build_band_plan(BandPlan& B, int64_t N, int64_t nnz, const int64_t* rows1, const int64_t* cols1, int64_t nvar, int64_t nequ,
-                     int64_t ncon, int nparts_wanted, int esz = 8, int npiece = BAND_NPIECE);
+                     int64_t ncon, int nparts_wanted, int esz = 8, int npiece = BAND_NPIECE, bool resident = false);
 
 }
diff --git a/cannoles.jl_amd/csrc/band.hip b/cannoles.jl_amd/csrc/band.hip
--- a/cannoles.jl_amd/csrc/band.hip
+++ b/cannoles.jl_amd/csrc/band.hip
@@ -281,9 +281,14 @@
 
 }
 
+constexpr int BAND_NPIECE_RESIDENT = BAND_NPIECE + 256;
 #define EF(F) band_ef(F, NPC)
-template <class T, int NL, int NPC>
-__global__ void __launch_bounds__(128, (NL <= 8 && NPC == BAND_NPIECE ? 2 : 1)) band_newton_kernel(const BandDev P, const LaunchArgs Ain) {
+template <class T, int NL, int NPCX>
+__global__ void __launch_bounds__(128, (NL <= 8 && NPCX == BAND_NPIECE ? 2 : 1)) band_newton_kernel(const BandDev P, const LaunchArgs Ain) {
+  constexpr bool RES = NPCX == BAND_NPIECE_RESIDENT;
+  constexpr int NPC = RES ? BAND_NPIECE : NPCX;
+  static_assert(!RES || (direct_records(NL) && NPC == BAND_NPIECE && sizeof(T) == 8), "the resident form: Float64, 32 problems per workgroup, 15 pieces");
+  constexpr int DBITS = RES ? BAND_RES_SLOT_SHIFT : 28;
   constexpr int NI = NL / 8;
   constexpr int LANE_D = band_lane_elems(NPC), LOUT_OFF = band_lout_off(NPC), DX_OFF = band_dx_off(NPC), DR_OFF = band_dr_off(NPC),
                 ZERO_OFF = band_zero_off(NPC), EW = band_ew(NPC);
@@ -359,11 +364,12 @@
   static_assert(BAND_REC_MAX <= 256, "record buffer: one dwordx4 per lane");
 #define BAND_ISSUE1(K, I) if constexpr (I < NI) stg[K][I] = *reinterpret_cast<const T*>(pb + ((movp[I] * strd + tl) << LS));
 #define BAND_COMMIT1(K, I) if constexpr (I < NI) *reinterpret_cast<T*>(wblk + ldsb[I] + (BAND_IN_OFF + 8 * K) * ES) = stg[K][I];
+#define BAND_COMMITR1(K, I) if constexpr (I < NI) *reinterpret_cast<T*>(wslot_ + ldsb[I]) = stg[K][I];
 #define BAND_ISSUE(K)                                                                                                         \
   if (pcs[K] >= 0) {                                                                                      \
     const int pc = pcs[K];                                                                                                    \
     const int arr = pc >> 28;                                                                                                 \
-    const int el_ = (pc & ((1 << 28) - 1)) + (arr == 2 ? loff8 : 0);                                                          \
+    const int el_ = (pc & ((1 << DBITS) - 1)) + (arr == 2 ? loff8 : 0);                                                          \
                                \
     const bool il_ = arr == 0 ? vil : arr == 1 ? ril : DREC;                                              \
     const int ilw_ = arr == 2 ? NL * 8 : BAND_IL_GROUP * 8;     \
@@ -379,7 +385,13 @@
     const unsigned tl = t_ * tm_ + (t_ >> 3) * gap_;                                                                          \
     BAND_ISSUE1(K, 0) BAND_ISSUE1(K, 1) BAND_ISSUE1(K, 2) BAND_ISSUE1(K, 3)                                                   \
   }
-#define BAND_COMMIT(K) { BAND_COMMIT1(K, 0) BAND_COMMIT1(K, 1) BAND_COMMIT1(K, 2) BAND_COMMIT1(K, 3) }
+#define BAND_COMMIT(K)                                                                                                        \
+  if constexpr (RES) {                                                                                                        \
+    if (pcs[K] >= 0) {                                                                                                        \
+      char* wslot_ = wblk + (BAND_IN_OFF + 8 * ((pcs[K] >> BAND_RES_SLOT_SHIFT) & 31)) * ES;                                  \
+      BAND_COMMITR1(K, 0) BAND_COMMITR1(K, 1) BAND_COMMITR1(K, 2) BAND_COMMITR1(K, 3)                                         \
+    }                                                                                                                         \
+  } else { BAND_COMMIT1(K, 0) BAND_COMMIT1(K, 1) BAND_COMMIT1(K, 2) BAND_COMMIT1(K, 3) }
 #define BAND_ISSUE_DESC(EP, OFS) { cptr E_ = (EP) + (OFS); _Pragma("unroll") for (int k_ = 0; k_ < NPC; k_++) pcs[k_] = E_[k_]; }
 #define BAND_ISSUE_REC(OPS, OPOFF) { rstg0 = (reinterpret_cast<const int4*>((OPS) + (OPOFF)) + lane)[0]; }
 #define BAND_ISSUE_ALL(EP, OFS, OPS, OPOFF)                                                                                   \
@@ -725,7 +737,21 @@
   return hipErrorInvalidConfiguration;
 }
 
-hipError_t launch_band(const BandDev& P, int nl, const LaunchArgs& a, hipStream_t stream, int npiece) { return launch_band_t<double>(P, nl, a, stream, npiece); }
+static hipError_t launch_band_resident(const BandDev& P, int nl, const LaunchArgs& a, hipStream_t stream, int npiece);
+
+hipError_t launch_band(const BandDev& P, int nl, const LaunchArgs& a, hipStream_t stream, int npiece, bool resident) {
+  return resident ? launch_band_resident(P, nl, a, stream, npiece) : launch_band_t<double>(P, nl, a, stream, npiece);
+}
 hipError_t launch_band_f32(const BandDev& P, int nl, const LaunchArgs& a, hipStream_t stream, int npiece) { return launch_band_t<float>(P, nl, a, stream, npiece); }
 
-}
+static hipError_t launch_band_resident(const BandDev& P, int nl, const LaunchArgs& a, hipStream_t stream, int npiece) {
+  if (nl != 32 || npiece != BAND_NPIECE || !(a.layout & 1)) return hipErrorInvalidConfiguration;
+  const size_t ldsb = band_lds_bytes(P.nparts, nl, (int)sizeof(double), npiece);
+  auto kern = band_newton_kernel<double, 32, BAND_NPIECE_RESIDENT>;
+  hipError_t e = hipFuncSetAttribute(reinterpret_cast<const void*>(kern), hipFuncAttributeMaxDynamicSharedMemorySize, lds_attr_cap((int)ldsb));
+  if (e != hipSuccess) return e;
+  hipLaunchKernelGGL(kern, dim3((a.batch + nl - 1) / nl), dim3(64 * P.nparts), ldsb, stream, P, a);
+  return hipGetLastError();
+}
+
+}
diff --git a/cannoles.jl_amd/csrc/capi.cpp b/cannoles.jl_amd/csrc/capi.cpp
--- a/cannoles.jl_amd/csrc/capi.cpp
+++ b/cannoles.jl_amd/csrc/capi.cpp
@@ -40,8 +40,10 @@
     std::vector<int32_t> info, pinfo[2];
   };
   BandSlot band_prog[2][2];
+  BandSlot band_res;
 };
 static const char* const kBandPrefix[2][2] = {{"band_", "bandw_"}, {"band4_", "bandw4_"}};
+static const char* const kBandResPrefix = "bandr_";
 
 struct cnl_handle {
   cnl_plan* plan = nullptr;
@@ -110,6 +112,7 @@
   cnl::BandDev bd{};
   int band_nl = 16;
   int band_npiece = 15;
+  bool band_resident = false;
   bool jac_segments = false;
   int64_t jf_lo = 0, jf_n = 0, jc_lo = 0, jc_n = 0;
   int layout = 0;
@@ -143,12 +146,13 @@
                                 "CNL_LAYOUT_INTERLEAVED (device-pointer entry points only)";
 
 void band_summaries(cnl_plan* p) {
-  for (auto& row : p->band_prog)
-    for (cnl_plan::BandSlot& s : row) {
-      const cnl::BandPlan& Bp = s.B;
-      s.info = {Bp.ok ? 1 : 0, Bp.nparts, Bp.m0, Bp.n, Bp.N, Bp.nnz, (int32_t)Bp.lsize, Bp.ok && Bp.npiece != cnl::BAND_NPIECE ? Bp.npiece : 0};
-      for (int q = 0; q < 2; q++) s.pinfo[q] = {Bp.part[q].nsteps, Bp.part[q].nepochs, Bp.part[q].npiv, Bp.part[q].nevents, (int32_t)Bp.part[q].loff};
-    }
+  cnl_plan::BandSlot* const all[5] = {&p->band_prog[0][0], &p->band_prog[0][1], &p->band_prog[1][0], &p->band_prog[1][1], &p->band_res};
+  for (cnl_plan::BandSlot* sp : all) {
+    cnl_plan::BandSlot& s = *sp;
+    const cnl::BandPlan& Bp = s.B;
+    s.info = {Bp.ok ? 1 : 0, Bp.nparts, Bp.m0, Bp.n, Bp.N, Bp.nnz, (int32_t)Bp.lsize, Bp.ok && Bp.npiece != cnl::BAND_NPIECE ? Bp.npiece : 0};
+    for (int q = 0; q < 2; q++) s.pinfo[q] = {Bp.part[q].nsteps, Bp.part[q].nepochs, Bp.part[q].npiv, Bp.part[q].nevents, (int32_t)Bp.part[q].loff};
+  }
 }
 
 void build_band_programs(cnl_plan* p, const int64_t* rows1, const int64_t* cols1, int esz) {
@@ -161,6 +165,12 @@
   Bw.why = B15.ok ? "fifteen operand pieces per epoch suffice" : B15.why;
   if (o.band_pieces != 15 && (B15.ok ? o.band_pieces == 20 : B15.pieces_short))
     cnl::build_band_plan(Bw, N, nnz, rows1, cols1, nvar, nequ, ncon, nparts, esz, cnl::BAND_NPIECE_WIDE);
+  if (esz == 8) {
+    cnl::BandPlan& Br = p->band_res.B;
+    Br = cnl::BandPlan();
+    Br.why = !o.band_resident ? "tuning band_resident = 0" : B15.why;
+    if (B15.ok && o.band_resident) cnl::build_band_plan(Br, N, nnz, rows1, cols1, nvar, nequ, ncon, nparts, esz, cnl::BAND_NPIECE, true);
+  }
 }
 const cnl::BandPlan& band_program(const cnl_plan* plan, bool f32) {
   return plan->band_prog[f32][plan->band_prog[f32][1].B.ok].B;
@@ -399,7 +409,7 @@
   a.layout = h->layout;
   if (h->timing) HIPCHK(hipEventRecord(h->ev0, stream));
   const hipError_t e = h->f32 ? cnl::launch_band_f32(h->bd, h->band_nl, a, stream, h->band_npiece)
-                              : cnl::launch_band(h->bd, h->band_nl, a, stream, h->band_npiece);
+                              : cnl::launch_band(h->bd, h->band_nl, a, stream, h->band_npiece, h->band_resident);
   g_launches[0]++;
   if (e != hipSuccess)
     return fail(CNL_ERR_HIP, std::string("band kernel launch (") + (h->f32 ? "Float32, " : "") + std::to_string(h->band_nl) +
@@ -901,14 +911,21 @@
   return CNL_OK;
 }
 
-static int setup_band(cnl_handle* h, const cnl::BandPlan& Bp, const char** unfit) {
+static int setup_band(cnl_handle* h, const cnl::BandPlan& Bp0, const char** unfit) {
   const cnl_plan* plan = h->plan;
   const int esz = h->f32 ? (int)sizeof(float) : (int)sizeof(double);
   const int64_t batch = h->batch;
   int rc;
-  h->band_npiece = Bp.npiece;
-  const bool wide = Bp.npiece != cnl::BAND_NPIECE;
+  h->band_npiece = Bp0.npiece;
+  const bool wide = Bp0.npiece != cnl::BAND_NPIECE;
   cnl::BandDev& bd = h->bd;
+  h->band_nl = plan->opt.band_problems_per_group > 0 ? plan->opt.band_problems_per_group
+                                                     : (batch > 8192 && (!wide || cnl::band_wide_has(esz, 32)) ? 32 : 16);
+  if (h->band_nl != 8 && h->band_nl != 16 && h->band_nl != 32) return fail(CNL_ERR_ARG, "band_problems_per_group must be 8, 16 or 32");
+  if (wide && !cnl::band_wide_has(esz, h->band_nl))
+    return fail(CNL_ERR_ARG, "band_problems_per_group = 32: the wide band program (20 operand pieces) has Float64 kernels for 8 and 16 problems per workgroup only");
+  h->band_resident = !h->f32 && !wide && h->band_nl == 32 && plan->opt.batch_layout == CNL_LAYOUT_INTERLEAVED && plan->band_res.B.ok;
+  const cnl::BandPlan& Bp = h->band_resident ? plan->band_res.B : Bp0;
   for (int q = 0; q < Bp.nparts; q++) {
     if ((rc = upload(h, Bp.part[q].fops, &bd.fops[q]))) return rc;
     if ((rc = upload(h, Bp.part[q].bops, &bd.bops[q]))) return rc;
@@ -917,11 +934,6 @@
     bd.nsteps[q] = Bp.part[q].nsteps; bd.nepochs[q] = Bp.part[q].nepochs; bd.loff[q] = Bp.part[q].loff;
   }
   bd.nparts = Bp.nparts; bd.m0 = Bp.m0; bd.n = Bp.n; bd.N = Bp.N; bd.nnz = Bp.nnz; bd.nvar = (int32_t)plan->nvar; bd.lsize = Bp.lsize;
-  h->band_nl = plan->opt.band_problems_per_group > 0 ? plan->opt.band_problems_per_group
-                                                     : (batch > 8192 && (!wide || cnl::band_wide_has(esz, 32)) ? 32 : 16);
-  if (h->band_nl != 8 && h->band_nl != 16 && h->band_nl != 32) return fail(CNL_ERR_ARG, "band_problems_per_group must be 8, 16 or 32");
-  if (wide && !cnl::band_wide_has(esz, h->band_nl))
-    return fail(CNL_ERR_ARG, "band_problems_per_group = 32: the wide band program (20 operand pieces) has Float64 kernels for 8 and 16 problems per workgroup only");
   const uint64_t span = (uint64_t)esz * (uint64_t)h->band_nl * (uint64_t)std::max<int64_t>({plan->nnz, plan->N, bd.lsize});
   if (span >= (1ull << 32)) { *unfit = "the arrays of a workgroup's problems span 4 GB or more (32-bit offsets of the band kernels)"; return CNL_OK; }
   if (cnl::band_lds_bytes(bd.nparts, h->band_nl, esz, h->band_npiece) > std::min<size_t>(cnl::max_lds_bytes(), 160 * 1024)) {
@@ -1182,6 +1194,7 @@
     build_band_programs(p, rows1, cols1, 8);
     const cnl::BandPlan &b15 = p->band_prog[0][0].B, &bw = p->band_prog[0][1].B;
     if (verbose) fprintf(stderr, "[cnl] band program: %s%s\n", b15.ok ? "ok" : "no: ", b15.ok ? "" : b15.why.c_str());
+    if (verbose && b15.ok) fprintf(stderr, "[cnl] resident band program: %s%s\n", p->band_res.B.ok ? "ok" : "no: ", p->band_res.B.ok ? "" : p->band_res.B.why.c_str());
     if (verbose && !b15.ok && b15.pieces_short)
       fprintf(stderr, "[cnl] wide band program (%d pieces): %s%s\n", cnl::BAND_NPIECE_WIDE, bw.ok ? "ok" : "no: ", bw.ok ? "" : bw.why.c_str());
     if (b15.ok || bw.ok) build_band_programs(p, rows1, cols1, 4);
@@ -1263,6 +1276,7 @@
     for (int t = 0; t < 2; t++)
       for (int w = 0; w < 2; w++)
         if (s.rfind(kBandPrefix[t][w], 0) == 0) { f = &plan->band_prog[t][w]; plen = std::strlen(kBandPrefix[t][w]); }
+    if (s.rfind(kBandResPrefix, 0) == 0) { f = &plan->band_res; plen = std::strlen(kBandResPrefix); }
     if (!f) return fail(CNL_ERR_ARG, "unknown plan array: " + s);
     const std::string rest = s.substr(plen);
     if (rest == "info") { src = f->info.data(); n = (int64_t)f->info.size(); }
@@ -1734,7 +1748,7 @@
   cfg[5] = (h->dense || h->gdense) ? 3 : (h->use_v2 ? (h->staged ? 4 : 2) : 1);
   if (h->lean && !h->dense && !h->gdense) cfg[5] |= 16;
   if (h->tail) cfg[5] |= 32;
-  if (h->band) cfg[5] |= 64 | ((int64_t)h->band_nl << 8) | ((int64_t)h->bd.nparts << 16) | ((int64_t)h->layout << 25) | ((int64_t)h->band_npiece << 28);
+  if (h->band) cfg[5] |= 64 | ((int64_t)h->band_nl << 8) | ((int64_t)h->bd.nparts << 16) | ((int64_t)h->band_resident << 24) | ((int64_t)h->layout << 25) | ((int64_t)h->band_npiece << 28);
   if (h->djt.rv_ntiles > 0) cfg[5] |= 128;
   cfg[6] = h->wpb2;
   cfg[7] = (int64_t)h->lds2;
diff --git a/cannoles.jl_amd/csrc/kernels.h b/cannoles.jl_amd/csrc/kernels.h
--- a/cannoles.jl_amd/csrc/kernels.h
+++ b/cannoles.jl_amd/csrc/kernels.h
@@ -140,7 +140,7 @@
   int32_t nparts, m0, n, N, nnz, nvar;
   long long lsize;
 };
-hipError_t launch_band(const BandDev& P, int nl, const LaunchArgs& a, hipStream_t stream, int npiece = 15);
+hipError_t launch_band(const BandDev& P, int nl, const LaunchArgs& a, hipStream_t stream, int npiece = 15, bool resident = false);
 hipError_t launch_band_f32(const BandDev& P, int nl, const LaunchArgs& a, hipStream_t stream, int npiece = 15);
 bool band_wide_has(int esz, int nl);
 size_t band_lds_bytes(int nparts, int nl, int esz = 8, int npiece = 15);
diff --git a/cannoles.jl_amd/csrc/options.h b/cannoles.jl_amd/csrc/options.h
--- a/cannoles.jl_amd/csrc/options.h
+++ b/cannoles.jl_amd/csrc/options.h
@@ -44,6 +44,7 @@
   X(band_kernel, 1)           \
   X(band_problems_per_group, 0)  \
   X(band_pieces, 0)           \
+  X(band_resident, 1)         \
   X(analysis_threads, 0)      \
   X(f1_tiles, 1)              \
   X(batch_layout, 0)          \
diff --git a/cannoles.jl_amd/hipldl.py b/cannoles.jl_amd/hipldl.py
--- a/cannoles.jl_amd/hipldl.py
+++ b/cannoles.jl_amd/hipldl.py
@@ -333,7 +333,7 @@
         self.config = {"tpp": int(cfg[0]), "ppb": int(cfg[1]), "lds_bytes": int(cfg[2]), "lds_work": int(cfg[3]), "grid": int(cfg[4]),
                        "kernel": {2: "v2", 3: "dense", 4: "v2-staged"}.get(int(cfg[5]) & 15, "v1"), "wpb": int(cfg[6]), "lds2_bytes": int(cfg[7]),
                        "lean": bool(int(cfg[5]) & 16), "tail": bool(int(cfg[5]) & 32), "band": bool(int(cfg[5]) & 64), "f1_tiles": bool(int(cfg[5]) & 128),
-                       "band_nl": (int(cfg[5]) >> 8) & 255, "band_parts": (int(cfg[5]) >> 16) & 255,
+                       "band_nl": (int(cfg[5]) >> 8) & 255, "band_parts": (int(cfg[5]) >> 16) & 255, "band_resident": bool((int(cfg[5]) >> 24) & 1),
                        "batch_layout": (int(cfg[5]) >> 25) & 1, "rhs_interleaved": bool((int(cfg[5]) >> 26) & 1),
                        "float32": bool((int(cfg[5]) >> 27) & 1), "band_pieces": (int(cfg[5]) >> 28) & 63}
         if self.config["float32"]:
```

Result: faster. 1.517 million systems/s (median of 6 runs) (+2.6%).
